# YuyangSunshine/ABR_IOD

Hardware: AMD Instinct MI355X
Metric: training images/sec (R50-C4 Faster R-CNN + ARD) (higher is better)
Workload: dtype f32 (tensors, accumulation and error bound; contractions via a 2-term fp16 split of both operands scaled by their amax, 3 cross products on the fp16 matrix cores: f16x3)

## Files before the change

abr_iod_amd/_lib.py:

```python
import ctypes as C
import os

import torch

_HERE = os.path.dirname(os.path.abspath(__file__))
LIB_PATH = os.environ.get("ABR_IOD_HIP_LIB") or os.path.join(_HERE, "libabr_iod_hip.so")

NCHW, NHWC = 0, 1

_vp, _i, _f, _i64 = C.c_void_p, C.c_int, C.c_float, C.c_int64


class ConvDesc(C.Structure):

    _fields_ = [
        ("B", _i), ("H", _i), ("W", _i), ("Cin", _i),
        ("Cout", _i), ("R", _i), ("S", _i),
        ("stride", _i), ("pad", _i),
        ("Ho", _i), ("Wo", _i),
        ("scale", _vp), ("bias", _vp), ("residual", _vp), ("mask", _vp),
        ("relu", _i),
        ("out_H", _i), ("out_W", _i), ("out_sh", _i), ("out_sw", _i),
        ("math", _i),
        ("wino_v", _vp),
        ("w_planes", _vp),
        ("w_version", _i64),
        ("x_amax", _vp), ("x_amax_epoch", C.c_uint32),
        ("gy_amax", _vp), ("gy_amax_epoch", C.c_uint32),
        ("out_amax", _vp), ("out_amax_epoch", C.c_uint32),
    ]


class ConvOp(C.Structure):

    _fields_ = [("kind", C.c_int32), ("reserved", C.c_int32), ("desc", ConvDesc), ("a", _vp), ("b", _vp), ("out", _vp), ("stream", _vp), ("other", _vp)]


OP_FORWARD, OP_WGRAD, OP_STREAM_WAIT = 0, 1, 2


class PrepItem(C.Structure):

    _fields_ = [("w", _vp), ("scale", _vp), ("wt", _vp),
                ("Cout", C.c_int32), ("R", C.c_int32), ("S", C.c_int32), ("Cin", C.c_int32), ("stride", C.c_int32), ("pad", C.c_int32), ("math", C.c_int32),
                ("w_version", _i64)]


_SIGS = {
    "abr_version": (_i, []),
    "abr_device_info": (_i, [_vp]),
    "abr_prof_begin": (_i, []),
    "abr_prof_mark_overlap": (_i, [_i]),
    "abr_prof_set_mask": (_i, [C.c_uint32, _i]),
    "abr_prof_end": (_i, [_vp, _i]),
    "abr_prof_totals": (_i, [_vp, _i]),
    "abr_prof_bytes": (_i, [_vp, _i]),
    "abr_prof_clocks": (_i, [_vp, _i]),
    "abr_prof_event_overhead_ms": (_i, [_vp, _vp]),
    "abr_prof_step_begin": (_i, []),
    "abr_conv_prepare_weights": (_i, [_vp, _i, _i, _i, _i, _i, _i, _i, _i64, _vp]),
    "abr_conv_prepare_batch": (_i, [_vp, _i, _vp]),
    "abr_conv_run": (_i, [_vp, _i]),
    "abr_conv_cache_clear": (_i, []),
    "abr_conv_cache_drop_range": (_i, [_vp, _i64]),
    "abr_conv_cache_bytes": (_i64, []),
    "abr_scratch_bytes": (_i64, []),
    "abr_roi_head_targets": (_i, [_vp, _vp, _vp, _i, _i, _i, _vp, _vp, _vp, _i, _f, _f, _f, _f, _f, _f, _i, _i, C.c_uint64,
                                  _vp, _vp, _vp, _vp, _vp, _vp, _vp, _vp, _vp, _vp, _vp, _vp, _vp, _vp, _vp, _vp, _vp, _i, _i, _vp]),
    "abr_roi_head_targets_table": (_i, [_vp, _vp, _vp, _i, _i, _vp, _vp, _vp, _i, _f, _f, _f, _f, _f, _f, _i, _i, C.c_uint64,
                                        _vp, _vp, _vp, _vp, _vp, _vp, _vp, _vp, _vp, _vp, _vp, _vp, _vp, _vp, _vp, _vp, _i, _i, _vp]),
    "abr_h3_amax_max": (_i, [_vp, _vp, _i, _vp, C.c_uint32, _vp]),
    "abr_rpn_targets_batched": (_i, [_vp, _i, _i, _vp, _vp, _i, _vp, _f, _f, _f, _f, _f, _f, _vp, _vp, _vp, _i64, _vp]),
    "abr_rpn_loss_indices": (_i, [_vp, _i, _vp, _i, _vp, _i, _i, _i, _vp, _vp, _vp, _vp, _vp, _vp]),
    "abr_loss_sum": (_i, [_vp, _vp, _vp, _i, _vp, _vp, _vp]),
    "abr_loss_sum_backward": (_i, [_vp, _i, _vp, _vp, _vp]),
    "abr_gather_proposals": (_i, [_vp, _vp, _vp, _i, _i, _i, _vp, _i, _vp, _vp, _vp]),
    "abr_h3_amax_alloc": (_i, [_vp, _vp]),
    "abr_h3_amax_alloc_block": (_i, [_i, _vp, _vp]),
    "abr_stream_wait_stream": (_i, [_vp, _vp]),
    "abr_h3_amax": (_i, [_vp, _i64, _vp, C.c_uint32, _vp]),
    "abr_h3_range_stats": (_i, [_vp, _i, _vp]),
    "abr_h3_range_stats_to_device": (_i, [_vp, _i, _vp]),
    "abr_x6_range_flags": (_i, [_vp, _i, _vp]),
    "abr_x6_range_flags_async": (_i, [_vp, _vp]),
    "abr_x6_range_flags_to_device": (_i, [_vp, _vp]),
    "abr_roi_align_forward": (_i, [_vp, _vp, _i, _i, _i, _i, _i, _f, _i, _i, _i, _i, _i, _vp, _vp]),
    "abr_roi_align_backward": (_i, [_vp, _vp, _i, _i, _i, _i, _i, _f, _i, _i, _i, _i, _i, _i, _vp, _vp]),
    "abr_roi_align_backward_ws_bytes": (_i64, [_i, _i, _i, _i, _i, _i, _i]),
    "abr_roi_align_backward_gather": (_i, [_vp, _vp, _i, _i, _i, _i, _i, _f, _i, _i, _i, _i, _i, _vp, _vp, _i64, _vp]),
    "abr_roi_align_taps": (_i, [_vp, _i, _i, _i, _f, _i, _i, _i, _i, _vp, _vp, _vp]),
    "abr_fpn_levels": (_i, [_vp, _i, _f, _f, _f, _f, _f, _vp, _vp]),
    "abr_roi_align_pyramid_forward": (_i, [_vp, _vp, _vp, _vp, _i, _vp, _i, _i, _i, _i, _i, _i, _f, _f, _f, _f, _f, _vp, _vp, _vp]),
    "abr_roi_align_pyramid_backward": (_i, [_vp, _vp, _i, _i, _i, _vp, _vp, _vp, _i, _i, _i, _i, _f, _f, _f, _f, _f, _i, _vp, _vp]),
    "abr_fpn_topdown_forward": (_i, [_vp, _vp, _vp, _vp, _i, _i, _i, _vp]),
    "abr_fpn_topdown_backward": (_i, [_vp, _vp, _vp, _vp, _i, _i, _i, _vp]),
    "abr_fpn_subsample2_forward": (_i, [_vp, _i, _i, _i, _i, _vp, _vp]),
    "abr_fpn_subsample2_backward": (_i, [_vp, _vp, _i, _i, _i, _i, _vp, _vp]),
    "abr_roi_pool_forward": (_i, [_vp, _vp, _i, _i, _i, _i, _i, _f, _i, _i, _i, _vp, _vp, _vp]),
    "abr_roi_pool_backward": (_i, [_vp, _vp, _vp, _i, _i, _i, _i, _i, _i, _i, _i, _i, _vp, _vp]),
    "abr_roi_pool_forward_f64": (_i, [_vp, _vp, _i, _i, _i, _i, _i, C.c_double, _i, _i, _vp, _vp, _vp]),
    "abr_roi_pool_backward_f64": (_i, [_vp, _vp, _vp, _i, _i, _i, _i, _i, _i, _i, _vp, _vp]),
    "abr_deform_psroi_forward": (_i, [_vp, _vp, _vp, _vp, _i, _i, _i, _i, _i, _f, _i, _i, _i, _i, _i, _f, _i, _i, _vp, _vp, _vp]),
    "abr_deform_psroi_backward": (_i, [_vp, _vp, _vp, _vp, _vp, _vp, _i, _i, _i, _i, _i, _f, _i, _i, _i, _i, _i, _f, _i, _i, _vp, _vp, _vp, _vp]),
    "abr_nms_workspace_bytes": (_i64, [_i, _i]),
    "abr_nms_unsorted_workspace_bytes": (_i64, [_i]),
    "abr_nms": (_i, [_vp, _vp, _i, _f, _i, _vp, _vp, _vp, _i64, _vp]),
    "abr_sort_scores_max_n": (_i64, []),
    "abr_sort_scores_desc": (_i, [_vp, _i, _vp, _vp]),
    "abr_nms_sorted_batched": (_i, [_vp, _vp, _i, _i, _f, _i, _i, _vp, _vp, _vp, _i64, _vp]),
    "abr_roi_align_forward_f64": (_i, [_vp, _vp, _i, _i, _i, _i, _i, C.c_double, _i, _i, _i, _vp, _vp]),
    "abr_roi_align_backward_f64": (_i, [_vp, _vp, _i, _i, _i, _i, _i, C.c_double, _i, _i, _i, _vp, _vp]),
    "abr_sigmoid_focal_forward_f64": (_i, [_vp, _vp, _i, _i, _f, _f, _vp, _vp]),
    "abr_sigmoid_focal_backward_f64": (_i, [_vp, _vp, _vp, _i, _i, _f, _f, _vp, _vp]),
    "abr_sigmoid_focal_forward": (_i, [_vp, _vp, _i, _i, _f, _f, _vp, _vp]),
    "abr_sigmoid_focal_backward": (_i, [_vp, _vp, _vp, _i, _i, _f, _f, _vp, _vp]),
    "abr_ard_forward": (_i, [_vp, _vp, _i, _i, _i, _f, _i, _vp, _vp, _vp]),
    "abr_ard_backward": (_i, [_vp, _vp, _vp, _i, _i, _i, _f, _i, _f, _vp, _vp, _vp]),
    "abr_smooth_l1": (_i, [_vp, _vp, _i64, _f, _f, _vp, _f, _vp, _vp]),
    "abr_smooth_l1_rows": (_i, [_vp, _i, _vp, _vp, _vp, _vp, _i, _f, _f, _vp, _vp, _f, _vp, _vp]),
    "abr_softmax_ce": (_i, [_vp, _i, _vp, _i, _i, _i, _i, _vp, _f, _vp, _i, _vp]),
    "abr_feat_distill": (_i, [_vp, _vp, _i64, _vp, _vp, _f, _vp, _vp]),
    "abr_rpn_distill": (_i, [_vp, _vp, _i, _i, _vp, _vp, _i, _i, _i64, _i, _f, _i, _vp, _f, _vp, _vp, _i, _i, _vp]),
    "abr_roi_distill": (_i, [_vp, _vp, _vp, _vp, _i, _i, _i, _vp, _i, _vp, _f, _vp, _vp, _vp]),
    "abr_bce_logits_gather": (_i, [_vp, _vp, _vp, _vp, _i, _vp, _vp, _f, _vp, _vp]),
    "abr_img_resample_u8": (_i, [_vp, _i, _i, _vp, _i, _i, _vp, _vp, _i, _vp, _vp, _i, _vp, _vp]),
    "abr_img_blend_paste_u8": (_i, [_vp, _i, _i, _vp, _i, _i, _i, _i, _i, _i, _i, _i, C.c_double, _vp]),
    "abr_img_copy_rect_u8": (_i, [_vp, _i, _i, _vp, _i, _i, _i, _i, _i, _i, _i, _i, _vp]),
    "abr_img_fill_u8": (_i, [_vp, _i64, _i, _vp]),
    "abr_img_color_jitter_u8": (_i, [_vp, _i, _i, _i, C.c_double, _vp, _vp]),
    "abr_img_normalize_to_batch": (_i, [_vp, _i, _i, _i, _i, C.POINTER(C.c_float), C.POINTER(C.c_float), _vp, _i, _i, _vp]),
    "abr_conv_forward": (_i, [C.POINTER(ConvDesc), _vp, _vp, _vp, _vp]),
    "abr_conv_tail64_forward": (_i, [C.POINTER(ConvDesc), C.POINTER(ConvDesc), _vp, _vp, _vp, _vp, _vp]),
    "abr_conv_wgrad": (_i, [C.POINTER(ConvDesc), _vp, _vp, _vp, _vp]),
    "abr_conv_wino_v_floats": (_i64, [C.POINTER(ConvDesc)]),
    "abr_conv_route_info": (_i, [C.POINTER(ConvDesc), C.POINTER(C.c_int32)]),
    "abr_conv_packed_bytes": (_i64, [_i64, _i64]),
    "abr_conv_pack_weights": (_i, [_vp, _i64, _i, _vp, _vp]),
    "abr_conv_dgrad_weights": (_i, [_vp, _vp, _i, _i, _i, _i, _vp, _vp]),
    "abr_bias_grad": (_i, [_vp, _i64, _i, _vp, _vp]),
    "abr_nchw_to_nhwc_pad": (_i, [_vp, _i, _i, _i, _i, _i, _vp, _vp]),
    "abr_nchw_to_nhwc": (_i, [_vp, _i, _i, _i, _i, _vp, _vp]),
    "abr_nhwc_to_nchw": (_i, [_vp, _i, _i, _i, _i, _vp, _vp]),
    "abr_maxpool3x3s2": (_i, [_vp, _i, _i, _i, _i, _vp, _vp]),
    "abr_maxpool3x3s2_backward": (_i, [_vp, _vp, _i, _i, _i, _i, _vp, _vp]),
    "abr_deform_im2col": (_i, [_vp, _vp, _i, _i, _i, _i, _i, _i, _i, _vp, _vp]),
    "abr_deform_col2im_coord": (_i, [_vp, _vp, _vp, _i, _i, _i, _i, _i, _i, _i, _vp, _vp, _vp, C.c_uint32, _vp]),
    "abr_deform_im2col_general": (_i, [_vp, _vp, _vp] + [_i] * 16 + [_vp, _vp]),
    "abr_deform_col2im_coord_general": (_i, [_vp, _vp, _vp, _vp] + [_i] * 16 + [_vp, _vp, _vp, _vp]),
    "abr_avgpool_forward": (_i, [_vp, _i, _i, _i, _vp, _vp]),
    "abr_avgpool_backward": (_i, [_vp, _i, _i, _i, _vp, _vp]),
    "abr_avgpool_relu_backward": (_i, [_vp, _vp, _i, _i, _i, _vp, _vp]),
    "abr_avgpool_relu_backward_amax": (_i, [_vp, _vp, _i, _i, _i, _vp, _vp, C.c_uint32, _vp]),
    "abr_channel_mean": (_i, [_vp, _i64, _i, _vp, _vp]),
    "abr_relu_backward": (_i, [_vp, _vp, _i64, _vp, _vp]),
    "abr_add_inplace": (_i, [_vp, _vp, _i64, _vp]),
    "abr_scale_inplace": (_i, [_vp, _i64, _f, _vp, _vp]),
    "abr_grid_anchors": (_i, [_vp, _i, _i, _i, _i, _i, _i, _i, _vp, _vp, _vp]),
    "abr_topk_sigmoid": (_i, [_vp, _i64, _i, _i, _i, _i, _i, _vp, _vp, _vp]),
    "abr_det_softmax_decode": (_i, [_vp, _i, _vp, _i, _i, _i, _vp, _i, _i, _vp, _f, _f, _f, _f, _vp, _vp, _vp]),
    "abr_det_select_workspace_bytes": (_i64, [_i, _i, _i]),
    "abr_det_select": (_i, [_vp, _vp, _vp, _i, _i, _i, _f, _f, _i, _i, _vp, _vp, _vp, _vp, _vp, _vp, _vp, _vp, _i64, _vp]),
    "abr_rpn_decode_clip": (_i, [_vp, _i, _i, _i, _vp, _vp, _i, _i, _i, _vp, _f, _f, _f, _f, _vp, _vp]),
    "abr_rpn_pyramid_max_k": (_i, []),
    "abr_rpn_pyramid_topk": (_i, [_vp, _vp, _vp, _vp, _i, _i, _i, _i, _vp, _vp, _vp]),
    "abr_rpn_pyramid_decode": (_i, [_vp, _vp, _vp, _vp, _vp, _i, _i, _i, _i, _vp, _vp, _vp, _f, _f, _f, _f, _f, _vp, _vp, _vp, _vp]),
    "abr_rpn_pyramid_select": (_i, [_vp, _vp, _vp, _vp, _i, _i, _i, _i, _i, _i, _vp, _vp, _vp, _vp, _vp]),
    "abr_rpn_pyramid_loss": (_i, [_vp, _vp, _i, _i, _i, _i, _vp, _vp, _vp, _i, _vp, _i, _vp, _vp, _vp, _vp, _vp]),
    "abr_rpn_pyramid_loss_backward": (_i, [_vp, _i, _i, _i, _i, _vp, _vp, _i, _i, _vp, _vp, _vp, _vp]),
    "abr_box_encode": (_i, [_vp, _vp, _i, _f, _f, _f, _f, _vp, _vp]),
    "abr_match_workspace_bytes": (_i64, [_i, _i]),
    "abr_match_encode": (_i, [_vp, _i, _vp, _vp, _i, _vp, _f, _f, _i, _f, _f, _f, _f, _vp, _vp, _vp, _vp, _vp, _i64, _vp]),
    "abr_sample_pos_neg": (_i, [_vp, _i, _i, _i, _i64, _i, _i, C.c_uint64, _i, _i64, _vp, _vp, _vp, _vp]),
    "abr_sgd_momentum": (_i, [_vp, _vp, _vp, _i64, _vp, _vp, _vp, _i, _f, _f, _i, _vp]),
    "abr_comm_rccl_version": (_i, []),
    "abr_comm_unique_id": (_i, [_vp]),
    "abr_comm_init": (_i, [_i, _i, _vp, C.POINTER(_vp)]),
    "abr_comm_info": (_i, [_vp, _vp]),
    "abr_comm_destroy": (_i, [_vp]),
    "abr_allreduce_flat": (_i, [_vp, _vp, _vp, _i, _vp]),
    "abr_mask_compact_pos": (_i, [_vp, _i, _i, _vp, _vp, _vp, _vp, _vp]),
    "abr_mask_gather_rows": (_i, [_vp, _vp, _i, _i, _i64, _vp, _vp]),
    "abr_mask_targets": (_i, [_vp, _vp, _i, _vp, _vp, _vp, _i, _i, _i, _i, _vp, _vp]),
    "abr_mask_d2s_bias_relu": (_i, [_vp, _vp, _i, _i, _i, _i, _vp, _vp]),
    "abr_mask_d2s_bias_relu_backward": (_i, [_vp, _vp, _i, _i, _i, _i, _vp, _vp]),
    "abr_mask_loss": (_i, [_vp, _i, _i, _vp, _vp, _i, _i, _vp, _vp, _f, _vp, _vp]),
    "abr_mask_select_sigmoid": (_i, [_vp, _i, _i, _vp, _i, _i, _vp, _vp]),
    "abr_mask_paste": (_i, [_vp, _vp, _i, _i, _i, _i, _f, _vp, _vp]),
    "abr_mask_pack_bits": (_i, [_vp, _i, _i, _i, _i, _vp, _vp]),
    "abr_mask_resize_pack_bits": (_i, [_vp, _i, _i, _i, _i, _i, _vp, _vp]),
    "abr_mask_pair_counts": (_i, [_vp, _vp, _vp, _vp, _i, _i, _i, _i, _i64, _vp, _vp, _vp, _vp]),
    "abr_rle_decode_workspace_bytes": (_i64, [_i, _i64]),
    "abr_rle_decode": (_i, [_vp, _vp, _vp, _i, _i64, _i, _i, _vp, _vp, _vp, _vp, _i64, _vp]),
    "abr_rle_encode_workspace_bytes": (_i64, [_i, _i, _i]),
    "abr_rle_encode": (_i, [_vp, _vp, _i, _i, _i, _vp, _i64, _vp, _vp, _vp, _i64, _vp]),
    "abr_poly_rasterize_workspace_bytes": (_i64, [_i64, _i, _i]),
    "abr_poly_rasterize": (_i, [_vp, _vp, _vp, _i, _i64, _i64, _i, _i, _vp, _vp, _vp, _vp, _i64, _vp]),
    "abr_poly_mask_targets": (_i, [_vp, _vp, _vp, _vp, _vp, _vp, _vp, _i, _i, _i, _i, _vp, _vp]),
    "abr_coco_match_max_gt": (_i, []),
    "abr_coco_box_iou": (_i, [_vp, _vp, _vp, _vp, _vp, _vp, _i, _i64, _vp, _vp]),
    "abr_coco_mask_iou": (_i, [_vp, _vp, _vp, _vp, _i, _i, _vp, _vp]),
    "abr_coco_match": (_i, [_vp, _vp, _vp, _vp, _vp, _vp, _vp, _i, _i64, _i64, _vp, _i, _vp, _i, _vp, _vp, _vp, _vp, _vp]),
    "abr_coco_match_ig": (_i, [_vp, _vp, _vp, _vp, _vp, _vp, _vp, _vp, _i, _i64, _i64, _vp, _i, _vp, _i, _vp, _vp, _vp, _vp, _vp]),
    "abr_coco_oks": (_i, [_vp, _vp, _vp, _vp, _vp, _i, _vp, _vp, _vp, _i, _i64, _vp, _vp]),
    "abr_kp_select_targets": (_i, [_vp, _vp, _i, _vp, _vp, _vp, _i, _i, _i, _i, _vp, _vp, _vp, _vp, _vp, _vp, _vp]),
    "abr_kp_deconv_fold": (_i, [_vp, _vp, _i, _i, _i, _i, _vp, _vp]),
    "abr_kp_deconv_unfold": (_i, [_vp, _i, _i, _i, _i, _vp, _vp]),
    "abr_kp_upsample2x": (_i, [_vp, _i, _i, _i, _i, _vp, _vp]),
    "abr_kp_loss_max_plane": (_i, []),
    "abr_kp_loss": (_i, [_vp, _i, _i, _i, _i, _vp, _vp, _vp, _f, _vp, _vp, _vp, _vp]),
    "abr_kp_decode": (_i, [_vp, _i64, _i64, _vp, _i, _i, _i, _i, _vp, _vp, _vp]),
    "abr_proposal_cover_max_prop": (_i, []),
    "abr_proposal_cover": (_i, [_vp, _vp, _vp, _vp, _vp, _i, _i64, _i64, _vp, _i, _vp, _i, _vp, _i, _vp, _vp, _vp, _vp, _vp]),
}

EXPORTS = sorted(list(_SIGS) + ["abr_last_error"])

_lib = None
# ... 60 lines not shown
```

abr_iod_amd/csrc/common.h:

```cpp
#pragma once
#include <hip/hip_runtime.h>
#include <stdint.h>
#include <stdio.h>

#include <functional>
#include <vector>

#include "abr_iod_hip.h"
#include "scratch.h"

namespace abr {

__device__ __forceinline__ float relu_f(const float v) { return v < 0.f ? 0.f : v; }

__device__ __forceinline__ float box_iou(const float4 g, const float4 b) {
#pragma clang fp contract(off)
    const float area1 = (g.z - g.x + 1) * (g.w - g.y + 1);
    const float area2 = (b.z - b.x + 1) * (b.w - b.y + 1);
    const float lx = fmaxf(g.x, b.x), ly = fmaxf(g.y, b.y), rx = fminf(g.z, b.z), ry = fminf(g.w, b.w);
    const float w = fmaxf(rx - lx + 1, 0.f), h = fmaxf(ry - ly + 1, 0.f);
    const float inter = w * h;
    return inter / (area1 + area2 - inter);
}

// ... 19 lines not shown
constexpr int kWave = 64;
constexpr int kNumXCD = 8;

__device__ __forceinline__ unsigned xcd_remap(unsigned bid, unsigned nblk) {
    const unsigned q = nblk / kNumXCD, r = nblk % kNumXCD;
    const unsigned xcd = bid % kNumXCD, pos = bid / kNumXCD;
    const unsigned base = xcd < r ? xcd * (q + 1) : r * (q + 1) + (xcd - r) * q;
    return base + pos;
}

__device__ __forceinline__ float wave_sum(float v) {
#pragma unroll
    for (int o = 32; o > 0; o >>= 1) v += __shfl_xor(v, o, 64);
    return v;
}
__device__ __forceinline__ float wave_max(float v) {
#pragma unroll
    for (int o = 32; o > 0; o >>= 1) v = fmaxf(v, __shfl_xor(v, o, 64));
    return v;
}

template <int NW>
__device__ __forceinline__ float block_sum(float v, float* sm) {
    v = wave_sum(v);
    const int w = threadIdx.x >> 6, l = threadIdx.x & 63;
    __syncthreads();
    if (l == 0) sm[w] = v;
    __syncthreads();
    float t = 0.f;
#pragma unroll
    for (int i = 0; i < NW; i++) t += sm[i];
    return t;
}

struct DetWs {
    float* part;
    unsigned* ticket;
};
DetWs det_ws(hipStream_t st, size_t nfloats);
template <int NV>
__device__ __forceinline__ bool det_sum_last(const float (&vals)[NV], const DetWs ws, float (&total)[NV]) {
    __shared__ int s_last;
    __shared__ float s_w[16];
    const unsigned nblk = gridDim.x * gridDim.y, bid = blockIdx.y * gridDim.x + blockIdx.x;
    if (threadIdx.x == 0) {
#pragma unroll
        for (int j = 0; j < NV; j++) __hip_atomic_store(ws.part + (size_t)bid * NV + j, vals[j], __ATOMIC_RELAXED, __HIP_MEMORY_SCOPE_AGENT);
        __builtin_amdgcn_fence(__ATOMIC_RELEASE, "agent");
        asm volatile("s_waitcnt vmcnt(0)" ::: "memory");
        s_last = atomicAdd(ws.ticket, 1u) == nblk - 1u;
    }
    __syncthreads();
    if (!s_last) return false;
    if (threadIdx.x == 0) {
        __builtin_amdgcn_fence(__ATOMIC_ACQUIRE, "agent");
        *ws.ticket = 0u;
    }
    __syncthreads();
#pragma unroll
    for (int j = 0; j < NV; j++) {
        float a = 0.f;
        for (unsigned i = threadIdx.x; i < nblk; i += blockDim.x) a += __hip_atomic_load(ws.part + (size_t)i * NV + j, __ATOMIC_RELAXED, __HIP_MEMORY_SCOPE_AGENT);
        a = wave_sum(a);
        __syncthreads();
        if ((threadIdx.x & 63) == 0) s_w[threadIdx.x >> 6] = a;
        __syncthreads();
        float t = 0.f;
        for (unsigned w = 0; w < (blockDim.x >> 6); w++) t += s_w[w];
        total[j] = t;
    }
    return true;
}

enum ProfId { PROF_IGEMM_128x128 = 0, PROF_IGEMM_128x64, PROF_IGEMM_64x64, PROF_IGEMM_SMALLC, PROF_WGRAD, PROF_ROIALIGN_FWD,
              PROF_ROIALIGN_BWD, PROF_IGEMM_BF16, PROF_WGRAD_BF16,
              PROF_X6_128x128, PROF_X6_128x64, PROF_X6_64x64, PROF_X6W_128x128, PROF_X6W_128x64, PROF_X6W_64x64, PROF_X6W_TAIL64,
              PROF_H3W_128x128, PROF_H3W_128x64, PROF_H3W_64x64, PROF_WGRAD_H3,
              PROF_F16W_128x128, PROF_F16W_128x64, PROF_F16W_64x64, PROF_WGRAD_F16, PROF_COUNT };
struct AmaxRef;
int wino_input_transform(const float* x, int B, int H, int W, int C, float* V, hipStream_t st, const AmaxRef* amax = nullptr);
int wino_output_transform(const float* M, int B, int H, int W, int N, const float* scale, const float* bias, int relu, const float* mask,
                          float* out, hipStream_t st, const AmaxRef* amax = nullptr);
int wino_outgrad_transform(const float* gy, int B, int H, int W, int N, float* Mg, hipStream_t st, const AmaxRef* amax = nullptr);
int wino_wgrad_inverse(const float* dU, int N, int C, const float* scale, float* dw, hipStream_t st);
ScratchPool& scratch_pool();
inline void* scratch(ScratchSlot slot, hipStream_t st, size_t bytes, size_t zero_prefix = 0) { return scratch_pool().scratch(slot, st, bytes, zero_prefix); }
inline float* wino_ws(hipStream_t st, size_t floats) { return static_cast<float*>(scratch(SCRATCH_WINO, st, floats * sizeof(float))); }
int num_cus();
enum DerivedKind { DERIVED_NONE = -1, DERIVED_WINO_U = 0, DERIVED_X6_PLANES = 1, DERIVED_WINO_U_X6_PLANES = 2, DERIVED_H3_PLANES = 3, DERIVED_WINO_U_H3_PLANES = 4 };
void* derived_cached(const void* w, int kind, size_t bytes, int64_t version, hipStream_t st, const std::function<int(void*)>& fill);
void* derived_acquire(const void* w, int kind, size_t bytes, int64_t version, hipStream_t st, void** token, std::vector<hipStream_t>* waited = nullptr);
void derived_commit(void* const* tokens, int n, hipStream_t st);
void derived_abandon(void* const* tokens, int n);

struct ConvRoute {
    int math;
    int wgrad_math;
    bool fwd_wino;
    bool wgrad_wino;
    int64_t v_floats;
    int kind;
    int64_t rows;
    int K;
    size_t bytes;
};
ConvRoute conv_route(const abr_conv_desc& d);

struct PrepJob {
    const float* src;
    const float* scale;
    void* dst;
    int a, b, c;
    int gx, gy;
    int first_block;
};
struct PrepTable { const PrepJob* jobs; int njobs; };
template <int PrepJob::*F = &PrepJob::first_block>
__device__ __forceinline__ PrepJob prep_job(const PrepTable& t, int block) {
    int lo = 0, hi = t.njobs - 1;
    while (lo < hi) {
        const int mid = (lo + hi + 1) >> 1;
        if (t.jobs[mid].*F <= block) lo = mid; else hi = mid - 1;
    }
    return t.jobs[lo];
}
template <int PrepJob::*F = &PrepJob::first_block>
__device__ __forceinline__ PrepJob prep_job(const PrepJob& j, int) { return j; }
struct PrepJobs { int n = 0; PrepJob one{}; const PrepJob* dev = nullptr; };
template <class F>
void prep_each(const PrepJobs& s, F&& f) {
    if (s.n == 1) f(s.one);
    else if (s.n > 1) f(PrepTable{s.dev, s.n});
}
__device__ __forceinline__ size_t h3_planes_bytes_dev(int rows, int K) { return (size_t)((rows + 31) / 32 * 32) * (size_t)K * 4; }
__host__ __device__ __forceinline__ int prep_transpose_tile(int Cout, int Cin, const void* w, const void* wt) {
    return (((Cout | Cin) & 3) == 0 && ((reinterpret_cast<uintptr_t>(w) | reinterpret_cast<uintptr_t>(wt)) & 15) == 0) ? 64 : 32;
}
void prep_wino_u(const PrepJobs& jobs, int blocks, hipStream_t st);
void prep_wino_h3_direct(const PrepJobs& jobs, int pack_blocks, int scale_blocks, unsigned* flags, hipStream_t st);
void derived_cache_clear();
void derived_cache_drop_range(const void* base, size_t bytes);
size_t derived_cache_bytes();

unsigned* x6_flags_ptr();
constexpr unsigned kX6TinyB = (17u << 24) - 1u;
__device__ __forceinline__ void x6_report(unsigned bmin, float nonfin, unsigned* flags) {
    unsigned f = 0;
    if (bmin < kX6TinyB) f |= ABR_X6_FLAG_TINY;
    if (nonfin != nonfin) f |= ABR_X6_FLAG_NONFINITE;
    if (f) atomicOr(flags, f);
}

struct AmaxRef {
    unsigned long long* word;
    unsigned epoch;
};
constexpr unsigned kH3RangeBinades = 18;
AmaxRef h3_amax_alloc();
int h3_amax_reduce(const float* x, int64_t n, AmaxRef ref, hipStream_t st);
void h3_amax_remember(const void* tensor, AmaxRef ref);
AmaxRef h3_amax_recall(const void* tensor);

__device__ __forceinline__ unsigned h3_amax_load(const unsigned long long* word, unsigned epoch) {
    const unsigned long long v = __hip_atomic_load(word, __ATOMIC_RELAXED, __HIP_MEMORY_SCOPE_AGENT);
    return (unsigned)(v >> 32) == epoch ? (unsigned)v : 0xFFFFFFFFu;
}
__device__ __forceinline__ void h3_scales(unsigned amax_bits, float& s, float& inv_s) {
    int e = (int)(amax_bits >> 23);
    if (amax_bits == 0u || e >= 255) { s = 1.f; inv_s = 1.f; return; }
    e = e < 15 ? 15 : e;
    s = __uint_as_float((unsigned)(e - 14) << 23);
    inv_s = __uint_as_float((unsigned)(268 - e) << 23);
}
__device__ __forceinline__ void h3_amax_emit(unsigned long long* word, unsigned epoch, unsigned local_bits) {
    __shared__ unsigned sm[16];
#pragma unroll
    for (int o = 32; o > 0; o >>= 1) local_bits = max(local_bits, (unsigned)__shfl_xor((int)local_bits, o, 64));
    __syncthreads();
    if ((threadIdx.x & 63) == 0) sm[threadIdx.x >> 6] = local_bits;
    __syncthreads();
    if (threadIdx.x == 0) {
        unsigned m = sm[0];
        for (unsigned i = 1; i < (blockDim.x >> 6); i++) m = max(m, sm[i]);
        const unsigned long long mine = ((unsigned long long)epoch << 32) | m;
        if (__hip_atomic_load(word, __ATOMIC_RELAXED, __HIP_MEMORY_SCOPE_AGENT) < mine) atomicMax(word, mine);
    }
}
__device__ __forceinline__ void h3_split2(const float a, const float b, const float inv_s, unsigned& o0, unsigned& o1) {
    unsigned h0, h1;
    asm("v_fma_mixlo_f16 %0, %1, %2, 0 op_sel_hi:[0,0,0]" : "=v"(h0) : "v"(a), "v"(inv_s));
    asm("v_fma_mixhi_f16 %0, %1, %2, 0 op_sel_hi:[0,0,0]" : "+v"(h0) : "v"(b), "v"(inv_s));
    asm("v_fma_mixlo_f16 %0, %1, %2, -%3 op_sel:[0,0,0] op_sel_hi:[0,0,1]" : "=v"(h1) : "v"(a), "v"(inv_s), "v"(h0));
    asm("v_fma_mixhi_f16 %0, %1, %2, -%3 op_sel:[0,0,1] op_sel_hi:[0,0,1]" : "+v"(h1) : "v"(b), "v"(inv_s), "v"(h0));
    o0 = h0; o1 = h1;
}
__device__ __forceinline__ unsigned h3_round2(const float a, const float b, const float inv_s) {
    unsigned h0;
// ... 57 lines not shown
```

abr_iod_amd/csrc/conv_igemm.hip:

```cpp
#include <algorithm>
#include <map>

#include <map>
#include <mutex>
#include <vector>

#include "common.h"

namespace {

typedef float f32x16 __attribute__((ext_vector_type(16)));

constexpr int BK = 32;
constexpr int LDP = BK + 4;

constexpr int kMaxSplitUnits = 1024, kMaxSplitTiles = 512;
constexpr int EPAD = 4;

struct FastDiv {
    unsigned mul, shr, d;
    __host__ void init(unsigned div) {
        d = div;
        shr = 0;
        while ((1u << shr) < div) shr++;
// ... 1151 lines not shown
    const int64_t t12864 = (int64_t)((p.M + 127) / 128) * ((p.Cout + 63) / 64) * nb;
    const int cus = abr::num_cus();
    static const int split_mode = getenv("ABR_IGEMM_SPLIT") ? atoi(getenv("ABR_IGEMM_SPLIT")) : 1;
    const int nk = (p.K + BK - 1) / BK;
    int best_nfull = -1, best_s = 1;
    double cost128 = (double)((t128 + cus - 1) / cus) * nk;
    if (split_mode && !small_c && p.Cout > 64 && nb == 1) {
        const long nfull = (t128 / cus) * cus, tail = t128 - nfull;
        for (int sp = 2; sp <= 6 && tail > 0 && nfull > 0; sp++) {
            if (nk / sp < 32 || tail * sp > kMaxSplitUnits || tail > kMaxSplitTiles) break;
            const double c = (double)(nfull / cus) * nk + (double)((tail * sp + cus - 1) / cus) * ((double)nk / sp + 24.0);
            if (c < cost128 * 0.93) { cost128 = c; best_nfull = (int)nfull; best_s = sp; }
        }
    }
    const int64_t t64 = (int64_t)((p.M + 63) / 64) * ((p.Cout + 63) / 64) * nb;
    const double cost12864 = (double)((t12864 + cus - 1) / cus) * nk * 0.5 / 0.85;
    const double cost64 = (double)((t64 + cus - 1) / cus) * nk * 0.25 / 0.80;
    const bool rule128 = p.Cout > 64 && t128 >= 2 * cus;
    const bool rule12864 = !rule128 && (t12864 >= 2 * cus || p.Cout <= 64);
    const bool take_split128 = best_s > 1 && (rule128 || cost128 < 0.9 * (rule12864 ? cost12864 : cost64));

    const int64_t wgs128 = take_split128 ? best_nfull + (t128 - best_nfull) * best_s : t128;
    const bool sb = p.K <= 512 || (wgs128 > 2 * cus && wgs128 <= 3 * cus) || take_split128;
    const char* fc_env = getenv("ABR_IGEMM_FC_SPLIT");
    const bool fc_split = !(fc_env && atoi(fc_env) == 0);
    if (fc_split && !small_c && nb == 1 && p.Cout <= 128 && t64 * 2 <= cus && nk >= 16 && t64 <= kMaxSplitTiles) {
        int sp = (int)std::min<int64_t>(nk / 4, std::max<int64_t>(2, 2 * cus / t64));
        sp = (int)std::min<int64_t>(sp, kMaxSplitUnits / t64);
        if (sp >= 2) {
            launch<64, 64, 2, 2, false, true>(p, x, w, out, st, abr::PROF_IGEMM_64x64, 0, sp);
            return;
        }
    }
    if (small_c) {
        launch<128, 64, 4, 1, true, true>(p, x, w, out, st, abr::PROF_IGEMM_SMALLC);
    } else if (rule128 || take_split128) {
        const int nf = take_split128 ? best_nfull : -1, sp = take_split128 ? best_s : 1;
        if (sb) launch<128, 128, 2, 2, false, true>(p, x, w, out, st, abr::PROF_IGEMM_128x128, nf, sp);
        else launch<128, 128, 2, 2, false, false>(p, x, w, out, st, abr::PROF_IGEMM_128x128, nf, sp);
    } else if (rule12864) {
        launch<128, 64, 4, 1, false, true>(p, x, w, out, st, abr::PROF_IGEMM_128x64);
    } else {
        launch<64, 64, 2, 2, false, true>(p, x, w, out, st, abr::PROF_IGEMM_64x64);
    }
}

static void dispatch_igemm_x6(const ConvP& p, const float* x, const float* , float* out, hipStream_t st) {
    const int cus = abr::num_cus();
    const int64_t nb = p.nbatch > 1 ? p.nbatch : 1;
    const int64_t t128 = (int64_t)((p.M + 127) / 128) * ((p.Cout + 127) / 128) * nb;
    const int64_t t12864 = (int64_t)((p.M + 127) / 128) * ((p.Cout + 63) / 64) * nb;
    if (p.K <= 256 && nb == 1 && p.nprod != 3) launch_x6w<64, 64, 2, 2>(p, x, out, st);
    else if (p.Cout > 64 && t128 >= 2 * cus) launch_x6w<128, 128, 1, 4>(p, x, out, st);
    else if (t12864 >= 2 * cus || p.Cout <= 64) launch_x6w<128, 64, 2, 2>(p, x, out, st);
    else launch_x6w<64, 64, 2, 2>(p, x, out, st);
}

namespace abr {
ConvRoute conv_route(const abr_conv_desc& d) {
    static const int min_c = getenv("ABR_WINOGRAD_MIN_C") ? atoi(getenv("ABR_WINOGRAD_MIN_C")) : 128;
    static const bool wino_wgrad = !(getenv("ABR_WINOGRAD_WGRAD") && atoi(getenv("ABR_WINOGRAD_WGRAD")) == 0);
    ConvRoute r{};
    const bool bf16_off = d.math == ABR_MATH_BF16 && d.Cin % 64 != 0;
    r.math = ((d.math == ABR_MATH_BF16X6 || d.math == ABR_MATH_F16X3 || d.math == ABR_MATH_F16) && d.Cin % BKX != 0) || bf16_off ? ABR_MATH_F32 : d.math;
    r.wgrad_math = bf16_off ? ABR_MATH_F32 : d.math;
    const int64_t T = (int64_t)d.B * ((d.H + 3) / 4) * ((d.W + 3) / 4);
    const bool wide3x3 = min_c > 0 && d.R == 3 && d.S == 3 && d.stride == 1 && d.pad == 1 && d.Cin >= min_c && d.Cout >= 128 &&
                         T * std::max(d.Cin, d.Cout) * 4 < (int64_t)0x7FFFFFF0;
    const bool scatter = !((d.out_H <= 0 || d.out_H == d.Ho) && (d.out_W <= 0 || d.out_W == d.Wo) && d.out_sh <= 1 && d.out_sw <= 1);
    const bool rounded = r.math == ABR_MATH_BF16 || r.math == ABR_MATH_F16, wg_rounded = r.wgrad_math == ABR_MATH_BF16 || r.wgrad_math == ABR_MATH_F16;
    r.fwd_wino = wide3x3 && !scatter && !d.residual && !rounded && d.Cin % BK == 0 && d.Cout % 4 == 0 &&
                 (r.math == ABR_MATH_F32 || d.Cout % 32 == 0);
    r.wgrad_wino = wide3x3 && wino_wgrad && !wg_rounded && d.Cin % 4 == 0;
    r.v_floats = r.fwd_wino && r.wgrad_wino && d.math != ABR_MATH_BF16 && d.math != ABR_MATH_F16 ? 36 * T * d.Cin : 0;
    const bool h3 = r.math == ABR_MATH_F16X3 || r.math == ABR_MATH_F16, x6 = r.math == ABR_MATH_BF16X6 || r.math == ABR_MATH_BF16;
    r.rows = r.fwd_wino ? (int64_t)36 * d.Cout : d.Cout;
    r.K = r.fwd_wino ? d.Cin : d.R * d.S * d.Cin;
    if (r.fwd_wino) r.kind = h3 ? DERIVED_WINO_U_H3_PLANES : (x6 ? DERIVED_WINO_U_X6_PLANES : DERIVED_WINO_U);
    else if ((h3 ? h3_planes_bytes(r.rows, r.K) : x6_packed_bytes(r.rows, r.K)) >= (int64_t)0xFFFFFFF0) r.kind = DERIVED_NONE;
    else r.kind = h3 ? DERIVED_H3_PLANES : (x6 ? DERIVED_X6_PLANES : DERIVED_NONE);
    r.bytes = r.kind == DERIVED_NONE ? 0 : (size_t)(r.kind == DERIVED_WINO_U ? r.rows * r.K * 4 : (h3 ? h3_packed_bytes(r.rows, r.K) : x6_packed_bytes(r.rows, r.K)));
    return r;
}
}

static bool wino_split_kind(int kind) { return kind == abr::DERIVED_WINO_U_X6_PLANES || kind == abr::DERIVED_WINO_U_H3_PLANES; }

namespace {
constexpr size_t kPrepRing = 8192;
struct PrepTables {
    abr::PrepJob* host = nullptr;
    abr::PrepJob* dev = nullptr;
    size_t head = 0;
    std::vector<std::pair<size_t, hipEvent_t>> inflight;
    size_t inflight_begin = 0;
};
std::map<hipStream_t, PrepTables> g_prep_tables;
std::mutex g_prep_mu;

bool prep_ring_take(PrepTables& T, hipStream_t st, size_t n, size_t* first) {
    if (n > kPrepRing) return false;
    if (!T.host) {
        void* dev = abr::scratch(abr::SCRATCH_PREP_RING, st, kPrepRing * sizeof(abr::PrepJob));
        if (!dev || hipHostMalloc(&T.host, kPrepRing * sizeof(abr::PrepJob)) != hipSuccess) { T.host = nullptr; return false; }
        T.dev = static_cast<abr::PrepJob*>(dev);
    }
    if (T.head + n > kPrepRing) {
        for (auto& pr : T.inflight) { (void)hipEventSynchronize(pr.second); (void)hipEventDestroy(pr.second); }
        T.inflight.clear();
        T.head = 0;
    }
    *first = T.head;
    T.head += n;
    return true;
}

enum PrepKind { PREP_TRANSPOSE, PREP_WINO_U, PREP_X6, PREP_H3, PREP_WINO_H3, PREP_KINDS };
struct PrepPlan {
    std::vector<abr::PrepJob> jobs[PREP_KINDS];
    int blocks[PREP_KINDS] = {};
    int scale_blocks[PREP_KINDS] = {};
    struct ViaU { size_t u_job, pack_job; int pack_kind; size_t off; };
    std::vector<ViaU> via_u;
    size_t u_floats = 0;

    abr::PrepJob& add(int k, const float* src, void* dst, int a, int b, int gx, int gy, int nblocks) {
        abr::PrepJob j{};
        j.src = src; j.dst = dst; j.a = a; j.b = b; j.gx = gx; j.gy = gy; j.first_block = blocks[k];
        blocks[k] += nblocks;
        jobs[k].push_back(j);
        return jobs[k].back();
    }
    void transpose(const float* w, const float* scale, float* wt, int Cout, int RS, int Cin) {
        const int tile = abr::prep_transpose_tile(Cout, Cin, w, wt);
        const int gx = (Cin + tile - 1) / tile, gy = (Cout + tile - 1) / tile;
        abr::PrepJob& j = add(PREP_TRANSPOSE, w, wt, Cout, RS, gx, gy, gx * gy * RS);
        j.scale = scale; j.c = Cin;
    }
    void pack(bool h3, const float* m, int64_t rows, int K, void* dst) {
        const int gx = (K + 63) / 64, gy = (int)((rows + 31) / 32);
        abr::PrepJob& j = add(h3 ? PREP_H3 : PREP_X6, m, dst, (int)rows, K, gx, gy, gx * gy);
        if (h3) { j.c = scale_blocks[PREP_H3]; scale_blocks[PREP_H3] += gy * 8; }
    }
    void derived(const abr::ConvRoute& r, const float* w, void* dst) {
        if (r.kind == abr::DERIVED_NONE) return;
        const bool h3 = r.kind == abr::DERIVED_H3_PLANES || r.kind == abr::DERIVED_WINO_U_H3_PLANES;
        if (r.kind == abr::DERIVED_H3_PLANES || r.kind == abr::DERIVED_X6_PLANES) return pack(h3, w, r.rows, r.K, dst);
        const int N = (int)(r.rows / 36), C = r.K;
        if (h3 && C % 64 == 0) {
            abr::PrepJob& j = add(PREP_WINO_H3, w, dst, N, C, C / 64, N / 32, (C / 64) * (N / 32));
            j.c = scale_blocks[PREP_WINO_H3];
            scale_blocks[PREP_WINO_H3] += N / 4;
            return;
        }
        const int gx = (int)(((int64_t)N * (C / 4) + 255) / 256);
        const bool via = r.kind != abr::DERIVED_WINO_U;
        add(PREP_WINO_U, w, via ? nullptr : dst, N, C, gx, 1, gx);
        if (!via) return;
        const int pk = h3 ? PREP_H3 : PREP_X6;
        via_u.push_back({jobs[PREP_WINO_U].size() - 1, jobs[pk].size(), pk, u_floats});
        pack(h3, nullptr, r.rows, r.K, dst);
        u_floats += (size_t)r.rows * r.K;
    }
};

const char* prep_launch(PrepPlan& p, float* u, hipStream_t st, PrepTables* T = nullptr) {
    if (p.u_floats && !u) return "no memory for the Winograd-domain scratch";
    for (const PrepPlan::ViaU& v : p.via_u) {
        p.jobs[PREP_WINO_U][v.u_job].dst = u + v.off;
        p.jobs[v.pack_kind][v.pack_job].src = u + v.off;
    }
    abr::PrepJobs src[PREP_KINDS];
    size_t njobs = 0;
    for (int k = 0; k < PREP_KINDS; k++) {
        src[k].n = (int)p.jobs[k].size();
        if (src[k].n == 1) src[k].one = p.jobs[k][0];
        else njobs += p.jobs[k].size();
    }
    if (njobs) {
        size_t first = 0;
        if (!T || !prep_ring_take(*T, st, njobs, &first)) return "no memory for the job tables";
        for (int k = 0, at = 0; k < PREP_KINDS; k++)
            if (src[k].n > 1) {
                std::copy(p.jobs[k].begin(), p.jobs[k].end(), T->host + first + at);
                src[k].dev = T->dev + first + at;
                at += src[k].n;
            }
        if (hipMemcpyAsync(T->dev + first, T->host + first, njobs * sizeof(abr::PrepJob), hipMemcpyHostToDevice, st) != hipSuccess) return "table upload failed";
        hipEvent_t up = nullptr;
        if (hipEventCreateWithFlags(&up, hipEventDisableTiming) == hipSuccess) {
            (void)hipEventRecord(up, st);
            T->inflight.emplace_back(first + njobs, up);
        }
    }
    abr::prep_each(src[PREP_TRANSPOSE], [&](auto s) { dgrad_weights_multi_kernel<<<(unsigned)p.blocks[PREP_TRANSPOSE], 256, 0, st>>>(s); });
    abr::prep_wino_u(src[PREP_WINO_U], p.blocks[PREP_WINO_U], st);
    abr::prep_each(src[PREP_X6], [&](auto s) { x6_pack_multi_kernel<<<(unsigned)p.blocks[PREP_X6], 256, 0, st>>>(s, abr::x6_flags_ptr()); });
    abr::prep_each(src[PREP_H3], [&](auto s) {
        h3_rowscale_multi_kernel<<<(unsigned)p.scale_blocks[PREP_H3], 256, 0, st>>>(s, abr::x6_flags_ptr());
        h3_pack_multi_kernel<<<(unsigned)p.blocks[PREP_H3], 256, 0, st>>>(s);
    });
    abr::prep_wino_h3_direct(src[PREP_WINO_H3], p.blocks[PREP_WINO_H3], p.scale_blocks[PREP_WINO_H3], abr::x6_flags_ptr(), st);
    return nullptr;
}
}

static const void* cached_weights(const abr::ConvRoute& r, const float* w, int64_t version, hipStream_t st) {
    if (!version) return nullptr;
    return abr::derived_cached(w, r.kind, r.bytes, version, st, [&](void* buf) {
        PrepPlan p;
        p.derived(r, w, buf);
        return prep_launch(p, p.u_floats ? abr::wino_ws(st, p.u_floats) : nullptr, st) || hipGetLastError() != hipSuccess;
    });
}

static const void* conv_weights(const abr::ConvRoute& r, const float* w, int64_t version, hipStream_t st, size_t own = 0, float** ws = nullptr) {
    const void* cached = cached_weights(r, w, version, st);
    const size_t mine = cached ? 0 : r.bytes / 4 + (wino_split_kind(r.kind) ? (size_t)r.rows * r.K : 0);
    float* s = own + mine ? abr::wino_ws(st, own + mine) : nullptr;
    if (ws) *ws = s;
    if (cached || !s) return cached;
    float* buf = s + own;
    PrepPlan p;
    p.derived(r, w, buf);
    return prep_launch(p, buf + r.bytes / 4, st) || hipGetLastError() != hipSuccess ? nullptr : buf;
}

static bool wino_conv(const ConvP& p, const abr::ConvRoute& r, const float* x, const float* w, float* out, hipStream_t st) {
    const int th_n = (p.H + 3) / 4, tw_n = (p.W + 3) / 4;
    const int64_t T = (int64_t)p.B * th_n * tw_n;
    const size_t nV = p.v_out ? 0 : (size_t)36 * T * p.Cin, nM = (size_t)36 * T * p.Cout;
    float* ws = nullptr;
    const void* U = conv_weights(r, w, p.w_version, st, nV + nM, &ws);
    if (!U || !ws) return false;
    float* V = p.v_out ? p.v_out : ws;
    float* Mm = ws + nV;
    const bool h3 = p.math == ABR_MATH_F16X3, x6 = p.math == ABR_MATH_BF16X6;
    abr::AmaxRef v_ref{nullptr, 0};
    if (h3) {
        v_ref = abr::h3_amax_alloc();
        if (!v_ref.word) return false;
        if (p.v_out) abr::h3_amax_remember(p.v_out, v_ref);
    }
    if (abr::wino_input_transform(x, p.B, p.H, p.W, p.Cin, V, st, h3 ? &v_ref : nullptr)) return false;
    ConvP g = p;
    g.B = (int)T; g.H = g.W = 1; g.R = g.S = 1; g.stride = 1; g.pad = 0; g.Ho = g.Wo = 1;
    g.M = (int)T; g.K = p.Cin;
    g.out_H = g.out_W = 1; g.out_sh = g.out_sw = 1; g.scatter = 0; g.relu = 0;
    g.scale = g.bias = g.residual = g.mask = nullptr;
    g.d_howo.init(1u); g.d_wo.init(1u); g.d_cin.init((unsigned)p.Cin); g.d_s.init(1u);
    g.x_bytes = (unsigned)(T * p.Cin * 4); g.w_bytes = (unsigned)((int64_t)p.Cout * p.Cin * 4);
    g.nbatch = 36; g.a_bs = (long)T * p.Cin; g.w_bs = (long)p.Cout * p.Cin; g.o_bs = (long)T * p.Cout;
    g.v_out = nullptr;
    g.out_amax = nullptr;
    if (h3) {
        g.w_planes = U; g.wp_bytes = (unsigned)h3_planes_bytes(p.Cout, p.Cin); g.wp_bs = (long)h3_planes_bytes(p.Cout, p.Cin); g.wp_nblocks = p.Cout / 32;
        g.w_scales = reinterpret_cast<const float*>(reinterpret_cast<const char*>(U) + h3_planes_bytes((int64_t)36 * p.Cout, p.Cin));
        g.a_amax = v_ref.word; g.a_epoch = v_ref.epoch;
    } else if (x6) {
        g.w_planes = U; g.wp_bytes = (unsigned)x6_packed_bytes(p.Cout, p.Cin); g.wp_bs = (long)x6_packed_bytes(p.Cout, p.Cin); g.wp_nblocks = p.Cout / 32;
    }
    if (h3 || x6) dispatch_igemm_x6(g, V, nullptr, Mm, st);
    else dispatch_igemm(g, V, static_cast<const float*>(U), Mm, st);
    const abr::AmaxRef o_ref{p.out_amax, p.out_epoch};
    return abr::wino_output_transform(Mm, p.B, p.H, p.W, p.Cout, p.scale, p.bias, p.relu, p.mask, out, st, p.out_amax ? &o_ref : nullptr) == 0;
}

extern "C" int64_t abr_conv_wino_v_floats(const abr_conv_desc* d) { return d ? abr::conv_route(*d).v_floats : 0; }

extern "C" int abr_conv_route_info(const abr_conv_desc* d, int32_t out[4]) {
    ABR_REQUIRE(d && out, "conv_route_info: null pointer");
    const abr::ConvRoute r = abr::conv_route(*d);
    out[0] = r.math; out[1] = r.fwd_wino ? 1 : 0; out[2] = r.wgrad_wino ? 1 : 0; out[3] = r.wgrad_math;
    return ABR_OK;
}

extern "C" int abr_conv_forward(const abr_conv_desc* d, const float* x, const float* w, float* out, void* stream) {
    ABR_REQUIRE(d && x && w && out, "conv_forward: null pointer");
    ABR_REQUIRE(d->B > 0 && d->H > 0 && d->W > 0 && d->Cin > 0 && d->Cout > 0 && d->R > 0 && d->S > 0 && d->stride > 0,
                "conv_forward: bad shape");
    ABR_REQUIRE(d->Cin % 4 == 0, "conv_forward: Cin must be a multiple of 4 (pad the 3-channel image to 4)");
    ABR_REQUIRE(d->Ho == (d->H + 2 * d->pad - d->R) / d->stride + 1 && d->Wo == (d->W + 2 * d->pad - d->S) / d->stride + 1,
                "conv_forward: Ho/Wo inconsistent with H,W,R,S,stride,pad");
    ConvP p;
    p.B = d->B; p.H = d->H; p.W = d->W; p.Cin = d->Cin; p.Cout = d->Cout; p.R = d->R; p.S = d->S;
    p.stride = d->stride; p.pad = d->pad; p.Ho = d->Ho; p.Wo = d->Wo;
    p.M = d->B * d->Ho * d->Wo;
    p.K = d->R * d->S * d->Cin;
    p.out_H = d->out_H > 0 ? d->out_H : d->Ho;
    p.out_W = d->out_W > 0 ? d->out_W : d->Wo;
    p.out_sh = d->out_sh > 0 ? d->out_sh : 1;
    p.out_sw = d->out_sw > 0 ? d->out_sw : 1;
    p.scatter = !(p.out_H == p.Ho && p.out_W == p.Wo && p.out_sh == 1 && p.out_sw == 1);
    ABR_REQUIRE((p.Ho - 1) * p.out_sh < p.out_H && (p.Wo - 1) * p.out_sw < p.out_W, "conv_forward: scatter out of range");
    p.relu = d->relu;
    p.scale = d->scale; p.bias = d->bias; p.residual = d->residual; p.mask = d->mask;
    p.tiles_m = p.tiles_n = 0; p.ngroup = 0;
    p.nbatch = 1; p.tiles_pb = 0; p.a_bs = p.w_bs = p.o_bs = 0;
    p.v_out = d->wino_v;
    p.w_version = d->w_version;
    p.w_planes = nullptr;
    ABR_REQUIRE(x6_packed_bytes(d->Cout, p.K) < (int64_t)0xFFFFFFF0, "conv_forward: weight tensor too large for 32-bit buffer offsets");
    p.wp_bytes = (unsigned)x6_packed_bytes(d->Cout, p.K); p.wp_bs = 0; p.wp_nblocks = (d->Cout + 31) / 32;
    const int64_t xb = (int64_t)d->B * d->H * d->W * d->Cin * 4, wb = (int64_t)d->Cout * p.K * 4;
    ABR_REQUIRE(xb < (int64_t)0x7FFFFFF0 && wb < (int64_t)0x7FFFFFF0, "conv_forward: input / weight tensors must be < 2 GB (32-bit buffer offsets)");
    p.x_bytes = (unsigned)xb; p.w_bytes = (unsigned)wb;
    p.d_howo.init((unsigned)(p.Ho * p.Wo)); p.d_wo.init((unsigned)p.Wo); p.d_cin.init((unsigned)p.Cin); p.d_s.init((unsigned)p.S);
    hipStream_t st = abr::as_stream(stream);
    ABR_REQUIRE(d->math == ABR_MATH_F32 || d->math == ABR_MATH_BF16 || d->math == ABR_MATH_BF16X6 || d->math == ABR_MATH_F16X3 || d->math == ABR_MATH_F16,
                "conv_forward: unknown math mode");
    const abr::ConvRoute r = abr::conv_route(*d);
    p.math = r.math;
    p.nprod = p.math == ABR_MATH_BF16 ? 1 : 6;
    p.a_amax = nullptr; p.a_epoch = 0; p.w_scales = nullptr;
    p.out_amax = reinterpret_cast<unsigned long long*>(d->out_amax); p.out_epoch = d->out_amax_epoch;
    const bool h3 = p.math == ABR_MATH_F16X3 || p.math == ABR_MATH_F16;
    if (h3) {
        abr::AmaxRef ar{reinterpret_cast<unsigned long long*>(const_cast<uint64_t*>(d->x_amax)), d->x_amax_epoch};
        if (!ar.word) {
            ar = abr::h3_amax_alloc();
            ABR_REQUIRE(ar.word && abr::h3_amax_reduce(x, (int64_t)d->B * d->H * d->W * d->Cin, ar, st) == 0, "conv_forward (f16x3): amax reduction failed");
        }
        p.a_amax = ar.word; p.a_epoch = ar.epoch;
        p.nprod = p.math == ABR_MATH_F16 ? 1 : 3;
        ABR_REQUIRE(h3_planes_bytes(d->Cout, p.K) < (int64_t)0xFFFFFFF0, "conv_forward: weight tensor too large for 32-bit buffer offsets");
        p.wp_bytes = (unsigned)h3_planes_bytes(d->Cout, p.K);
    }
    if (r.fwd_wino) {
        ABR_REQUIRE(wino_conv(p, r, x, w, out, st), "conv_forward (winograd): no memory for the scratch or an amax word, or a launch failed");
        ABR_CHECK_LAUNCH("conv_forward (winograd)");
        return ABR_OK;
    }
    ABR_REQUIRE(!d->wino_v, "conv_forward: wino_v given for a conv that does not take the Winograd path (abr_conv_wino_v_floats)");
    if (p.math != ABR_MATH_F32) {
        p.w_planes = !h3 ? d->w_planes : nullptr;
        if (!p.w_planes) p.w_planes = conv_weights(r, w, p.w_version, st);
        ABR_REQUIRE(p.w_planes, "conv_forward: no memory for the weight planes");
        if (h3) p.w_scales = reinterpret_cast<const float*>(reinterpret_cast<const char*>(p.w_planes) + h3_planes_bytes(d->Cout, p.K));
        dispatch_igemm_x6(p, x, w, out, st);
    } else {
        dispatch_igemm(p, x, w, out, st);
    }
    ABR_CHECK_LAUNCH("conv_forward");
    return ABR_OK;
}

static void convp_from_desc(const abr_conv_desc* d, ConvP& p) {
    p.B = d->B; p.H = d->H; p.W = d->W; p.Cin = d->Cin; p.Cout = d->Cout; p.R = d->R; p.S = d->S;
    p.stride = d->stride; p.pad = d->pad; p.Ho = d->Ho; p.Wo = d->Wo;
    p.M = d->B * d->Ho * d->Wo;
    p.K = d->R * d->S * d->Cin;
    p.out_H = d->Ho; p.out_W = d->Wo; p.out_sh = p.out_sw = 1; p.scatter = 0;
    p.relu = d->relu;
    p.scale = d->scale; p.bias = d->bias; p.residual = d->residual; p.mask = d->mask;
    p.tiles_m = (p.M + 127) / 128; p.tiles_n = 1; p.ngroup = 0;
    p.nbatch = 1; p.tiles_pb = p.tiles_m; p.a_bs = p.w_bs = p.o_bs = 0;
    p.n_full = p.tiles_m; p.split = 1; p.ws = nullptr; p.cnt = nullptr;
    p.v_out = nullptr;
    p.w_version = d->w_version;
    p.w_planes = d->w_planes;
    p.wp_bytes = (unsigned)x6_packed_bytes(d->Cout, p.K); p.wp_bs = 0; p.wp_nblocks = (d->Cout + 31) / 32;
    p.x_bytes = (unsigned)((int64_t)d->B * d->H * d->W * d->Cin * 4); p.w_bytes = (unsigned)((int64_t)d->Cout * p.K * 4);
    p.d_howo.init((unsigned)(p.Ho * p.Wo)); p.d_wo.init((unsigned)p.Wo); p.d_cin.init((unsigned)p.Cin); p.d_s.init((unsigned)p.S);
    p.math = d->math;
    p.nprod = 6;
    p.x6_flags = abr::x6_flags_ptr();
    p.prof_ts = nullptr;
}

extern "C" int abr_conv_tail64_forward(const abr_conv_desc* d2, const abr_conv_desc* d3, const float* x, const float* w2, const float* w3, float* out,
                                       void* stream) {
    ABR_REQUIRE(d2 && d3 && x && w2 && w3 && out, "conv_tail64_forward: null pointer");
    ABR_REQUIRE(d2->math == ABR_MATH_BF16X6 && d3->math == ABR_MATH_BF16X6, "conv_tail64_forward: bf16x6 arithmetic only");
    ABR_REQUIRE(d2->R == 3 && d2->S == 3 && d2->stride == 1 && d2->pad == 1 && d2->Cin == 64 && d2->Cout == 64 && d2->Ho == d2->H && d2->Wo == d2->W &&
                    !d2->residual && !d2->mask,
                "conv_tail64_forward: the first conv must be 3x3, stride 1, pad 1, 64 -> 64 channels, without residual / mask");
    ABR_REQUIRE(d3->R == 1 && d3->S == 1 && d3->stride == 1 && d3->pad == 0 && d3->Cin == 64 && d3->Cout == 256 && d3->B == d2->B && d3->H == d2->H &&
                    d3->W == d2->W && d3->Ho == d2->H && d3->Wo == d2->W && !d3->mask,
                "conv_tail64_forward: the second conv must be 1x1, stride 1, 64 -> 256 channels, on the first conv's output");
    ABR_REQUIRE((d2->out_H <= 0 || d2->out_H == d2->Ho) && (d3->out_H <= 0 || d3->out_H == d3->Ho) && d2->out_sh <= 1 && d3->out_sh <= 1 &&
                    (d2->out_W <= 0 || d2->out_W == d2->Wo) && (d3->out_W <= 0 || d3->out_W == d3->Wo) && d2->out_sw <= 1 && d3->out_sw <= 1,
                "conv_tail64_forward: no scattered outputs");
    ABR_REQUIRE((int64_t)d2->B * d2->H * d2->W * 256 * 4 < (int64_t)0x7FFFFFF0, "conv_tail64_forward: tensors must be < 2 GB (32-bit buffer offsets)");
    hipStream_t st = abr::as_stream(stream);
    ConvP p, q;
    convp_from_desc(d2, p);
    convp_from_desc(d3, q);
    auto planes_of = [&](const abr_conv_desc* d, const float* w, ConvP& c) -> bool {
        if (!c.w_planes) c.w_planes = cached_weights(abr::conv_route(*d), w, d->w_version, st);
        return c.w_planes != nullptr;
    };
    ABR_REQUIRE(planes_of(d2, w2, p) && planes_of(d3, w3, q), "conv_tail64_forward: needs w_version != 0 (or caller-packed planes) for both weights");
    static bool attr_set = false;
    if (!attr_set) {
        (void)hipFuncSetAttribute(reinterpret_cast<const void*>(conv_tail64_x6w_kernel), hipFuncAttributeMaxDynamicSharedMemorySize, (int)kTail64Lds);
        attr_set = true;
    }
    p.prof_ts = abr::prof_stamp_slot(abr::PROF_X6W_TAIL64, 2.0 * (double)p.M * ((double)p.Cout * p.K + (double)q.Cout * q.K));
    abr::prof_add_bytes(abr::PROF_X6W_TAIL64, 4.0 * (double)p.M * (64.0 + 256.0 * (q.residual ? 2.0 : 1.0)) + 6.0 * (64.0 * 576.0 + 256.0 * 64.0));
    conv_tail64_x6w_kernel<<<(unsigned)p.tiles_m, 256, kTail64Lds, st>>>(p, q, x, out);
    ABR_CHECK_LAUNCH("conv_tail64_forward");
    return ABR_OK;
}

static abr::ConvRoute prep_route(int Cout, int R, int S, int Cin, int stride, int pad, int math) {
    abr_conv_desc d{};
    d.Cout = Cout; d.R = R; d.S = S; d.Cin = Cin; d.stride = stride; d.pad = pad; d.math = math;
    return abr::conv_route(d);
}

extern "C" int abr_conv_prepare_weights(const float* w, int Cout, int R, int S, int Cin, int stride, int pad, int math, int64_t w_version,
                                        void* stream) {
    ABR_REQUIRE(w && w_version != 0, "conv_prepare_weights: needs a weight pointer and a non-zero w_version");
    ABR_REQUIRE(Cout > 0 && R > 0 && S > 0 && Cin > 0, "conv_prepare_weights: bad shape");
    const abr::ConvRoute r = prep_route(Cout, R, S, Cin, stride, pad, math);
    if (r.kind == abr::DERIVED_NONE) return ABR_OK;
    ABR_REQUIRE(cached_weights(r, w, w_version, abr::as_stream(stream)) != nullptr, "conv_prepare_weights: no memory for the derived weights");
    ABR_CHECK_LAUNCH("conv_prepare_weights");
    return ABR_OK;
}

extern "C" int abr_conv_prepare_batch(const abr_prep_item* items, int n, void* stream) {
    ABR_REQUIRE(n >= 0 && (n == 0 || items), "conv_prepare_batch: bad args");
    if (n == 0) return ABR_OK;
    hipStream_t st = abr::as_stream(stream);
    std::lock_guard<std::mutex> lock(g_prep_mu);
    PrepTables& T = g_prep_tables[st];
    PrepPlan plan;
    std::vector<void*> tokens;
    std::vector<hipStream_t> waited;
    struct TokenGuard {
        std::vector<void*>& t; bool committed = false;
        ~TokenGuard() { if (!committed && !t.empty()) abr::derived_abandon(t.data(), (int)t.size()); }
    } token_guard{tokens};
    auto derive = [&](const float* w, int Cout, int R, int S, int Cin, int stride, int pad, int math, int64_t ver) {
        const abr::ConvRoute r = prep_route(Cout, R, S, Cin, stride, pad, math);
        if (r.kind == abr::DERIVED_NONE) return true;
        void* tok = nullptr;
        void* dst = abr::derived_acquire(w, r.kind, r.bytes, ver, st, &tok, &waited);
        if (!dst) return false;
        if (tok) {
            tokens.push_back(tok);
            plan.derived(r, w, dst);
        }
        return true;
    };
    for (int i = 0; i < n; i++) {
        const abr_prep_item& it = items[i];
        ABR_REQUIRE(it.w && it.w_version != 0 && it.Cout > 0 && it.R > 0 && it.S > 0 && it.Cin > 0, "conv_prepare_batch: bad item");
        ABR_REQUIRE(derive(it.w, it.Cout, it.R, it.S, it.Cin, it.stride, it.pad, it.math, it.w_version), "conv_prepare_batch: no memory for the derived weights");
        if (it.wt) {
            plan.transpose(it.w, it.scale, it.wt, it.Cout, it.R * it.S, it.Cin);
            ABR_REQUIRE(derive(it.wt, it.Cin, it.R, it.S, it.Cout, 1, it.R - 1 - it.pad, it.math, it.w_version),
                        "conv_prepare_batch: no memory for the derived weights");
        }
    }
    float* u = plan.u_floats ? static_cast<float*>(abr::scratch(abr::SCRATCH_PREP_U, st, plan.u_floats * sizeof(float))) : nullptr;
    ABR_REQUIRE(!plan.u_floats || u, "conv_prepare_batch: no memory for the Winograd-domain scratch");
    const char* err = prep_launch(plan, u, st, &T);
    ABR_REQUIRE(!err, "conv_prepare_batch: %s", err);
    ABR_REQUIRE(hipGetLastError() == hipSuccess, "conv_prepare_batch: launch failed");
    abr::derived_commit(tokens.data(), (int)tokens.size(), st);
    token_guard.committed = true;
    ABR_CHECK_LAUNCH("conv_prepare_batch");
    return ABR_OK;
}

extern "C" int abr_conv_run(const abr_conv_op* ops, int n) {
    ABR_REQUIRE(n >= 0 && (n == 0 || ops), "conv_run: bad args");
    for (int i = 0; i < n; i++) {
        const abr_conv_op& o = ops[i];
        int rc;
        switch (o.kind) {
            case ABR_OP_FORWARD: rc = abr_conv_forward(&o.desc, o.a, o.b, o.out, o.stream); break;
            case ABR_OP_WGRAD: rc = abr_conv_wgrad(&o.desc, o.a, o.b, o.out, o.stream); break;
            case ABR_OP_STREAM_WAIT: rc = abr_stream_wait_stream(o.stream, o.other); break;
            default: ABR_REQUIRE(false, "conv_run: unknown op kind");
        }
        if (rc != ABR_OK) return rc;
    }
    return ABR_OK;
}

extern "C" int abr_conv_cache_clear(void) {
    abr::derived_cache_clear();
    return ABR_OK;
}
extern "C" int abr_conv_cache_drop_range(const void* base, int64_t bytes) {
    if (base && bytes > 0) abr::derived_cache_drop_range(base, (size_t)bytes);
    return ABR_OK;
}
extern "C" int64_t abr_conv_cache_bytes(void) { return (int64_t)abr::derived_cache_bytes(); }

extern "C" int64_t abr_conv_packed_bytes(int64_t rows, int64_t K) { return rows > 0 && K > 0 && K % 16 == 0 ? x6_packed_bytes(rows, K) : 0; }

extern "C" int abr_conv_pack_weights(const float* w, int64_t rows, int K, void* planes, void* stream) {
    ABR_REQUIRE(w && planes && rows > 0 && K > 0 && K % 16 == 0, "conv_pack_weights: needs pointers, rows > 0 and K a positive multiple of 16");
    ABR_REQUIRE(x6_packed_bytes(rows, K) < (int64_t)0xFFFFFFF0, "conv_pack_weights: packed matrix must stay below 4 GB (32-bit buffer offsets)");
    PrepPlan p;
    p.pack(false, w, rows, K, planes);
    ABR_REQUIRE(!prep_launch(p, nullptr, abr::as_stream(stream)) && hipGetLastError() == hipSuccess, "conv_pack_weights: launch failed");
    return ABR_OK;
}

extern "C" int abr_conv_dgrad_weights(const float* w, const float* scale, int Cout, int R, int S, int Cin, float* wt,
                                      void* stream) {
    ABR_REQUIRE(w && wt && Cout > 0 && R > 0 && S > 0 && Cin > 0, "conv_dgrad_weights: bad args");
    PrepPlan p;
    p.transpose(w, scale, wt, Cout, R * S, Cin);
    const char* err = prep_launch(p, nullptr, abr::as_stream(stream));
    ABR_REQUIRE(!err, "conv_dgrad_weights: %s", err);
    ABR_CHECK_LAUNCH("conv_dgrad_weights");
    return ABR_OK;
}

extern "C" int abr_bias_grad(const float* gy, int64_t M, int C, float* db, void* stream) {
    ABR_REQUIRE(M >= 0 && C > 0 && db, "bias_grad: bad args");
    if (M == 0) return ABR_OK;
    ABR_REQUIRE(gy, "bias_grad: null pointer");
    const int rows_per_block = 256;
    dim3 grid((C + 63) / 64, (unsigned)((M + rows_per_block - 1) / rows_per_block));
    abr::DetWs ws = grid.x <= 64 ? abr::det_ws(abr::as_stream(stream), (size_t)grid.x * grid.y * 64) : abr::DetWs{nullptr, nullptr};
    unsigned* tk = ws.part ? static_cast<unsigned*>(abr::scratch(abr::SCRATCH_BIAS_TICKETS, abr::as_stream(stream), 64 * sizeof(unsigned), 64 * sizeof(unsigned))) : nullptr;
    bias_grad_kernel<<<grid, 256, 0, abr::as_stream(stream)>>>(gy, M, C, rows_per_block, db, tk ? ws.part : nullptr, tk);
    ABR_CHECK_LAUNCH("bias_grad");
    return ABR_OK;
}
```

abr_iod_amd/csrc/conv_wgrad.hip:

```cpp
#include <algorithm>

#include "common.h"

namespace {

typedef float f32x16 __attribute__((ext_vector_type(16)));
typedef _Float16 f16x8 __attribute__((ext_vector_type(8)));

constexpr int TN_ = 128;
constexpr int TK_ = 128;
constexpr int MR = 32;

struct FastDiv {
    unsigned mul, shr, d;
    __host__ void init(unsigned div) {
        d = div;
        shr = 0;
        while ((1u << shr) < div) shr++;
        mul = (unsigned)((((unsigned long long)1 << 32) * (((unsigned long long)1 << shr) - div)) / div + 1);
    }
    __device__ __forceinline__ void divmod(unsigned n, unsigned& q, unsigned& r) const {
        q = (__umulhi(n, mul) + n) >> shr;
        r = n - q * d;
    }
// ... 481 lines not shown
    if (p.overwrite) splits = 1;
    p.splits = splits;
    p.mt_per_split = (m_tiles + splits - 1) / splits;
    wgrad_plan_reduction(p, tiles, abr::as_stream(stream));
    if (p.final_store && splits > 1 && !p.ws) {
        (void)hipMemsetAsync(dw, 0, sizeof(float) * (size_t)nb * p.Cout * p.K, abr::as_stream(stream));
        p.final_store = 0;
    }
    if (p.math == ABR_MATH_BF16X6 || p.math == ABR_MATH_BF16 || p.math == ABR_MATH_F16X3 || p.math == ABR_MATH_F16) {
        static bool attr6 = false;
        const bool one = p.math == ABR_MATH_BF16;
        const bool h3 = p.math == ABR_MATH_F16X3;
        const bool f16 = p.math == ABR_MATH_F16;
        const size_t lds6 = sizeof(unsigned) * (one || f16 ? 1 : (h3 ? 2 : 3)) * (MRX / 2) * (TN_ + TK_);
        if (!attr6) {
            (void)hipFuncSetAttribute(reinterpret_cast<const void*>(conv_wgrad_x6_kernel<6>), hipFuncAttributeMaxDynamicSharedMemorySize,
                                      (int)(sizeof(unsigned) * 3 * (MRX / 2) * (TN_ + TK_)));
            attr6 = true;
        }
        p.map4 = 1;
        p.x6_flags = !one ? abr::x6_flags_ptr() : nullptr;
        p.h3_stats = (h3 && p.x6_flags) ? abr::h3_stats_ptr() : nullptr;
        if (p.h3_stats) abr::h3_stats_inspected((double)nb * p.M * ((double)p.Cout + (double)p.K));
        const int pid6 = h3 ? abr::PROF_WGRAD_H3 : (f16 ? abr::PROF_WGRAD_F16 : abr::PROF_WGRAD_BF16);
        const int rec6 = abr::prof_start(abr::as_stream(stream), pid6, 2.0 * (double)p.M * (double)p.Cout * (double)p.K * nb);
        p.prof_ts = abr::prof_clock_slot(rec6);
        abr::prof_add_bytes(pid6, 4.0 * nb * ((double)p.M * p.Cout + (p.plain ? (double)p.M * p.K : (double)p.B * p.H * p.W * p.Cin) + (double)p.Cout * p.K));
        if (h3) conv_wgrad_x6_kernel<3><<<(unsigned)(tiles * splits), 256, lds6, abr::as_stream(stream)>>>(p, x, gy, dw);
        else if (f16) conv_wgrad_x6_kernel<1, true><<<(unsigned)(tiles * splits), 256, lds6, abr::as_stream(stream)>>>(p, x, gy, dw);
        else if (one) conv_wgrad_x6_kernel<1><<<(unsigned)(tiles * splits), 256, lds6, abr::as_stream(stream)>>>(p, x, gy, dw);
        else conv_wgrad_x6_kernel<6><<<(unsigned)(tiles * splits), 256, lds6, abr::as_stream(stream)>>>(p, x, gy, dw);
        abr::prof_stop(abr::as_stream(stream), rec6);
        wgrad_reduce(p, tiles, dw, abr::as_stream(stream));
        return;
    }
    const int rec = abr::prof_start(abr::as_stream(stream), abr::PROF_WGRAD, 2.0 * (double)p.M * (double)p.Cout * (double)p.K * nb);
    p.prof_ts = abr::prof_clock_slot(rec);
    conv_wgrad_kernel<true><<<(unsigned)(tiles * splits), 256, sizeof(float) * MR * (TN_ + TK_), abr::as_stream(stream)>>>(p, x, gy, dw);
    abr::prof_stop(abr::as_stream(stream), rec);
    wgrad_reduce(p, tiles, dw, abr::as_stream(stream));
}

extern "C" int abr_conv_wgrad(const abr_conv_desc* d, const float* x, const float* gy, float* dw, void* stream) {
    ABR_REQUIRE(d && x && gy && dw, "conv_wgrad: null pointer");
    ABR_REQUIRE(d->Cin % 4 == 0 && d->Cout % 4 == 0, "conv_wgrad: Cin and Cout must be multiples of 4");
    ABR_REQUIRE(d->Ho == (d->H + 2 * d->pad - d->R) / d->stride + 1 && d->Wo == (d->W + 2 * d->pad - d->S) / d->stride + 1,
                "conv_wgrad: Ho/Wo inconsistent");
    WgP p;
    p.B = d->B; p.H = d->H; p.W = d->W; p.Cin = d->Cin; p.Cout = d->Cout; p.R = d->R; p.S = d->S;
    p.stride = d->stride; p.pad = d->pad; p.Ho = d->Ho; p.Wo = d->Wo;
    p.M = d->B * d->Ho * d->Wo;
    p.K = d->R * d->S * d->Cin;
    p.plain = (d->R == 1 && d->S == 1 && d->stride == 1 && d->pad == 0);
    p.scale = d->scale;
    const int64_t xb = (int64_t)d->B * d->H * d->W * d->Cin * 4, gb = (int64_t)p.M * d->Cout * 4;
    ABR_REQUIRE(xb < (int64_t)0x7FFFFFF0 && gb < (int64_t)0x7FFFFFF0, "conv_wgrad: activation / gradient tensors must be < 2 GB (32-bit buffer offsets)");
    p.x_bytes = (unsigned)xb; p.gy_bytes = (unsigned)gb;
    p.d_howo.init((unsigned)(d->Ho * d->Wo)); p.d_wo.init((unsigned)d->Wo);
    p.tiles_n = (p.Cout + TN_ - 1) / TN_;
    p.tiles_k = (p.K + TK_ - 1) / TK_;
    if (p.M == 0) return ABR_OK;
    p.nbatch = 1; p.tiles_pb = 0; p.x_bs = p.gy_bs = p.dw_bs = 0; p.overwrite = 0;
    p.ws = nullptr; p.final_store = 0; p.map4 = 0;
    p.x6_flags = nullptr;
    p.gy_amax = p.x_amax = nullptr; p.gy_epoch = p.x_epoch = 0; p.h3_stats = nullptr;
    hipStream_t st = abr::as_stream(stream);
    ABR_REQUIRE(d->math == ABR_MATH_F32 || d->math == ABR_MATH_BF16 || d->math == ABR_MATH_BF16X6 || d->math == ABR_MATH_F16X3 || d->math == ABR_MATH_F16,
                "conv_wgrad: unknown math mode");
    const abr::ConvRoute route = abr::conv_route(*d);
    p.math = route.wgrad_math;
    const bool h3 = p.math == ABR_MATH_F16X3 || p.math == ABR_MATH_F16;
    abr::AmaxRef gy_ref{reinterpret_cast<unsigned long long*>(const_cast<uint64_t*>(d->gy_amax)), d->gy_amax_epoch};
    abr::AmaxRef x_ref{reinterpret_cast<unsigned long long*>(const_cast<uint64_t*>(d->x_amax)), d->x_amax_epoch};
    auto need_ref = [&](abr::AmaxRef& r, const float* t, int64_t n) -> bool {
        if (r.word) return true;
        r = abr::h3_amax_alloc();
        return r.word && abr::h3_amax_reduce(t, n, r, st) == 0;
    };
    if (route.wgrad_wino) {
        const int th_n = (d->H + 3) / 4, tw_n = (d->W + 3) / 4;
        const int64_t T = (int64_t)d->B * th_n * tw_n;
        const size_t nV = (size_t)36 * T * d->Cin, nM = (size_t)36 * T * d->Cout, nU = (size_t)36 * d->Cout * d->Cin;
        float* vin = route.v_floats ? d->wino_v : nullptr;
        float* ws = abr::wino_ws(st, (vin ? 0 : nV) + nM + nU);
        if (ws) {
            float* V = vin ? vin : ws;
            float *Mg = ws + (vin ? 0 : nV), *dU = Mg + nM;
            abr::AmaxRef v_ref{nullptr, 0}, m_ref{nullptr, 0};
            if (h3) {
                if (vin) v_ref = abr::h3_amax_recall(vin);
                else v_ref = abr::h3_amax_alloc();
                m_ref = abr::h3_amax_alloc();
                ABR_REQUIRE(m_ref.word && (vin || v_ref.word), "conv_wgrad (f16x3): no amax words");
                if (vin && !v_ref.word) ABR_REQUIRE(need_ref(v_ref, vin, (int64_t)nV), "conv_wgrad (f16x3): amax reduction failed");
            }
            int bad = vin ? 0 : abr::wino_input_transform(x, d->B, d->H, d->W, d->Cin, V, st, h3 ? &v_ref : nullptr);
            bad |= abr::wino_outgrad_transform(gy, d->B, d->H, d->W, d->Cout, Mg, st, h3 ? &m_ref : nullptr);
            const int cus_ = abr::num_cus();
            const long out_tiles = 36L * ((d->Cout + TN_ - 1) / TN_) * ((d->Cin + TK_ - 1) / TK_);
            const int own = out_tiles >= 2L * cus_;
            if (!bad) {
                WgP g = p;
                g.overwrite = own;
                g.final_store = !own;
                g.B = (int)T; g.H = g.W = 1; g.R = g.S = 1; g.stride = 1; g.pad = 0; g.Ho = g.Wo = 1;
                g.M = (int)T; g.K = d->Cin; g.plain = 1; g.scale = nullptr;
                g.d_howo.init(1u); g.d_wo.init(1u);
                g.tiles_n = (g.Cout + TN_ - 1) / TN_; g.tiles_k = (g.K + TK_ - 1) / TK_;
                g.x_bytes = (unsigned)(T * d->Cin * 4); g.gy_bytes = (unsigned)(T * d->Cout * 4);
                g.nbatch = 36; g.x_bs = (long)T * d->Cin; g.gy_bs = (long)T * d->Cout; g.dw_bs = (long)d->Cout * d->Cin;
                if (h3) { g.x_amax = v_ref.word; g.x_epoch = v_ref.epoch; g.gy_amax = m_ref.word; g.gy_epoch = m_ref.epoch; }
                launch_wgrad(g, V, Mg, dU, stream);
                bad = abr::wino_wgrad_inverse(dU, d->Cout, d->Cin, d->scale, dw, st);
            }
            ABR_REQUIRE(!bad, "conv_wgrad: winograd launch failed");
            ABR_CHECK_LAUNCH("conv_wgrad (winograd)");
            return ABR_OK;
        }
    }
    if (h3) {
        ABR_REQUIRE(need_ref(gy_ref, gy, (int64_t)p.M * d->Cout) && need_ref(x_ref, x, (int64_t)d->B * d->H * d->W * d->Cin), "conv_wgrad (f16x3): amax reduction failed");
        p.gy_amax = gy_ref.word; p.gy_epoch = gy_ref.epoch; p.x_amax = x_ref.word; p.x_epoch = x_ref.epoch;
    }
    launch_wgrad(p, x, gy, dw, stream);
    ABR_CHECK_LAUNCH("conv_wgrad");
    return ABR_OK;
}
```

abr_iod_amd/csrc/conv_winograd.hip:

```cpp
#include <map>

#include <algorithm>
#include <map>
#include <functional>
#include <mutex>
#include <utility>
#include <type_traits>
#include <vector>

#include "common.h"

namespace {

template <int V>
struct vf {
    float v[V];
};
template <int V>
__device__ __forceinline__ vf<V> operator+(vf<V> a, vf<V> b) {
    vf<V> r;
#pragma unroll
    for (int i = 0; i < V; i++) r.v[i] = a.v[i] + b.v[i];
    return r;
}
// ... 60 lines not shown
}

template <int V>
__device__ __forceinline__ unsigned vabs_max(unsigned m, vf<V> a) {
#pragma unroll
    for (int i = 0; i < V; i++) m = max(m, __float_as_uint(a.v[i]) & 0x7FFFFFFFu);
    return m;
}

template <int V>
__global__ __launch_bounds__(256) void wino_input_kernel(const float* __restrict__ x, int B, int H, int W, int C, int th_n, int tw_n,
                                                         float* __restrict__ Vo, unsigned long long* amax, unsigned epoch) {
    unsigned am = 0;
    typedef vf<V> f2;
    const int64_t T = (int64_t)B * th_n * tw_n;
    const int C2 = C / V;
    const int64_t total = T * C2;
    const int64_t ps = T * C;
    const __amdgpu_buffer_rsrc_t rx = __builtin_amdgcn_make_buffer_rsrc(const_cast<float*>(x), 0, (unsigned)((int64_t)B * H * W * C * 4), 0x00020000);
    for (int64_t idx = (int64_t)blockIdx.x * blockDim.x + threadIdx.x; idx < total; idx += (int64_t)gridDim.x * blockDim.x) {
        const int c = V * (int)(idx % C2);
        const int64_t t = idx / C2;
        const int tw = (int)(t % tw_n), th = (int)((t / tw_n) % th_n), b = (int)(t / ((int64_t)tw_n * th_n));
        const int y0 = 4 * th - 1, x0 = 4 * tw - 1;
        f2 tcol[6][6];
        const int base = (b * H * W) * C + c;
#pragma unroll
        for (int j = 0; j < 6; j++) {
            const int xx = x0 + j;
            const bool xin = (unsigned)xx < (unsigned)W;
            f2 d[6];
#pragma unroll
            for (int i = 0; i < 6; i++) {
                const int y = y0 + i;
                const bool in = xin & ((unsigned)y < (unsigned)H);
                d[i] = vld_buf<V>(rx, in ? (unsigned)(base + (y * W + xx) * C) * 4u : 0x80000000u);
            }
            bt6(d[0], d[1], d[2], d[3], d[4], d[5], tcol[0][j], tcol[1][j], tcol[2][j], tcol[3][j], tcol[4][j], tcol[5][j]);
        }
#pragma unroll
        for (int i = 0; i < 6; i++) {
            f2 v0, v1, v2, v3, v4, v5;
            bt6(tcol[i][0], tcol[i][1], tcol[i][2], tcol[i][3], tcol[i][4], tcol[i][5], v0, v1, v2, v3, v4, v5);
            float* o = Vo + ((int64_t)(6 * i) * T + t) * C + c;
            vst(o, v0); vst(o + ps, v1); vst(o + 2 * ps, v2); vst(o + 3 * ps, v3); vst(o + 4 * ps, v4); vst(o + 5 * ps, v5);
            if (amax) am = vabs_max(vabs_max(vabs_max(vabs_max(vabs_max(vabs_max(am, v0), v1), v2), v3), v4), v5);
        }
    }
    if (amax) abr::h3_amax_emit(amax, epoch, am);
}

template <int I, int V>
__device__ __forceinline__ void wino_u_row(const vf<V> (&g)[3][3], vf<V> (&u)[6]) {
#pragma clang fp contract(off)
    constexpr float k6 = -1.f / 6.f, c24 = 1.f / 24.f, c12 = 1.f / 12.f, c6 = 1.f / 6.f;
    constexpr float k = I == 0 ? 0.25f : k6;
#pragma unroll
    for (int e = 0; e < V; e++) {
        float t[3], s[3];
#pragma unroll
        for (int q = 0; q < 3; q++) {
            const float a = g[0][q].v[e], b = g[1][q].v[e], c = g[2][q].v[e];
            if constexpr (I == 0) { s[q] = a; t[q] = 0.25f * a; }
            else if constexpr (I == 1) { s[q] = (a + b) + c; t[q] = k6 * s[q]; }
            else if constexpr (I == 2) { s[q] = (a - b) + c; t[q] = k6 * s[q]; }
            else if constexpr (I == 3) { s[q] = 0.f; t[q] = __builtin_fmaf(c, c6, __builtin_fmaf(a, c24, b * c12)); }
            else if constexpr (I == 4) { s[q] = 0.f; t[q] = __builtin_fmaf(c, c6, __builtin_fmaf(a, c24, -(b * c12))); }
            else { s[q] = 0.f; t[q] = c; }
        }
        u[0].v[e] = 0.25f * t[0];
        if constexpr (I < 3) {
            u[1].v[e] = k6 * __builtin_fmaf(s[2], k, __builtin_fmaf(s[1], k, t[0]));
            u[2].v[e] = k6 * __builtin_fmaf(s[2], k, __builtin_fmaf(-s[1], k, t[0]));
        } else {
            u[1].v[e] = k6 * ((t[0] + t[1]) + t[2]);
            u[2].v[e] = k6 * ((t[0] - t[1]) + t[2]);
        }
        const float m = t[1] * c12;
        u[3].v[e] = __builtin_fmaf(t[2], c6, __builtin_fmaf(t[0], c24, m));
        u[4].v[e] = __builtin_fmaf(t[2], c6, __builtin_fmaf(t[0], c24, -m));
        u[5].v[e] = t[2];
    }
}
template <typename F>
__device__ __forceinline__ void for_rows6(F&& f) {
    f(std::integral_constant<int, 0>{}); f(std::integral_constant<int, 1>{}); f(std::integral_constant<int, 2>{});
    f(std::integral_constant<int, 3>{}); f(std::integral_constant<int, 4>{}); f(std::integral_constant<int, 5>{});
}

template <class Src>
__global__ __launch_bounds__(256) void wino_weight_multi_kernel(Src jobs) {
    typedef vf<4> fv;
    const abr::PrepJob jb = abr::prep_job(jobs, blockIdx.x);
    const float* w = jb.src;
    float* U = reinterpret_cast<float*>(jb.dst);
    const int N = jb.a, C = jb.b, Cv = C / 4;
    const int64_t total = (int64_t)N * Cv, ps = (int64_t)N * C;
    const int64_t idx = (int64_t)(blockIdx.x - jb.first_block) * 256 + threadIdx.x;
    if (idx >= total) return;
    const int c = 4 * (int)(idx % Cv);
    const int64_t n = idx / Cv;
    fv g[3][3];
#pragma unroll
    for (int r = 0; r < 3; r++)
#pragma unroll
        for (int q = 0; q < 3; q++) g[r][q] = vld<4>(w + ((n * 3 + r) * 3 + q) * C + c);
    for_rows6([&](auto I) {
        constexpr int i = decltype(I)::value;
        fv u[6];
        wino_u_row<i>(g, u);
        float* o = U + ((int64_t)(6 * i) * N + n) * C + c;
        vst(o, u[0]); vst(o + ps, u[1]); vst(o + 2 * ps, u[2]); vst(o + 3 * ps, u[3]); vst(o + 4 * ps, u[4]); vst(o + 5 * ps, u[5]);
    });
}


template <class Src>
__global__ __launch_bounds__(256, 3) void wino_h3_scales_multi_kernel(Src jobs, unsigned* flags) {
    typedef vf<4> fv;
    const abr::PrepJob jb = abr::prep_job<&abr::PrepJob::c>(jobs, blockIdx.x);
    const float* w = jb.src;
    const int N = jb.a, C = jb.b;
    const int lane = threadIdx.x & 63;
    const int64_t n = (int64_t)(blockIdx.x - jb.c) * 4 + (threadIdx.x >> 6);
    float* scales = reinterpret_cast<float*>(reinterpret_cast<char*>(jb.dst) + abr::h3_planes_bytes_dev(36 * N, C));
    unsigned mx[36];
#pragma unroll
    for (int k = 0; k < 36; k++) mx[k] = 0u;
#pragma clang loop unroll(disable) vectorize(disable) interleave(disable)
    for (int c = 4 * lane; c < C; c += 256) {
        fv g[3][3];
#pragma unroll
        for (int r = 0; r < 3; r++)
#pragma unroll
            for (int q = 0; q < 3; q++) g[r][q] = vld<4>(w + ((n * 3 + r) * 3 + q) * C + c);
        for_rows6([&](auto I) {
            constexpr int i = decltype(I)::value;
            fv u[6];
            wino_u_row<i>(g, u);
#pragma unroll
            for (int jj = 0; jj < 6; jj++) mx[6 * i + jj] = vabs_max(mx[6 * i + jj], u[jj]);
        });
    }
    __shared__ __attribute__((aligned(16))) unsigned red_[4][36][64];
    unsigned (*red)[64] = red_[threadIdx.x >> 6];
#pragma unroll
    for (int k = 0; k < 36; k++) red[k][lane] = mx[k];
    __builtin_amdgcn_wave_barrier();
    unsigned mine = 0u;
    if (lane < 36) {
        const uint4* rowp = reinterpret_cast<const uint4*>(red[lane]);
#pragma unroll
        for (int q = 0; q < 16; q++) {
            const uint4 v = rowp[q];
            mine = max(max(mine, max(v.x, v.y)), max(v.z, v.w));
        }
    }
    if (lane < 36) {
        float sc, inv;
        abr::h3_scales(mine, sc, inv);
        scales[(size_t)lane * N + n] = sc;
        if (flags && (mine >> 23) >= 255u) atomicOr(flags, ABR_X6_FLAG_NONFINITE);
    }
}

constexpr int kWhPitch = 9 * 64 + 4;
constexpr size_t kWhLds = sizeof(float) * 32 * kWhPitch;

template <class Src>
__global__ __launch_bounds__(256) void wino_h3_pack_multi_kernel(Src jobs) {
    typedef vf<4> fv;
    extern __shared__ __attribute__((aligned(16))) float wt_[];
    const abr::PrepJob jb = abr::prep_job(jobs, blockIdx.x);
    const float* w = jb.src;
    const int N = jb.a, C = jb.b;
    const int lb = blockIdx.x - jb.first_block;
    const int nblk = lb / jb.gx, kc = lb % jb.gx;
    const int n0 = nblk * 32, k0 = kc * 64;
    const int tid = threadIdx.x;
#pragma unroll
    for (int it = 0; it < 18; it++) {
        const int f = tid + 256 * it, rt = f >> 4, c4 = (f & 15) * 4;
        const int row = rt / 9, tap = rt - row * 9;
        *reinterpret_cast<float4*>(wt_ + row * kWhPitch + tap * 64 + c4) =
            *reinterpret_cast<const float4*>(w + (((int64_t)(n0 + row)) * 9 + tap) * C + k0 + c4);
    }
    __syncthreads();
    const int wave = tid >> 6, lane = tid & 63, row = lane & 31, k8 = wave * 16 + (lane >> 5) * 8;
    const float* src = wt_ + row * kWhPitch + k8;
    fv gA[3][3], gB[3][3];
#pragma unroll
    for (int r = 0; r < 3; r++)
#pragma unroll
        for (int q = 0; q < 3; q++) {
            const float4 a = *reinterpret_cast<const float4*>(src + (r * 3 + q) * 64), b = *reinterpret_cast<const float4*>(src + (r * 3 + q) * 64 + 4);
            gA[r][q] = {{a.x, a.y, a.z, a.w}};
            gB[r][q] = {{b.x, b.y, b.z, b.w}};
        }
    uint4* planes = reinterpret_cast<uint4*>(jb.dst);
    const float* scales = reinterpret_cast<const float*>(reinterpret_cast<const char*>(jb.dst) + abr::h3_planes_bytes_dev(36 * N, C));
    const int ks = kc * 4 + wave, KS = C / 16;
    auto emit = [&](int xi, const fv& uA, const fv& uB, float sc) {
        const float inv = 1.f / sc;
        unsigned h0[4], h1[4];
        abr::h3_split2(uA.v[0], uA.v[1], inv, h0[0], h1[0]);
        abr::h3_split2(uA.v[2], uA.v[3], inv, h0[1], h1[1]);
        abr::h3_split2(uB.v[0], uB.v[1], inv, h0[2], h1[2]);
        abr::h3_split2(uB.v[2], uB.v[3], inv, h0[3], h1[3]);
        const size_t nb = ((size_t)xi * N + n0) / 32;
        const size_t ch = (nb * KS + ks) * 2;
        planes[ch * 64 + lane] = make_uint4(h0[0], h0[1], h0[2], h0[3]);
        planes[(ch + 1) * 64 + lane] = make_uint4(h1[0], h1[1], h1[2], h1[3]);
    };
    auto row_i = [&](auto I) {
        constexpr int i = decltype(I)::value;
        float sc[6];
#pragma unroll
        for (int jj = 0; jj < 6; jj++) sc[jj] = scales[(size_t)(6 * i + jj) * N + n0 + row];
        fv uA[6], uB[6];
        wino_u_row<i>(gA, uA);
        wino_u_row<i>(gB, uB);
#pragma unroll
        for (int jj = 0; jj < 6; jj++) emit(6 * i + jj, uA[jj], uB[jj], sc[jj]);
    };
    for_rows6(row_i);
}

template <typename T>
__device__ __forceinline__ void at4(const T m0, const T m1, const T m2, const T m3, const T m4, const T m5, T& o0, T& o1, T& o2, T& o3) {
    const T s12 = m1 + m2, d12 = m1 - m2, s34 = m3 + m4, d34 = m3 - m4;
    o0 = m0 + s12 + s34;
    o1 = d12 + 2.f * d34;
    o2 = s12 + 4.f * s34;
    o3 = d12 + 8.f * d34 + m5;
}

template <int V>
__global__ __launch_bounds__(256) void wino_output_kernel(const float* __restrict__ Mm, int B, int H, int W, int N, int th_n, int tw_n,
                                                          const float* __restrict__ scale, const float* __restrict__ bias, int relu,
                                                          const float* __restrict__ mask, float* __restrict__ out, unsigned long long* amax, unsigned epoch) {
    typedef vf<V> f2;
    unsigned am = 0;
    const int64_t T = (int64_t)B * th_n * tw_n;
    const int N2 = N / V;
    const int64_t total = T * N2;
    const int64_t ps = T * N;
    for (int64_t idx = (int64_t)blockIdx.x * blockDim.x + threadIdx.x; idx < total; idx += (int64_t)gridDim.x * blockDim.x) {
        const int n = V * (int)(idx % N2);
        const int64_t t = idx / N2;
        const int tw = (int)(t % tw_n), th = (int)((t / tw_n) % th_n), b = (int)(t / ((int64_t)tw_n * th_n));
        const float* m = Mm + t * N + n;
        f2 tcol[4][6];
#pragma unroll
        for (int j = 0; j < 6; j++)
            at4(vld<V>(m + (0 + j) * ps), vld<V>(m + (6 + j) * ps), vld<V>(m + (12 + j) * ps), vld<V>(m + (18 + j) * ps), vld<V>(m + (24 + j) * ps),
                vld<V>(m + (30 + j) * ps), tcol[0][j], tcol[1][j], tcol[2][j], tcol[3][j]);
        f2 sc, bi;
#pragma unroll
        for (int e = 0; e < V; e++) { sc.v[e] = scale ? scale[n + e] : 1.f; bi.v[e] = bias ? bias[n + e] : 0.f; }
        f2 mk[4][4];
        if (mask) {
#pragma unroll
            for (int i = 0; i < 4; i++)
#pragma unroll
                for (int j = 0; j < 4; j++) {
                    const int oy = 4 * th + i, ox = 4 * tw + j;
                    const bool in = oy < H && ox < W;
                    mk[i][j] = vld<V>(mask + (((int64_t)b * H + (in ? oy : 4 * th)) * W + (in ? ox : 4 * tw)) * N + n);
                }
        }
#pragma unroll
        for (int i = 0; i < 4; i++) {
            f2 y[4];
            at4(tcol[i][0], tcol[i][1], tcol[i][2], tcol[i][3], tcol[i][4], tcol[i][5], y[0], y[1], y[2], y[3]);
            const int oy = 4 * th + i;
            if (oy >= H) continue;
#pragma unroll
            for (int j = 0; j < 4; j++) {
                const int ox = 4 * tw + j;
                if (ox >= W) continue;
                const int64_t o = (((int64_t)b * H + oy) * W + ox) * N + n;
                f2 v;
#pragma unroll
                for (int e = 0; e < V; e++) {
                    v.v[e] = y[j].v[e] * sc.v[e] + bi.v[e];
                    if (relu) v.v[e] = abr::relu_f(v.v[e]);
                }
                if (mask) {
#pragma unroll
                    for (int e = 0; e < V; e++) v.v[e] = mk[i][j].v[e] > 0.f ? v.v[e] : 0.f;
                }
                vst(out + o, v);
                if (amax) am = vabs_max(am, v);
            }
        }
    }
    if (amax) abr::h3_amax_emit(amax, epoch, am);
}

template <typename T>
__device__ __forceinline__ void a6(const T y0, const T y1, const T y2, const T y3, T& o0, T& o1, T& o2, T& o3, T& o4, T& o5) {
    o0 = y0;
    o1 = y0 + y1 + y2 + y3;
    o2 = y0 - y1 + y2 - y3;
    o3 = y0 + 2.f * y1 + 4.f * y2 + 8.f * y3;
    o4 = y0 - 2.f * y1 + 4.f * y2 - 8.f * y3;
    o5 = y3;
}

template <int V>
__global__ __launch_bounds__(256) void wino_outgrad_kernel(const float* __restrict__ gy, int B, int H, int W, int N, int th_n, int tw_n,
                                                           float* __restrict__ Mg, unsigned long long* amax, unsigned epoch) {
    typedef vf<V> f2;
    unsigned am = 0;
    const int64_t T = (int64_t)B * th_n * tw_n;
    const int N2 = N / V;
    const int64_t total = T * N2;
    const int64_t ps = T * N;
    for (int64_t idx = (int64_t)blockIdx.x * blockDim.x + threadIdx.x; idx < total; idx += (int64_t)gridDim.x * blockDim.x) {
        const int n = V * (int)(idx % N2);
        const int64_t t = idx / N2;
        const int tw = (int)(t % tw_n), th = (int)((t / tw_n) % th_n), b = (int)(t / ((int64_t)tw_n * th_n));
        f2 tcol[6][4];
#pragma unroll
        for (int j = 0; j < 4; j++) {
            const int ox = 4 * tw + j;
            f2 y[4];
#pragma unroll
            for (int i = 0; i < 4; i++) {
                const int oy = 4 * th + i;
                y[i] = (oy < H && ox < W) ? vld<V>(gy + (((int64_t)b * H + oy) * W + ox) * N + n) : vzero<V>();
            }
            a6(y[0], y[1], y[2], y[3], tcol[0][j], tcol[1][j], tcol[2][j], tcol[3][j], tcol[4][j], tcol[5][j]);
        }
#pragma unroll
        for (int i = 0; i < 6; i++) {
            f2 v0, v1, v2, v3, v4, v5;
            a6(tcol[i][0], tcol[i][1], tcol[i][2], tcol[i][3], v0, v1, v2, v3, v4, v5);
            float* o = Mg + ((int64_t)(6 * i) * T + t) * N + n;
            vst(o, v0); vst(o + ps, v1); vst(o + 2 * ps, v2); vst(o + 3 * ps, v3); vst(o + 4 * ps, v4); vst(o + 5 * ps, v5);
            if (amax) am = vabs_max(vabs_max(vabs_max(vabs_max(vabs_max(vabs_max(am, v0), v1), v2), v3), v4), v5);
        }
    }
    if (amax) abr::h3_amax_emit(amax, epoch, am);
}

template <typename T>
__device__ __forceinline__ void gt3(const T u0, const T u1, const T u2, const T u3, const T u4, const T u5, T& o0, T& o1, T& o2) {
    o0 = 0.25f * u0 - (1.f / 6.f) * (u1 + u2) + (1.f / 24.f) * (u3 + u4);
    o1 = (1.f / 6.f) * (u2 - u1) + (1.f / 12.f) * (u3 - u4);
    o2 = (1.f / 6.f) * (u3 + u4 - u1 - u2) + u5;
}

template <int V>
__global__ __launch_bounds__(256) void wino_wgrad_inverse_kernel(const float* __restrict__ dU, int N, int C, const float* __restrict__ scale,
                                                                 float* __restrict__ dw) {
    typedef vf<V> fv;
    const int Cv = C / V;
    const int64_t total = (int64_t)N * Cv;
    const int64_t ps = (int64_t)N * C;
    for (int64_t idx = (int64_t)blockIdx.x * blockDim.x + threadIdx.x; idx < total; idx += (int64_t)gridDim.x * blockDim.x) {
        const int c = V * (int)(idx % Cv);
        const int64_t n = idx / Cv;
        const float* u = dU + n * C + c;
        fv tcol[3][6];
#pragma unroll
        for (int j = 0; j < 6; j++)
            gt3(vld<V>(u + (0 + j) * ps), vld<V>(u + (6 + j) * ps), vld<V>(u + (12 + j) * ps), vld<V>(u + (18 + j) * ps), vld<V>(u + (24 + j) * ps),
                vld<V>(u + (30 + j) * ps), tcol[0][j], tcol[1][j], tcol[2][j]);
        const float sc = scale ? scale[n] : 1.f;
        fv old[3][3];
#pragma unroll
        for (int r = 0; r < 3; r++)
#pragma unroll
            for (int q = 0; q < 3; q++) old[r][q] = vld<V>(dw + ((n * 3 + r) * 3 + q) * C + c);
#pragma unroll
        for (int r = 0; r < 3; r++) {
            fv g0, g1, g2;
            gt3(tcol[r][0], tcol[r][1], tcol[r][2], tcol[r][3], tcol[r][4], tcol[r][5], g0, g1, g2);
            float* o = dw + ((n * 3 + r) * 3) * C + c;
            vst(o, old[r][0] + sc * g0); vst(o + C, old[r][1] + sc * g1); vst(o + 2 * C, old[r][2] + sc * g2);
        }
    }
}

inline unsigned grid_for(int64_t n) { return (unsigned)std::min<int64_t>((n + 255) / 256, 32768); }
inline unsigned grid_for(int64_t n, bool) { return grid_for(n); }

}

namespace abr {

static inline bool wide(int64_t tiles, int C) {
    return C % 4 == 0 && tiles * (C / 4) >= (int64_t)256 * 4 * 256;
}

int wino_input_transform(const float* x, int B, int H, int W, int C, float* V, hipStream_t st, const AmaxRef* amax) {
    const int th_n = (H + 3) / 4, tw_n = (W + 3) / 4;
    unsigned long long* aw = amax ? amax->word : nullptr;
    const unsigned ae = amax ? amax->epoch : 0u;
    wino_input_kernel<2><<<grid_for((int64_t)B * th_n * tw_n * (C / 2), aw != nullptr), 256, 0, st>>>(x, B, H, W, C, th_n, tw_n, V, aw, ae);
    return hipGetLastError() == hipSuccess ? 0 : 1;
}

void prep_wino_h3_direct(const PrepJobs& jobs, int pack_blocks, int scale_blocks, unsigned* flags, hipStream_t st) {
    if (!jobs.n) return;
    static std::once_flag attr_once;
    std::call_once(attr_once, [] {
        (void)hipFuncSetAttribute(reinterpret_cast<const void*>(wino_h3_pack_multi_kernel<PrepTable>), hipFuncAttributeMaxDynamicSharedMemorySize, (int)kWhLds);
        (void)hipFuncSetAttribute(reinterpret_cast<const void*>(wino_h3_pack_multi_kernel<PrepJob>), hipFuncAttributeMaxDynamicSharedMemorySize, (int)kWhLds);
    });
    prep_each(jobs, [&](auto src) {
        wino_h3_scales_multi_kernel<<<(unsigned)scale_blocks, 256, 0, st>>>(src, flags);
        wino_h3_pack_multi_kernel<<<(unsigned)pack_blocks, 256, kWhLds, st>>>(src);
    });
}

void prep_wino_u(const PrepJobs& jobs, int blocks, hipStream_t st) {
    prep_each(jobs, [&](auto src) { wino_weight_multi_kernel<<<(unsigned)blocks, 256, 0, st>>>(src); });
}

int wino_output_transform(const float* Mm, int B, int H, int W, int N, const float* scale, const float* bias, int relu, const float* mask,
                          float* out, hipStream_t st, const AmaxRef* amax) {
    const int th_n = (H + 3) / 4, tw_n = (W + 3) / 4;
    unsigned long long* aw = amax ? amax->word : nullptr;
    const unsigned ae = amax ? amax->epoch : 0u;
    if (wide((int64_t)B * th_n * tw_n, N))
        wino_output_kernel<4><<<grid_for((int64_t)B * th_n * tw_n * (N / 4), aw != nullptr), 256, 0, st>>>(Mm, B, H, W, N, th_n, tw_n, scale, bias, relu, mask, out, aw, ae);
    else
        wino_output_kernel<2><<<grid_for((int64_t)B * th_n * tw_n * (N / 2), aw != nullptr), 256, 0, st>>>(Mm, B, H, W, N, th_n, tw_n, scale, bias, relu, mask, out, aw, ae);
    return hipGetLastError() == hipSuccess ? 0 : 1;
}

int wino_outgrad_transform(const float* gy, int B, int H, int W, int N, float* Mg, hipStream_t st, const AmaxRef* amax) {
    const int th_n = (H + 3) / 4, tw_n = (W + 3) / 4;
    unsigned long long* aw = amax ? amax->word : nullptr;
    const unsigned ae = amax ? amax->epoch : 0u;
    if (wide((int64_t)B * th_n * tw_n, N)) wino_outgrad_kernel<4><<<grid_for((int64_t)B * th_n * tw_n * (N / 4), aw != nullptr), 256, 0, st>>>(gy, B, H, W, N, th_n, tw_n, Mg, aw, ae);
    else wino_outgrad_kernel<2><<<grid_for((int64_t)B * th_n * tw_n * (N / 2), aw != nullptr), 256, 0, st>>>(gy, B, H, W, N, th_n, tw_n, Mg, aw, ae);
    return hipGetLastError() == hipSuccess ? 0 : 1;
}

int wino_wgrad_inverse(const float* dU, int N, int C, const float* scale, float* dw, hipStream_t st) {
    if (C % 4 == 0) wino_wgrad_inverse_kernel<4><<<grid_for((int64_t)N * (C / 4)), 256, 0, st>>>(dU, N, C, scale, dw);
    else wino_wgrad_inverse_kernel<2><<<grid_for((int64_t)N * (C / 2)), 256, 0, st>>>(dU, N, C, scale, dw);
    return hipGetLastError() == hipSuccess ? 0 : 1;
}

namespace {
struct DEntry {
    void* buf = nullptr; size_t bytes = 0; int64_t version = 0; hipStream_t stream = nullptr; hipEvent_t filled = nullptr;
    std::vector<hipStream_t> readers;
    uint64_t last_use = 0;
    int64_t pending = 0;
};
std::map<std::pair<const void*, int>, DEntry> g_dcache;
std::mutex g_dcache_mu;
uint64_t g_dcache_clock = 0;
size_t g_dcache_bytes = 0;

void dcache_drop(DEntry& e) {
    if (e.stream) (void)hipStreamSynchronize(e.stream);
    for (hipStream_t r : e.readers) (void)hipStreamSynchronize(r);
    if (e.buf) { (void)hipFree(e.buf); g_dcache_bytes -= e.bytes; }
    if (e.filled) (void)hipEventDestroy(e.filled);
    e = DEntry();
}
size_t dcache_limit() {
    static const size_t mb = getenv("ABR_WINO_CACHE_MB") ? (size_t)atoll(getenv("ABR_WINO_CACHE_MB")) : 4096;
    return mb << 20;
}
}

static DEntry* dcache_acquire_locked(const void* w, int kind, size_t bytes, int64_t version, hipStream_t st, bool* needs_fill, std::vector<hipStream_t>* waited = nullptr) {
    DEntry& e = g_dcache[std::make_pair(w, kind)];
    e.last_use = ++g_dcache_clock;
    if (e.buf && e.bytes != bytes) dcache_drop(e);
    if (!e.buf) {
        while (g_dcache_bytes + bytes > dcache_limit()) {
            auto victim = g_dcache.end();
            for (auto it = g_dcache.begin(); it != g_dcache.end(); ++it)
                if (it->second.buf && &it->second != &e && !it->second.pending && (victim == g_dcache.end() || it->second.last_use < victim->second.last_use)) victim = it;
            if (victim == g_dcache.end()) break;
            dcache_drop(victim->second);
            g_dcache.erase(victim);
        }
        if (hipMalloc(&e.buf, bytes) != hipSuccess) { e.buf = nullptr; return nullptr; }
        e.bytes = bytes;
        g_dcache_bytes += bytes;
        e.last_use = g_dcache_clock;
        if (!e.filled) (void)hipEventCreateWithFlags(&e.filled, hipEventDisableTiming);
    }
    if (e.version == version && !e.pending) {
        if (st != e.stream && std::find(e.readers.begin(), e.readers.end(), st) == e.readers.end()) {
            (void)hipStreamWaitEvent(st, e.filled, 0);
            e.readers.push_back(st);
        }
        *needs_fill = false;
        return &e;
    }
    std::vector<hipStream_t> users = e.readers;
    if (e.stream && e.stream != st) users.push_back(e.stream);
    for (hipStream_t r : users) {
        if (r == st) continue;
        if (waited) {
            if (std::find(waited->begin(), waited->end(), r) != waited->end()) continue;
            waited->push_back(r);
        }
        hipEvent_t ev = nullptr;
        if (hipEventCreateWithFlags(&ev, hipEventDisableTiming) != hipSuccess) { (void)hipStreamSynchronize(r); continue; }
        (void)hipEventRecord(ev, r);
        (void)hipStreamWaitEvent(st, ev, 0);
        (void)hipEventDestroy(ev);
// ... 82 lines not shown
```

abr_iod_amd/modeling/backbone/resnet.py:

```python
import os
import threading
from collections import namedtuple

import torch
from torch import nn
from torch.autograd import Function

from ... import ops
from ...layers import FrozenBatchNorm2d
from ...layers._layout import as_nhwc, from_nhwc

StageSpec = namedtuple("StageSpec", ["index", "block_count", "return_features"])
ResNet50StagesTo4 = tuple(StageSpec(index=i, block_count=c, return_features=r) for (i, c, r) in ((1, 3, False), (2, 4, False), (3, 6, True)))
ResNet50StagesTo5 = tuple(StageSpec(index=i, block_count=c, return_features=r) for (i, c, r) in ((1, 3, False), (2, 4, False), (3, 6, False), (4, 3, True)))
ResNet101StagesTo4 = tuple(StageSpec(index=i, block_count=c, return_features=r) for (i, c, r) in ((1, 3, False), (2, 4, False), (3, 23, True)))
ResNet50FPNStagesTo5 = tuple(StageSpec(index=i, block_count=c, return_features=r) for (i, c, r) in ((1, 3, True), (2, 4, True), (3, 6, True), (4, 3, True)))
ResNet101FPNStagesTo5 = tuple(StageSpec(index=i, block_count=c, return_features=r) for (i, c, r) in ((1, 3, True), (2, 4, True), (3, 23, True), (4, 3, True)))
ResNet152FPNStagesTo5 = tuple(StageSpec(index=i, block_count=c, return_features=r) for (i, c, r) in ((1, 3, True), (2, 8, True), (3, 36, True), (4, 3, True)))

STAGE_SPECS = {"R-50-C4": ResNet50StagesTo4, "R-101-C4": ResNet101StagesTo4,
               "R-50-FPN": ResNet50FPNStagesTo5, "R-101-FPN": ResNet101FPNStagesTo5, "R-152-FPN": ResNet152FPNStagesTo5}
FPN_BODIES = ("R-50-FPN", "R-101-FPN", "R-152-FPN")


# ... 273 lines not shown
        self.stride = stride
        self.math = ops.MATH_F32

    def _conv(self, x, conv, stride, pad, **kw):
        return ops.conv_forward(x, conv.weight, stride, pad, math=self.math, w_version=conv.version(), **kw)

    def _dgrad(self, g, conv, scale, pad, **kw):
        return ops.conv_forward(g, conv.dgrad_weight(scale), 1, pad, math=self.math, w_version=conv.version(), **kw)

    def prep_entries(self):
        return [(conv, scale, conv.stride, conv.padding, self.math) for conv, scale in self._conv_scales()
                if conv.weight.requires_grad and conv.weight.is_cuda]

    def _conv_scales(self):
        if self.dcn:
            pairs = [(self.conv1, self.bn1), (self.conv2.offset, None), (self.conv2.conv, self.bn2), (self.conv3, self.bn3)]
        else:
            pairs = [(self.conv1, self.bn1), (self.conv2, self.bn2), (self.conv3, self.bn3)]
        if self.downsample is not None:
            pairs.append((self.downsample[0], self.downsample[1]))
        return [(conv, bn.scale_bias()[0] if bn is not None else None) for conv, bn in pairs]

    def fwd(self, x, save, stride=None):
        s = self.stride if stride is None else stride
        if self.dcn:
            return self._fwd_dcn(x, save, s)
        if (BLOCK_PLANS and ops.H3_TAGS and x.is_cuda and x.is_contiguous() and x.dtype == torch.float32
                and (save or not (self.math == ops.MATH_BF16X6 and self.conv2.weight.shape[0] == 64))):
            plans = self.__dict__.setdefault("_fwd_plans", {})
            keep_v = bool(save and ops.KEEP_WINO_V and self.conv2.weight.requires_grad)
            key = (x.shape, s, self.math, save, keep_v)
            plan = plans.get(key)
            if plan is None or not plan.valid():
                if len(plans) > 32:
                    plans.clear()
                plan = plans[key] = _FwdPlan(self, x.shape, s, save)
            return plan.run(x)
        s1, b1 = self.bn1.scale_bias()
        s2, b2 = self.bn2.scale_bias()
        s3, b3 = self.bn3.scale_bias()
        o1 = self._conv(x, self.conv1, s, 0, scale=s1, bias=b1, relu=True)
        v2 = ops.wino_v_alloc(o1, self.conv2.weight, 1, 1, self.math) if (save and self.conv2.weight.requires_grad) else None
        if self.downsample is not None:
            sd, bd = self.downsample[1].scale_bias()
            idt = self._conv(x, self.downsample[0], s, 0, scale=sd, bias=bd)
        else:
            idt = x
        if not save and ops.bottleneck_tail64_applies(o1, self.conv2.weight, self.conv3.weight, self.math):
            out = ops.bottleneck_tail64(o1, self.conv2.weight, self.conv3.weight, s2, b2, s3, b3, idt, self.conv2.version(), self.conv3.version())
            return out, None
        o2 = self._conv(o1, self.conv2, 1, 1, scale=s2, bias=b2, relu=True, wino_v=v2)
        out = self._conv(o2, self.conv3, 1, 0, scale=s3, bias=b3, residual=idt, relu=True)
        return out, ((x, o1, o2, out, s, v2) if save else None)

    def _fwd_dcn(self, x, save, s):
        s1, b1 = self.bn1.scale_bias()
        s2, b2 = self.bn2.scale_bias()
        s3, b3 = self.bn3.scale_bias()
        off, dc = self.conv2.offset, self.conv2.conv
        o1 = self._conv(x, self.conv1, s, 0, scale=s1, bias=b1, relu=True)
        if self.downsample is not None:
            sd, bd = self.downsample[1].scale_bias()
            idt = self._conv(x, self.downsample[0], s, 0, scale=sd, bias=bd)
        else:
            idt = x
        om = self._conv(o1, off, 1, 1, bias=off.bias)
        cols = ops.deform_im2col(o1, om, self.conv2.deformable_groups, self.conv2.modulated)
        o2 = self._conv(cols, dc, 1, 0, scale=s2, bias=b2, relu=True)
        out = self._conv(o2, self.conv3, 1, 0, scale=s3, bias=b3, residual=idt, relu=True)
        return out, ((x, o1, o2, out, s, om, cols) if save else None)

    def bwd(self, saved, gout, need_dx, g_owned, g_masked=False, mask_dx=None):
        if self.dcn:
            return self._bwd_dcn(saved, gout, need_dx, g_owned, g_masked, mask_dx)
        x, o1, o2, out, s, v2 = saved
        s1, _ = self.bn1.scale_bias()
        s2, _ = self.bn2.scale_bias()
        s3, _ = self.bn3.scale_bias()
        g = gout if g_masked else ops.relu_backward(gout, out, inplace=g_owned)
        if BLOCK_PLANS:
            return self._bwd_pairs(x, o1, o2, s, v2, g, need_dx, mask_dx, s1, s2, s3)
        ops.conv_wgrad_async(o2, g, _grad_buf(self.conv3.weight), 1, 0, scale=s3, math=self.math)
        g2 = self._dgrad(g, self.conv3, s3, 0, mask=o2)
        ops.conv_wgrad_async(o1, g2, _grad_buf(self.conv2.weight), 1, 1, scale=s2, math=self.math, wino_v=v2)
        g1 = self._dgrad(g2, self.conv2, s2, 1, mask=o1)
        ops.conv_wgrad_async(x, g1, _grad_buf(self.conv1.weight), s, 0, scale=s1, math=self.math)
        ds = self.downsample
        if ds is not None:
            sd, _ = ds[1].scale_bias()
            ops.conv_wgrad_async(x, g, _grad_buf(ds[0].weight), s, 0, scale=sd, math=self.math)
        if not need_dx:
            return None
        if s == 1:
            if ds is not None:
                gx = self._dgrad(g, ds[0], sd, 0)
                return self._dgrad(g1, self.conv1, s1, 0, residual=gx, out=gx, mask=mask_dx)
            return self._dgrad(g1, self.conv1, s1, 0, residual=g, mask=mask_dx)
        B, H, W, _ = x.shape
        assert mask_dx is None, "stride-2 blocks open a stage: their input is not a block output of the same stage"
        gx = self._dgrad(g1, self.conv1, s1, 0, out_hw=(H, W), out_stride=(s, s))
        if ds is not None:
            self._dgrad(g, ds[0], sd, 0, residual=gx, out=gx, out_hw=(H, W), out_stride=(s, s))
        return gx


def _bwd_pairs(self, x, o1, o2, s, v2, g, need_dx, mask_dx, s1, s2, s3):
    m = self.math
    c1, c2, c3 = self.conv1, self.conv2, self.conv3
    g2 = ops.conv_backward(o2, g, _grad_buf(c3.weight), c3.dgrad_weight(s3), 1, 0, scale=s3, math=m, w_version=c3.version(), mask=o2)
    g1 = ops.conv_backward(o1, g2, _grad_buf(c2.weight), c2.dgrad_weight(s2), 1, 1, scale=s2, math=m, w_version=c2.version(), wino_v=v2, mask=o1)
    return _bwd_head(self, x, g, g1, s, need_dx, mask_dx, s1)


def _bwd_dcn(self, saved, gout, need_dx, g_owned, g_masked=False, mask_dx=None):
    x, o1, o2, out, s, om, cols = saved
    s1, _ = self.bn1.scale_bias()
    s2, _ = self.bn2.scale_bias()
    s3, _ = self.bn3.scale_bias()
    m = self.math
    c3, off, dc = self.conv3, self.conv2.offset, self.conv2.conv
    g = gout if g_masked else ops.relu_backward(gout, out, inplace=g_owned)
    g2 = ops.conv_backward(o2, g, _grad_buf(c3.weight), c3.dgrad_weight(s3), 1, 0, scale=s3, math=m, w_version=c3.version(), mask=o2)
    dcol = ops.conv_backward(cols, g2, _grad_buf(dc.weight), dc.dgrad_weight(s2), 1, 0, scale=s2, math=m, w_version=dc.version())
    dx_part, d_om = ops.deform_col2im_coord(dcol, o1, om, self.conv2.deformable_groups, self.conv2.modulated)
    del dcol
    g1 = ops.conv_backward(o1, d_om, _grad_buf(off.weight), off.dgrad_weight(None), 1, 1, math=m, w_version=off.version(), residual=dx_part, mask=o1)
    ops.bias_grad(d_om, _grad_buf(off.bias))
    return _bwd_head(self, x, g, g1, s, need_dx, mask_dx, s1)


def _bwd_head(self, x, g, g1, s, need_dx, mask_dx, s1):
    m = self.math
    c1 = self.conv1
    ds = self.downsample
    sd = ds[1].scale_bias()[0] if ds is not None else None
    if not need_dx:
        ops.conv_backward(x, g1, _grad_buf(c1.weight), None, s, 0, scale=s1, math=m, dgrad=False)
        if ds is not None:
            ops.conv_backward(x, g, _grad_buf(ds[0].weight), None, s, 0, scale=sd, math=m, dgrad=False)
        return None
    if s == 1:
        if ds is not None:
            gx = ops.conv_backward(x, g, _grad_buf(ds[0].weight), ds[0].dgrad_weight(sd), s, 0, scale=sd, math=m, w_version=ds[0].version())
            return ops.conv_backward(x, g1, _grad_buf(c1.weight), c1.dgrad_weight(s1), s, 0, scale=s1, math=m, w_version=c1.version(),
                                     residual=gx, out=gx, mask=mask_dx)
        return ops.conv_backward(x, g1, _grad_buf(c1.weight), c1.dgrad_weight(s1), s, 0, scale=s1, math=m, w_version=c1.version(),
                                 residual=g, mask=mask_dx)
    B, H, W, _ = x.shape
    assert mask_dx is None, "stride-2 blocks open a stage: their input is not a block output of the same stage"
    gx = ops.conv_backward(x, g1, _grad_buf(c1.weight), c1.dgrad_weight(s1), s, 0, scale=s1, math=m, w_version=c1.version(),
                           out_hw=(H, W), out_stride=(s, s))
    if ds is not None:
        ops.conv_backward(x, g, _grad_buf(ds[0].weight), ds[0].dgrad_weight(sd), s, 0, scale=sd, math=m, w_version=ds[0].version(),
                          residual=gx, out=gx, out_hw=(H, W), out_stride=(s, s))
    return gx


Bottleneck._bwd_pairs = _bwd_pairs
Bottleneck._bwd_dcn = _bwd_dcn


class _StageFn(Function):

    @staticmethod
    def forward(ctx, x, blocks, first_stride, need_dx, *params):
        ctx.blocks, ctx.need_dx = blocks, need_dx
        ctx.saved = []
        save = True
# ... 209 lines not shown
```

abr_iod_amd/modeling/rpn/rpn.py:

```python
import math

import numpy as np
import os

import torch
from torch import nn
from torch.autograd import Function

from ... import ops
from ...layers._layout import as_nhwc, from_nhwc
from ...structures.bounding_box import BoxList
from ...structures.image_list import ImageList
from ..backbone.resnet import Conv2d, _grad_buf
from ..balanced_positive_negative_sampler import BalancedPositiveNegativeSampler
from ..box_coder import BoxCoder
from ..matcher import Matcher


def generate_anchors(stride=16, sizes=(32, 64, 128, 256, 512), aspect_ratios=(0.5, 1, 2)):
    base = float(stride)
    xc = yc = 0.5 * (base - 1)
    area = base * base
    out = []
    for r in aspect_ratios:
# ... 64 lines not shown
    def level_cell_anchors(self, level):
        return self.cell_anchors if level == 0 else getattr(self, "cell_anchors_%d" % level)

    def num_anchors_per_location(self):
        return [self.level_cell_anchors(l).shape[0] for l in range(len(self.strides))]

    def grid(self, H, W, image_hw, level=0):
        cell = self.level_cell_anchors(level)
        lv = (level,) if level else ()
        key = (H, W, int(image_hw[0]), int(image_hw[1]), cell.device) + lv
        hit = self._cache.get(key)
        if hit is None:
            a, vis = ops.grid_anchors(cell, H, W, self.strides[level], int(image_hw[0]), int(image_hw[1]), self.straddle_thresh)
            a = self._cache.setdefault((H, W, cell.device) + lv, a)
            hit = self._cache[key] = (a, vis, vis.bool())
        return hit

    def pyramid(self, grids, image_hw):
        grids = tuple((int(h), int(w)) for h, w in grids)
        assert len(grids) == len(self.strides), "one grid per anchor stride"
        dev = self.cell_anchors.device
        key = ("pyramid", grids, int(image_hw[0]), int(image_hw[1]), dev)
        hit = self._cache.get(key)
        if hit is None:
            per = [self.grid(H, W, image_hw, l) for l, (H, W) in enumerate(grids)]
            boxes = self._cache.get(("pyramid", grids, dev))
            if boxes is None:
                boxes = self._cache[("pyramid", grids, dev)] = torch.cat([p[0] for p in per])
            offs = [0]
            for p in per:
                offs.append(offs[-1] + p[0].shape[0])
            hit = self._cache[key] = (boxes, torch.cat([p[1] for p in per]), tuple(offs))
        return hit

    def forward(self, image_list, feature_maps):
        assert len(feature_maps) == len(self.strides), "one feature map per anchor stride"
        grids = [f.shape[-2:] for f in feature_maps]
        anchors = []
        for (ih, iw) in image_list.image_sizes:
            per_level = []
            for l, (H, W) in enumerate(grids):
                a, vis, vis_bool = self.grid(H, W, (ih, iw), l)
                bl = BoxList(a, (iw, ih), mode="xyxy")
                bl.add_field("visibility", vis_bool)
                bl._visibility_u8 = vis
                per_level.append(bl)
            if len(grids) > 1:
                per_level[0]._pyramid = self.pyramid(grids, (ih, iw))
            anchors.append(per_level)
        return anchors


def make_anchor_generator(cfg):
    sizes, strides = cfg.MODEL.RPN.ANCHOR_SIZES, cfg.MODEL.RPN.ANCHOR_STRIDE
    if cfg.MODEL.RPN.USE_FPN:
        assert len(strides) == len(sizes), "FPN should have len(ANCHOR_STRIDE) == len(ANCHOR_SIZES)"
    else:
        assert len(strides) == 1, "Non-FPN should have a single ANCHOR_STRIDE"
    return AnchorGenerator(sizes, cfg.MODEL.RPN.ASPECT_RATIOS, strides, cfg.MODEL.RPN.STRADDLE_THRESH)


class _RPNHeadFn(Function):

    @staticmethod
    def forward(ctx, x, head, *params):
        xh = as_nhwc(x)
        v = ops.wino_v_alloc(xh, head.conv.weight, 1, 1, head.math) if head.conv.weight.requires_grad else None
        t = ops.conv_forward(xh, head.conv.weight, 1, 1, bias=head.conv.bias, relu=True, math=head.math, wino_v=v, w_version=head.conv.version())
        y = ops.conv_forward(t, head.fused_weight, 1, 0, bias=head.fused_bias, math=head.math, w_version=head.fused_version())
        ctx.head, ctx.saved = head, (xh, t, v)
        ctx.need_dx = x.requires_grad
        return from_nhwc(y)

    @staticmethod
    def backward(ctx, gy):
        head = ctx.head
        xh, t, v = ctx.saved
        g = as_nhwc(gy)
        if not g.is_contiguous():
            g = g.contiguous()
        ops.conv_wgrad_async(t, g, head.fused_weight_grad, 1, 0, math=head.math)
        ops.bias_grad(g, head.fused_bias_grad)
        gt = ops.conv_forward(g, head.fused_dgrad_weight(), 1, 0, mask=t, math=head.math)
        ops.conv_wgrad_async(xh, gt, _grad_buf(head.conv.weight), 1, 1, math=head.math, wino_v=v)
        ops.bias_grad(gt, _grad_buf(head.conv.bias))
        gx = from_nhwc(ops.conv_forward(gt, head.conv.dgrad_weight(), 1, 1, math=head.math, w_version=head.conv.version())) if ctx.need_dx else None
        ctx.saved = None
        return (gx, None) + (None,) * (len(ctx.needs_input_grad) - 2)


class RPNHead(nn.Module):

    def __init__(self, cfg, in_channels, num_anchors):
        super().__init__()
        self.num_anchors = num_anchors
        self.math = ops.MATH_F32
        self.conv = Conv2d(in_channels, in_channels, 3, stride=1, padding=1)
        self.cls_logits = Conv2d(in_channels, num_anchors, 1)
        self.bbox_pred = Conv2d(in_channels, num_anchors * 4, 1)
        for l in (self.conv, self.cls_logits, self.bbox_pred):
            nn.init.normal_(l.weight, std=0.01)
            nn.init.constant_(l.bias, 0)
        if cfg.MODEL.RPN.CONV_FREEZE:
            for p in self.conv.parameters():
                p.requires_grad = False
        if cfg.MODEL.RPN.CLS_FREEZE:
            for p in self.cls_logits.parameters():
                p.requires_grad = False
        if cfg.MODEL.RPN.BBS_FREEZE:
            for p in self.bbox_pred.parameters():
                p.requires_grad = False
        self.n_out = num_anchors * 5
        self.n_out_pad = (self.n_out + 3) // 4 * 4
        self._fuse()

    def _fuse(self):
        A, C_, dev = self.num_anchors, self.conv.in_channels, self.cls_logits.weight.device
        fw = torch.zeros(self.n_out_pad, 1, 1, C_, device=dev)
        fb = torch.zeros(self.n_out_pad, device=dev)
        with torch.no_grad():
            fw[:A].copy_(self.cls_logits.weight)
            fw[A:5 * A].copy_(self.bbox_pred.weight)
            fb[:A].copy_(self.cls_logits.bias)
            fb[A:5 * A].copy_(self.bbox_pred.bias)
        self._set_fused(fw, fb, torch.zeros_like(fw), torch.zeros_like(fb))

    def _set_fused(self, fw, fb, gw, gb):
        A = self.num_anchors
        self.fused_weight, self.fused_bias = fw, fb
        self.fused_weight_grad, self.fused_bias_grad = gw, gb
        for mod, lo, hi in ((self.cls_logits, 0, A), (self.bbox_pred, A, 5 * A)):
            mod.weight.data, mod.bias.data = fw[lo:hi], fb[lo:hi]
            mod.weight.grad, mod.bias.grad = gw[lo:hi], gb[lo:hi]
        self._wt, self._wt_version = None, -1

    def rehome(self, which, view, grad_view):
        if which == "weight":
            shp = self.fused_weight.shape
            self._set_fused(view.view(shp), self.fused_bias, grad_view.view(shp), self.fused_bias_grad)
        else:
            self._set_fused(self.fused_weight, view, self.fused_weight_grad, grad_view)

    def _apply(self, fn, *a, **k):
        out = super()._apply(fn, *a, **k)
        self._fuse()
        return out

    def flat_groups(self):
        return [("weight", [self.cls_logits.weight, self.bbox_pred.weight], self.n_out_pad - self.n_out),
                ("bias", [self.cls_logits.bias, self.bbox_pred.bias], self.n_out_pad - self.n_out)]

    def prep_entries(self):
        return [(self.conv, None, 1, 1, self.math)] if (self.conv.weight.requires_grad and self.conv.weight.is_cuda) else []

    def prepare_rest(self):
        if self.fused_weight.is_cuda and self.fused_weight_grad is not None and (self.cls_logits.weight.requires_grad or self.bbox_pred.weight.requires_grad):
            self.fused_dgrad_weight()
            ops.conv_prepare_weights(self.fused_weight, 1, 0, self.math, self.fused_version())

    def fused_version(self):
        from ..backbone.resnet import _PARAM_VERSION, _STATIC_VERSION
        opt = self.cls_logits._optimised or self.bbox_pred._optimised
        return 2 * _PARAM_VERSION[0] + 1 if opt else 2 * _STATIC_VERSION[0] + 2

    def fused_dgrad_weight(self):
        from ..backbone.resnet import _PARAM_VERSION
        ops.prep_wait()
        if self._wt is None or self._wt_version != _PARAM_VERSION[0]:
            self._wt = ops.conv_dgrad_weights(self.fused_weight, None, out=self._wt)
# ... 436 lines not shown
```

abr_iod_amd/ops.py:

```python
import ctypes as C
import os
import threading

import torch

from . import _lib as L

_f32 = torch.float32


def _empty(shape, like, dtype=_f32):
    return torch.empty(shape, dtype=dtype, device=like.device)


def _cached_workspace(cache, nbytes, device, floor):
    key = (device, L.stream())
    ws = cache.get(key)
    if ws is None or ws.numel() < nbytes:
        ws = cache[key] = torch.empty((max(nbytes, floor),), dtype=torch.uint8, device=device)
    return ws


def roi_align_forward(feat, rois, spatial_scale, ph, pw, sampling_ratio, bin_step=1, out=None):
    L.require_cuda(feat, rois)
# ... 446 lines not shown
            try:
                c = next(_amax_block["it"])
            except StopIteration:
                base, first = C.c_void_p(0), C.c_uint64(0)
                L.check(L.lib().abr_h3_amax_alloc_block(_AMAX_BLOCK, C.byref(base), C.byref(first)), "h3_amax_alloc_block")
                _amax_block["base"] = int(base.value)
                it = iter(range(int(first.value), int(first.value) + _AMAX_BLOCK))
                c = next(it)
                _amax_block["it"] = it
    _amax_count[0] += 1
    return _amax_block["base"] + (c % _AMAX_RING) * 8, (c + 1) & 0xFFFFFFFF


def amax_tag(t, word, epoch, stream=None):
    t._abr_amax = (word, epoch, t.data_ptr(), t._version, _amax_count[0], stream)
    return t


def amax_of(t):
    tag = getattr(t, "_abr_amax", None)
    if (tag is not None and tag[2] == t.data_ptr() and tag[3] == t._version and _amax_count[0] - tag[4] < _AMAX_RING // 4
            and (tag[5] is None or tag[5] == L.stream())):
        return tag[0], tag[1]
    return None, 0


def amax_carry(dst, src):
    tag = getattr(src, "_abr_amax", None)
    if tag is not None and tag[2] == dst.data_ptr() and dst.numel() == src.numel():
        dst._abr_amax = (tag[0], tag[1], tag[2], dst._version, tag[4], tag[5])
    return dst


def amax_carry_bound(dst, src):
    w, e = amax_of(src)
    if w is not None:
        dst._abr_amax = (w, e, dst.data_ptr(), dst._version, src._abr_amax[4], src._abr_amax[5])
    return dst


def amax_drop(t):
    if getattr(t, "_abr_amax", None) is not None:
        t._abr_amax = None
    if getattr(t, "_abr_scatter", None) is not None:
        t._abr_scatter = None
    return t


def amax_compute(t):
    t = L.f32c(t)
    w, e = amax_new()
    st = L.stream()
    L.check(L.lib().abr_h3_amax(L.ptr(t), t.numel(), w, e, st), "h3_amax")
    amax_reductions[0] += 1
    amax_reductions[1] += t.numel() * 4
    return amax_tag(t, w, e, st)


def amax_bound_levels(dst, srcs):
    if not H3_TAGS or not 1 <= len(srcs) <= MAX_PYRAMID_LEVELS:
        return dst
    refs = [amax_of(s) for s in srcs]
    if any(w is None for w, _ in refs):
        return dst
    streams = {s._abr_amax[5] for s in srcs} - {None}
    st = L.stream()
    if streams - {st}:
        return dst
    n = len(refs)
    words = (C.c_void_p * n)(*[w for w, _ in refs])
    epochs = (C.c_uint32 * n)(*[e for _, e in refs])
    w, e = amax_new()
    L.check(L.lib().abr_h3_amax_max(C.cast(words, C.c_void_p), C.cast(epochs, C.c_void_p), n, w, e, st), "h3_amax_max")
    return amax_tag(dst, w, e, st if streams else None)


def amax_operand(t, reduce=True):
    w, e = amax_of(t)
    if w is None and reduce and H3_TAGS:
        w, e = amax_of(amax_compute(t))
    return w, e


def amax_wgrad_operands(x, gy, wino_v=None):
    return amax_operand(x, reduce=wino_v is None), amax_operand(gy)


def conv_out_emits(out, residual, sh, sw, emit_amax, math):
    if emit_amax is None:
        emit_amax = uses_amax(math)
    if not (emit_amax and H3_TAGS):
        return False
    if out is None:
        return True
    if out is not residual:
        return False
    return (sh == 1 and sw == 1) or getattr(out, "_abr_scatter", None) == (out.data_ptr(), sh, sw)


def conv_out_done(out, fresh, word, epoch, sh=1, sw=1):
    if word is not None:
        amax_tag(out, word, epoch)
    elif not fresh:
        amax_drop(out)
    if fresh and (sh != 1 or sw != 1):
        out._abr_scatter = (out.data_ptr(), sh, sw)
    return out


def _conv_result(d, scattered, device):
    return (torch.zeros if scattered else torch.empty)((d.B, d.out_H, d.out_W, d.Cout), dtype=_f32, device=device)


def h3_range_stats(reset=True):
    import ctypes
    v = (ctypes.c_uint64 * 2)(0, 0)
    L.check(L.lib().abr_h3_range_stats(ctypes.cast(v, ctypes.c_void_p), int(bool(reset)), L.stream()), "h3_range_stats")
    return int(v[0]), int(v[1])


def x6_range_flags(reset=True):
    import ctypes
    v = ctypes.c_uint32(0)
    L.check(L.lib().abr_x6_range_flags(ctypes.cast(ctypes.pointer(v), ctypes.c_void_p), int(bool(reset)), L.stream()), "x6_range_flags")
    return int(v.value)


class X6RangeWatch(object):

    def __init__(self):
        self._host = torch.zeros(1, dtype=torch.int32).pin_memory()
        self._dev = None
        self._event = None

    def poll(self, reduce_over_ranks=False):
        seen = 0
        if self._event is not None and reduce_over_ranks:
            self._event.synchronize()
        if self._event is not None and self._event.query():
            seen = int(self._host[0].item()) & 0xFFFFFFFF
            self._event = None
        if self._event is None:
            if reduce_over_ranks:
                import torch.distributed as dist
                if self._dev is None:
                    self._dev = torch.zeros(1, dtype=torch.int32, device="cuda")
                L.check(L.lib().abr_x6_range_flags_to_device(self._dev.data_ptr(), L.stream()), "x6_range_flags_to_device")
                dist.all_reduce(self._dev, op=dist.ReduceOp.MAX)
                self._host.copy_(self._dev, non_blocking=True)
            else:
                L.check(L.lib().abr_x6_range_flags_async(self._host.data_ptr(), L.stream()), "x6_range_flags_async")
            self._event = torch.cuda.Event()
            self._event.record()
        return seen

    def reset(self):
        x6_range_flags(reset=True)
        self._event = None
        self._host.zero_()

    def poll_h3_stats(self, reduce_over_ranks=False):
        seen = None
        ev = getattr(self, "_h3_event", None)
        if ev is not None and reduce_over_ranks:
            ev.synchronize()
        if ev is not None and ev.query():
            seen = (int(self._h3_host[0].item()), int(self._h3_host[1].item()))
            self._h3_event = ev = None
        if ev is None:
            if getattr(self, "_h3_dev", None) is None:
                self._h3_dev = torch.zeros(2, dtype=torch.int64, device="cuda")
                self._h3_host = torch.zeros(2, dtype=torch.int64).pin_memory()
            L.check(L.lib().abr_h3_range_stats_to_device(self._h3_dev.data_ptr(), 1, L.stream()), "h3_range_stats_to_device")
            if reduce_over_ranks:
                import torch.distributed as dist
                dist.all_reduce(self._h3_dev, op=dist.ReduceOp.SUM)
            self._h3_host.copy_(self._h3_dev, non_blocking=True)
            self._h3_event = torch.cuda.Event()
            self._h3_event.record()
        return seen


_desc_templates = {}


def conv_desc(x_shape, w_shape, stride, pad, scale=None, bias=None, residual=None, mask=None, relu=False,
              out_hw=None, out_stride=(1, 1), math=MATH_F32):
    key = (x_shape, w_shape, stride, pad, relu, out_hw, out_stride, math)
    tmpl = _desc_templates.get(key)
    if tmpl is None:
        B, H, W, Cin = x_shape
        Cout, R, S, Cin2 = w_shape
        if Cin != Cin2:
            raise RuntimeError(f"conv: input has {Cin} channels, weight expects {Cin2}")
        Ho = (H + 2 * pad - R) // stride + 1
        Wo = (W + 2 * pad - S) // stride + 1
        d = L.ConvDesc()
        d.B, d.H, d.W, d.Cin, d.Cout, d.R, d.S = B, H, W, Cin, Cout, R, S
        d.stride, d.pad, d.Ho, d.Wo = stride, pad, Ho, Wo
        d.relu = int(relu)
        if out_hw is None:
            d.out_H, d.out_W, d.out_sh, d.out_sw = Ho, Wo, 1, 1
        else:
            d.out_H, d.out_W = out_hw
            d.out_sh, d.out_sw = out_stride
        d.math = int(math)
        if len(_desc_templates) > 8192:
            _desc_templates.clear()
        tmpl = _desc_templates[key] = bytes(d)
    d = L.ConvDesc.from_buffer_copy(tmpl)
    if scale is not None:
        d.scale = scale.data_ptr()
    if bias is not None:
        d.bias = bias.data_ptr()
    if residual is not None:
        d.residual = residual.data_ptr()
    if mask is not None:
        d.mask = mask.data_ptr()
    return d


def conv_route_info(x_shape, w_shape, stride, pad, scale=None, bias=None, residual=None, mask=None, relu=False,
                    out_hw=None, out_stride=(1, 1), math=MATH_F32):
    d = conv_desc(tuple(x_shape), tuple(w_shape), stride, pad, scale, bias, residual, mask, relu, out_hw, out_stride, math)
    out = (C.c_int32 * 4)()
    L.check(L.lib().abr_conv_route_info(C.byref(d), out), "conv_route_info")
    return int(out[0]), bool(out[1]), bool(out[2]), int(out[3])


KEEP_WINO_V = os.environ.get("ABR_WINOGRAD_KEEP_V", "1") != "0"


def wino_v_alloc(x, w, stride, pad, math=MATH_F32):
    if not KEEP_WINO_V:
        return None
    d = conv_desc(x.shape, w.shape, stride, pad, math=math)
    n = int(L.lib().abr_conv_wino_v_floats(C.byref(d)))
    return torch.empty(n, dtype=_f32, device=x.device) if n > 0 else None


def conv_forward(x, w, stride=1, pad=0, scale=None, bias=None, residual=None, mask=None, relu=False,
                 out=None, out_hw=None, out_stride=(1, 1), math=MATH_F32, wino_v=None, w_planes=None, w_version=0, emit_amax=None):
    L.require_cuda(x, w)
    xc, w = L.f32c(x), L.f32c(w)
    d = conv_desc(xc.shape, w.shape, stride, pad, scale, bias, residual, mask, relu, out_hw, out_stride, math)
    d.wino_v = L.ptr(wino_v)
    d.w_planes = L.ptr(w_planes)
    d.w_version = int(w_version)
    if uses_amax(math):
        d.x_amax, d.x_amax_epoch = amax_operand(xc)
    fresh = out is None
    ow, oe = amax_new() if conv_out_emits(out, residual, d.out_sh, d.out_sw, emit_amax, math) else (None, 0)
    d.out_amax, d.out_amax_epoch = ow, oe
    if fresh:
        out = _conv_result(d, out_hw is not None, x.device)
    L.check(L.lib().abr_conv_forward(C.byref(d), L.ptr(xc), L.ptr(w), L.ptr(out), L.stream()), "conv_forward")
    return conv_out_done(out, fresh, ow, oe, d.out_sh, d.out_sw)


STEP_MARKS = os.environ.get("ABR_STEP_MARKS", "0") != "0"
_marks = []


def mark(name):
    if STEP_MARKS and torch.cuda.is_available():
        ev = torch.cuda.Event(enable_timing=True)
        ev.record()
        _marks.append((name, ev))


def take_marks():
    torch.cuda.synchronize()
    out = [(n, _marks[0][1].elapsed_time(e)) for n, e in _marks] if _marks else []
    del _marks[:]
    return out


def bottleneck_tail64_applies(o1, w2, w3, math):
    return (math == MATH_BF16X6 and tuple(w2.shape) == (64, 3, 3, 64) and tuple(w3.shape) == (256, 1, 1, 64)
            and o1.shape[-1] == 64 and o1.numel() * 4 * 4 < 0x7FFFFFF0)


def bottleneck_tail64(o1, w2, w3, scale2, bias2, scale3, bias3, residual, w2_version, w3_version, out=None):
    L.require_cuda(o1, w2, w3)
    o1, w2, w3 = L.f32c(o1), L.f32c(w2), L.f32c(w3)
    d2 = conv_desc(o1.shape, w2.shape, 1, 1, scale2, bias2, None, None, True, math=MATH_BF16X6)
    B, H, W, _ = o1.shape
    d3 = conv_desc((B, H, W, 64), w3.shape, 1, 0, scale3, bias3, residual, None, True, math=MATH_BF16X6)
    d2.w_version, d3.w_version = int(w2_version), int(w3_version)
    if out is None:
        out = _empty((B, H, W, 256), o1)
    L.check(L.lib().abr_conv_tail64_forward(C.byref(d2), C.byref(d3), L.ptr(o1), L.ptr(w2), L.ptr(w3), L.ptr(out), L.stream()), "conv_tail64_forward")
    return out


def conv_prepare_weights(w, stride, pad, math, w_version):
    Cout, R, S, Cin = w.shape
    L.check(L.lib().abr_conv_prepare_weights(L.ptr(w), Cout, R, S, Cin, stride, pad, int(math), int(w_version), L.stream()), "conv_prepare_weights")


def conv_prepare_batch(entries):
    if not entries:
        return
    arr = (L.PrepItem * len(entries))()
    keep = []
    for a, (w, scale, wt, stride, pad, math, ver) in zip(arr, entries):
        Cout, R, S, Cin = w.shape
        if scale is not None:
            scale = L.f32c(scale)
            keep.append(scale)
        a.w, a.scale, a.wt = L.ptr(w), L.ptr(scale), L.ptr(wt)
        a.Cout, a.R, a.S, a.Cin, a.stride, a.pad, a.math, a.w_version = Cout, R, S, Cin, int(stride), int(pad), int(math), int(ver)
    L.check(L.lib().abr_conv_prepare_batch(C.cast(arr, C.c_void_p), len(entries), L.stream()), "conv_prepare_batch")


class PreparedBatch(object):

    def __init__(self, entries):
        self.n = len(entries)
        self.arr = (L.PrepItem * max(self.n, 1))()
        self.keep, self.vers, self.sig_src = [], [], []
        for a, (w, scale, wt, stride, pad, math, ver) in zip(self.arr, entries):
            Cout, R, S, Cin = w.shape
            if scale is not None:
                scale = L.f32c(scale)
            self.keep.append((w, scale, wt))
            a.w, a.scale, a.wt = L.ptr(w), L.ptr(scale), L.ptr(wt)
            a.Cout, a.R, a.S, a.Cin, a.stride, a.pad, a.math = Cout, R, S, Cin, int(stride), int(pad), int(math)
            self.vers.append(ver)
        self.ptr = C.cast(self.arr, C.c_void_p)

    def run(self):
        if not self.n:
            return
        for a, ver in zip(self.arr, self.vers):
            a.w_version = int(ver())
        L.check(L.lib().abr_conv_prepare_batch(self.ptr, self.n, L.stream()), "conv_prepare_batch")


def conv_cache_clear():
    L.check(L.lib().abr_conv_cache_clear(), "conv_cache_clear")


def conv_cache_drop_range(base, nbytes):
    L.check(L.lib().abr_conv_cache_drop_range(int(base), int(nbytes)), "conv_cache_drop_range")


def conv_cache_bytes():
    return int(L.lib().abr_conv_cache_bytes())


def scratch_bytes():
    return int(L.lib().abr_scratch_bytes())


def conv_wgrad(x, gy, dw, stride=1, pad=0, scale=None, math=MATH_F32, wino_v=None, amax_refs=None, stream=None):
    L.require_cuda(x, gy, dw)
    xc, gyc = L.f32c(x), L.f32c(gy)
    d = conv_desc(xc.shape, dw.shape, stride, pad, scale=scale, math=math)
    d.wino_v = L.ptr(wino_v)
    if uses_amax(math):
        (d.x_amax, d.x_amax_epoch), (d.gy_amax, d.gy_amax_epoch) = amax_refs or amax_wgrad_operands(xc, gyc, wino_v)
    L.check(L.lib().abr_conv_wgrad(C.byref(d), L.ptr(xc), L.ptr(gyc), L.ptr(dw), L.stream() if stream is None else stream), "conv_wgrad")
    return dw


WGRAD_SIDE_STREAM = os.environ.get("ABR_WGRAD_STREAM", "1") != "0"
_side_streams = {}
_join_pending = [False]


def h2d(values, dtype, device):
    t = torch.tensor(values, dtype=dtype)
    if torch.device(device).type != "cuda":
        return t.to(device)
    return t.pin_memory().to(device, non_blocking=True)


_prep = {"event": None, "waited": set()}


def prep_done(stream):
    ev = torch.cuda.Event()
    ev.record(stream)
    _prep["event"], _prep["waited"] = ev, set()


def prep_wait():
    ev = _prep["event"]
    if ev is not None:
        raw = L.stream()
        if raw not in _prep["waited"]:
            torch.cuda.current_stream().wait_event(ev)
            _prep["waited"].add(raw)


def side_stream(key):
    s = _side_streams.get(key)
    if s is None:
        s = _side_streams[key] = torch.cuda.Stream(device=key[0] if isinstance(key, tuple) else key)
    return s


def mark_overlap(on):
    L.lib().abr_prof_mark_overlap(1 if on else 0)


WGRAD_STREAMS = max(1, int(os.environ.get("ABR_WGRAD_STREAMS", "2")))
_wg_owner = {}
_wg_keep = {}
_wg_lock = threading.Lock()


def _wg_hold(main, item):
    lst = _wg_keep.get(main)
    if lst is None:
        with _wg_lock:
            lst = _wg_keep.setdefault(main, [])
    lst.append(item)


_wgrad_keys = {}


def _wgrad_stream(dev, i):
    key = _wgrad_keys.get((dev, i))
    if key is None:
        key = _wgrad_keys[(dev, i)] = dev if i == 0 else (dev, "wgrad%d" % i)
    return side_stream(key)


def _wgrad_owner(dw):
    owner = _wg_owner.get(dw.data_ptr())
    if owner is None:
        owner = _wg_owner[dw.data_ptr()] = len(_wg_owner) % WGRAD_STREAMS
    return owner


def _arm_join():
    if not _join_pending[0]:
        _join_pending[0] = True
        L.lib().abr_prof_mark_overlap(1)
        torch.autograd.Variable._execution_engine.queue_callback(join_side_stream)


def join_side_stream():
    if _join_pending[0]:
        L.lib().abr_prof_mark_overlap(0)
    _join_pending[0] = False
    if torch.cuda.is_available():
        dev = torch.cuda.current_device()
        for i in range(WGRAD_STREAMS):
            s = _side_streams.get(dev if i == 0 else (dev, "wgrad%d" % i))
            if s is not None:
                torch.cuda.current_stream().wait_stream(s)
    lst = _wg_keep.get(L.stream()) if torch.cuda.is_available() else None
    if lst:
        del lst[:]


def conv_wgrad_async(x, gy, dw, stride=1, pad=0, scale=None, math=MATH_F32, wino_v=None):
    if not WGRAD_SIDE_STREAM:
        return conv_wgrad(x, gy, dw, stride, pad, scale, math, wino_v)
    side = _wgrad_stream(x.device.index, _wgrad_owner(dw))
    _arm_join()
    x, gy = L.f32c(x), L.f32c(gy)
    refs = amax_wgrad_operands(x, gy, wino_v) if uses_amax(math) else None
    raw = side.cuda_stream
    main = L.stream()
    L.check(L.lib().abr_stream_wait_stream(raw, main), "stream_wait_stream")
    conv_wgrad(x, gy, dw, stride, pad, scale, math, wino_v, amax_refs=refs, stream=raw)
    _wg_hold(main, (x, gy, wino_v))
    return dw


_bwd_plans = {}


def conv_backward(x, gy, dw, wt, stride, pad, scale=None, math=MATH_F32, w_version=0, wino_v=None, dgrad=True, mask=None, residual=None,
                  out=None, out_hw=None, out_stride=(1, 1)):
    if not (WGRAD_SIDE_STREAM and H3_TAGS and x.is_contiguous() and gy.is_contiguous() and x.dtype == _f32 and gy.dtype == _f32):
        conv_wgrad_async(x, gy, dw, stride, pad, scale=scale, math=math, wino_v=wino_v)
        if not dgrad:
            return None
        return conv_forward(gy, wt, 1, dw.shape[1] - 1 - pad, mask=mask, residual=residual, out=out, out_hw=out_hw, out_stride=out_stride,
                            math=math, w_version=w_version)
    key = (dw.data_ptr(), x.shape, gy.shape, stride, pad, math, dgrad, out_hw, out_stride, wino_v is not None)
    plan = _bwd_plans.get(key)
    wtp = wt.data_ptr() if dgrad else 0
    scp = scale.data_ptr() if scale is not None else 0
    if plan is None or plan[2] != wtp or plan[3] != scp:
        if len(_bwd_plans) > 4096:
            _bwd_plans.clear()
        arr = (L.ConvOp * 3)()
        arr[0].kind = L.OP_STREAM_WAIT
        arr[1].kind = L.OP_WGRAD
        arr[1].desc = conv_desc(x.shape, dw.shape, stride, pad, scale=scale, math=math)
        arr[1].out = dw.data_ptr()
        if dgrad:
            arr[2].kind = L.OP_FORWARD
            arr[2].desc = conv_desc(gy.shape, wt.shape, 1, dw.shape[1] - 1 - pad, out_hw=out_hw, out_stride=out_stride, math=math)
            arr[2].b = wtp
        plan = _bwd_plans[key] = (arr, C.cast(arr, C.c_void_p), wtp, scp, _wgrad_owner(dw), (scale, dw), threading.Lock())
    arr, ptr, _, _, owner, _, lock = plan
    with lock:
        return _conv_backward_run(arr, ptr, owner, x, gy, dw, math, wino_v, dgrad, mask, residual, out, out_hw, w_version)


def _conv_backward_run(arr, ptr, owner, x, gy, dw, math, wino_v, dgrad, mask, residual, out, out_hw, w_version):
    side = _wgrad_stream(x.device.index, owner).cuda_stream
    _arm_join()
    main = L.stream()
    h3 = uses_amax(math)
    xp, gp = x.data_ptr(), gy.data_ptr()
    a0, a1 = arr[0], arr[1]
    a0.stream, a0.other = side, main
    a1.a, a1.b, a1.stream = xp, gp, side
    d1 = a1.desc
    d1.wino_v = wino_v.data_ptr() if wino_v is not None else None
    if h3:
        (d1.x_amax, d1.x_amax_epoch), (gw, ge) = amax_wgrad_operands(x, gy, wino_v)
        d1.gy_amax, d1.gy_amax_epoch = gw, ge
    if dgrad:
        a2 = arr[2]
        d2 = a2.desc
        fresh = out is None
        ow, oe = amax_new() if conv_out_emits(out, residual, d2.out_sh, d2.out_sw, None, math) else (None, 0)
        if h3:
            d2.x_amax, d2.x_amax_epoch, d2.out_amax, d2.out_amax_epoch = gw, ge, ow, oe
        if fresh:
            out = _conv_result(d2, out_hw is not None, x.device)
        a2.a, a2.out, a2.stream = gp, out.data_ptr(), main
        d2.residual = residual.data_ptr() if residual is not None else None
        d2.mask = mask.data_ptr() if mask is not None else None
        d2.w_version = int(w_version)
    L.check(L.lib().abr_conv_run(ptr, 3 if dgrad else 2), "conv_run (conv backward)")
    if dgrad:
        conv_out_done(out, fresh, ow, oe, d2.out_sh, d2.out_sw)
    _wg_hold(main, (x, gy, wino_v))
    return out if dgrad else None


def pack_weights(w, out=None):
    L.require_cuda(w)
    w = L.f32c(w)
    rows, K = w.shape[0], w.numel() // w.shape[0]
    n = int(L.lib().abr_conv_packed_bytes(rows, K))
    if n <= 0:
        raise RuntimeError("pack_weights: K = {} is not a positive multiple of 16".format(K))
    if out is None:
        out = torch.empty(n, dtype=torch.uint8, device=w.device)
    L.check(L.lib().abr_conv_pack_weights(L.ptr(w), rows, K, L.ptr(out), L.stream()), "conv_pack_weights")
    return out


def conv_dgrad_weights(w, scale=None, out=None):
    w = L.f32c(w)
    Cout, R, S, Cin = w.shape
    if out is None:
        out = _empty((Cin, R, S, Cout), w)
    L.check(L.lib().abr_conv_dgrad_weights(L.ptr(w), L.ptr(scale), Cout, R, S, Cin, L.ptr(out), L.stream()), "dgrad_weights")
    return out


def bias_grad(gy, db):
    gy = L.f32c(gy)
    Ch = gy.shape[-1]
    L.check(L.lib().abr_bias_grad(L.ptr(gy), gy.numel() // Ch, Ch, L.ptr(db), L.stream()), "bias_grad")
    return db


def deform_im2col(x, om, dg=1, modulated=False):
    L.require_cuda(x, om)
    x, om = L.f32c(x), L.f32c(om)
    B, H, W, Ch = x.shape
    if tuple(om.shape[:3]) != (B, H, W):
        raise RuntimeError(f"deform_im2col: offsets {tuple(om.shape)} do not match x {tuple(x.shape)}")
    cols = _empty((B, H, W, 9 * Ch), x)
    L.check(L.lib().abr_deform_im2col(L.ptr(x), L.ptr(om), B, H, W, Ch, om.shape[3], int(dg), int(bool(modulated)), L.ptr(cols), L.stream()),
            "deform_im2col")
    return amax_carry_bound(cols, x)


def deform_col2im_coord(dcol, x, om, dg=1, modulated=False):
    L.require_cuda(dcol, x, om)
    dcol, x, om = L.f32c(dcol), L.f32c(x), L.f32c(om)
    B, H, W, Ch = x.shape
    if tuple(dcol.shape) != (B, H, W, 9 * Ch) or tuple(om.shape[:3]) != (B, H, W):
        raise RuntimeError(f"deform_col2im_coord: dcol {tuple(dcol.shape)} / offsets {tuple(om.shape)} do not match x {tuple(x.shape)}")
    dx = torch.zeros_like(x)
    d_om = _empty(tuple(om.shape), om)
    w, e = amax_new() if H3_TAGS else (None, 0)
    L.check(L.lib().abr_deform_col2im_coord(L.ptr(dcol), L.ptr(x), L.ptr(om), B, H, W, Ch, om.shape[3], int(dg), int(bool(modulated)),
                                            L.ptr(dx), L.ptr(d_om), w, e, L.stream()), "deform_col2im_coord")
    if w is not None:
        amax_tag(d_om, w, e)
    return dx, d_om


def deform_out_size(H, W, kernel, stride, padding, dilation):
    return tuple((n + 2 * p - (d * (k - 1) + 1)) // s + 1 for n, k, s, p, d in zip((H, W), kernel, stride, padding, dilation))


def _deform_general_args(name, x, offset, mask, kernel, stride, padding, dilation, groups, dg):
    B, H, W, Ch = x.shape
    K = kernel[0] * kernel[1]
    Ho, Wo = offset.shape[1], offset.shape[2]
    if tuple(offset.shape) != (B, Ho, Wo, dg * 2 * K):
        raise RuntimeError(f"{name}: offset {tuple(offset.shape)} is not [{B}, Ho, Wo, {dg * 2 * K}]")
    if mask is not None and tuple(mask.shape) != (B, Ho, Wo, dg * K):
        raise RuntimeError(f"{name}: mask {tuple(mask.shape)} is not [{B}, {Ho}, {Wo}, {dg * K}]")
    return (B, H, W, Ch, Ho, Wo, kernel[0], kernel[1], stride[0], stride[1], padding[0], padding[1], dilation[0], dilation[1], int(groups), int(dg))


def deform_im2col_general(x, offset, mask=None, kernel=(3, 3), stride=(1, 1), padding=(1, 1), dilation=(1, 1), groups=1, dg=1):
    L.require_cuda(x, offset, mask)
    x, offset = L.f32c(x), L.f32c(offset)
    mask = None if mask is None else L.f32c(mask)
    a = _deform_general_args("deform_im2col_general", x, offset, mask, kernel, stride, padding, dilation, groups, dg)
    B, Ch, Ho, Wo, K = a[0], a[3], a[4], a[5], a[6] * a[7]
    cols = _empty((int(groups), B * Ho * Wo, K * (Ch // int(groups))), x)
    L.check(L.lib().abr_deform_im2col_general(L.ptr(x), L.ptr(offset), L.ptr(mask), *a, L.ptr(cols), L.stream()), "deform_im2col_general")
# ... 1282 lines not shown
```

include/abr_iod_hip.h:

```cpp
#ifndef ABR_IOD_HIP_H
#define ABR_IOD_HIP_H

#include <stdint.h>

#ifdef __cplusplus
extern "C" {
#endif

#define ABR_OK 0
#define ABR_E_INVALID (-1)
#define ABR_E_LAUNCH (-2)
#define ABR_E_WORKSPACE (-3)

#define ABR_NCHW 0
#define ABR_NHWC 1

const char* abr_last_error(void);
int abr_version(void);
int abr_device_info(int32_t* out_host);

int abr_prof_begin(void);
int abr_prof_mark_overlap(int on);
int abr_stream_wait_stream(void* waiter, void* signaller);
int abr_prof_set_mask(uint32_t id_mask, int every_nth);
// ... 70 lines not shown
                             int W, float spatial_scale, int output_dim, int group_size, int pooled_size, int part_size, int sample_per_part,
                             float trans_std, int num_classes, int layout, float* out, float* top_count, void* stream);

int abr_deform_psroi_backward(const float* out_grad, const float* feat, const float* rois, const float* trans, const float* mask_logits,
                              const float* top_count, int K, int B, int C, int H, int W, float spatial_scale, int output_dim, int group_size,
                              int pooled_size, int part_size, int sample_per_part, float trans_std, int num_classes, int layout,
                              float* grad_feat, float* grad_trans, float* grad_mask_logits, void* stream);

int64_t abr_nms_workspace_bytes(int N, int n_max);
int abr_nms_sorted_batched(const float* boxes, const int32_t* counts, int N, int n_max, float thr,
                           int strict_gt, int max_keep, int32_t* keep, int32_t* n_keep,
                           void* workspace, int64_t workspace_bytes, void* stream);

int64_t abr_nms_unsorted_workspace_bytes(int n);
int abr_nms(const float* dets, const float* scores, int n, float thr, int strict_gt, int64_t* keep_out, int32_t* n_keep_out, void* workspace,
            int64_t workspace_bytes, void* stream);
int64_t abr_sort_scores_max_n(void);
int abr_sort_scores_desc(const float* scores, int n, int64_t* order, void* stream);

int abr_sigmoid_focal_forward(const float* logits, const int32_t* targets, int N, int C, float gamma,
                              float alpha, float* losses, void* stream);
int abr_sigmoid_focal_backward(const float* logits, const int32_t* targets, const float* d_losses, int N,
                               int C, float gamma, float alpha, float* d_logits, void* stream);
int abr_sigmoid_focal_forward_f64(const double* logits, const int32_t* targets, int N, int C, float gamma, float alpha, double* losses, void* stream);
int abr_sigmoid_focal_backward_f64(const double* logits, const int32_t* targets, const double* d_losses, int N, int C, float gamma, float alpha,
                                   double* d_logits, void* stream);


int abr_ard_forward(const float* f_src, const float* f_tgt, int N, int C, int HW, float gamma, int layout,
                    float* coef, float* loss_out, void* stream);
int abr_ard_backward(const float* f_src, const float* f_tgt, const float* coef, int N, int C, int HW,
                     float gamma, int layout, float gscale, const float* gscale_dev, float* grad_tgt,
                     void* stream);

int abr_smooth_l1(const float* x, const float* t, int64_t n, float beta, float scale, float* loss_out,
                  float gscale, float* grad, void* stream);
int abr_smooth_l1_rows(const float* x, int x_cols, const float* t, const int64_t* rows, const int64_t* col0,
                       const int64_t* trows , int n_rows, float beta, float scale,
                       const float* denom_dev ,
                       float* loss_out, float gscale, float* grad, void* stream);

int abr_softmax_ce(const float* logits, int ld_logits , const int64_t* labels, int n, int K,
                   int inclusive, int n_old, float* loss_out, float gscale, float* d_logits, int ld_dlogits,
                   void* stream);

int abr_feat_distill(const float* src, const float* tgt, int64_t n, float* loss_out, float* stats3, float gscale, float* d_tgt,
                     void* stream);
int abr_rpn_distill(const float* obj_s, const float* reg_s, int ld_obj_s, int ld_reg_s, const float* obj_t, const float* reg_t,
                    int ld_obj_t, int ld_reg_t, int64_t rows, int A, float bbox_threshold, int use_bbox, float* loss_out,
                    float gscale, float* d_obj_t, float* d_reg_t, int ld_d_obj, int ld_d_reg, void* stream);

int abr_roi_distill(const float* z_s, const float* b_s, const float* z_t, const float* b_t, int n, int K_old,
                    int K_all, const int32_t* ld_host, int dist_id, float* loss_out, float gscale, float* d_zt,
                    float* d_bt, void* stream);

int abr_bce_logits_gather(const float* x, const float* y, const int64_t* idx, const int64_t* yidx ,
                          int n_idx, const float* denom_dev ,
                          float* loss_out, float gscale, float* grad, void* stream);

#define ABR_MATH_F32 0
#define ABR_MATH_BF16 1
#define ABR_MATH_BF16X6 2
#define ABR_MATH_F16X3 3
#define ABR_MATH_F16 4

typedef struct {
    int B, H, W, Cin;
    int Cout, R, S;
    int stride, pad;
    int Ho, Wo;
    const float* scale;
    const float* bias;
    const float* residual;
    const float* mask;
    int relu;
    int out_H, out_W, out_sh, out_sw;
    int math;
    float* wino_v;
    const void* w_planes;
    int64_t w_version;
    const uint64_t* x_amax;   uint32_t x_amax_epoch;
    const uint64_t* gy_amax;  uint32_t gy_amax_epoch;
    uint64_t* out_amax;       uint32_t out_amax_epoch;
} abr_conv_desc;

#define ABR_H3_AMAX_RING 65536
int abr_h3_amax_alloc(uint64_t** word_out, uint32_t* epoch_out);
int abr_h3_amax_alloc_block(int n, uint64_t** ring_base_out, uint64_t* first_count_out);
int abr_h3_range_stats(uint64_t* out_host, int reset, void* stream);
int abr_h3_range_stats_to_device(uint64_t* out_device, int reset, void* stream);
int abr_h3_amax(const float* x, int64_t n, uint64_t* word, uint32_t epoch, void* stream);
int abr_h3_amax_max(const uint64_t* const* words_host, const uint32_t* epochs_host, int L, uint64_t* out_word, uint32_t out_epoch, void* stream);

int abr_conv_forward(const abr_conv_desc* d_host, const float* x, const float* w, float* out, void* stream);
int abr_conv_tail64_forward(const abr_conv_desc* d2_host, const abr_conv_desc* d3_host, const float* x, const float* w2, const float* w3, float* out,
                            void* stream);
int abr_conv_prepare_weights(const float* w, int Cout, int R, int S, int Cin, int stride, int pad, int math, int64_t w_version, void* stream);
typedef struct abr_prep_item {
    const float* w;
    const float* scale;
    float* wt;
    int32_t Cout, R, S, Cin, stride, pad, math;
    int64_t w_version;
} abr_prep_item;
int abr_conv_prepare_batch(const abr_prep_item* items_host, int n, void* stream);

#define ABR_OP_FORWARD 0
#define ABR_OP_WGRAD 1
#define ABR_OP_STREAM_WAIT 2
typedef struct abr_conv_op {
    int32_t kind;
    int32_t reserved;
    abr_conv_desc desc;
    const float* a;
    const float* b;
    float* out;
    void* stream;
    void* other;
} abr_conv_op;
int abr_conv_run(const abr_conv_op* ops, int n);
int abr_conv_cache_clear(void);
int abr_conv_cache_drop_range(const void* base, int64_t bytes);
int64_t abr_conv_cache_bytes(void);
int64_t abr_scratch_bytes(void);
int64_t abr_conv_wino_v_floats(const abr_conv_desc* d_host);
int abr_conv_route_info(const abr_conv_desc* d_host, int32_t out[4]);
int64_t abr_conv_packed_bytes(int64_t rows, int64_t K);
int abr_conv_pack_weights(const float* w, int64_t rows, int K, void* planes, void* stream);

int abr_conv_wgrad(const abr_conv_desc* d_host, const float* x, const float* gy, float* dw, void* stream);

int abr_conv_dgrad_weights(const float* w, const float* scale, int Cout, int R, int S, int Cin, float* wt,
                           void* stream);
int abr_bias_grad(const float* gy, int64_t M, int C, float* db, void* stream);

int abr_nchw_to_nhwc_pad(const float* x, int B, int C, int H, int W, int Cpad, float* out, void* stream);
int abr_nhwc_to_nchw(const float* x, int B, int C, int H, int W, float* out, void* stream);
int abr_nchw_to_nhwc(const float* x, int B, int C, int H, int W, float* out, void* stream);
int abr_maxpool3x3s2(const float* x, int B, int H, int W, int C, float* out, void* stream);
int abr_maxpool3x3s2_backward(const float* y, const float* g_pool, int B, int H, int W, int C, float* g_y, void* stream);
int abr_deform_im2col(const float* x, const float* om, int B, int H, int W, int C, int Com, int dg, int modulated, float* cols, void* stream);
int abr_deform_col2im_coord(const float* dcol, const float* x, const float* om, int B, int H, int W, int C, int Com, int dg, int modulated,
                            float* dx, float* d_om, uint64_t* d_om_amax, uint32_t d_om_amax_epoch, void* stream);
int abr_deform_im2col_general(const float* x, const float* offset, const float* mask, int B, int H, int W, int C, int Ho, int Wo, int kh, int kw,
                              int stride_h, int stride_w, int pad_h, int pad_w, int dil_h, int dil_w, int groups, int dg, float* cols,
                              void* stream);
int abr_deform_col2im_coord_general(const float* dcol, const float* x, const float* offset, const float* mask, int B, int H, int W, int C, int Ho,
                                    int Wo, int kh, int kw, int stride_h, int stride_w, int pad_h, int pad_w, int dil_h, int dil_w, int groups,
                                    int dg, float* dx, float* d_offset, float* d_mask, void* stream);
int abr_avgpool_forward(const float* x, int N, int HW, int C, float* out, void* stream);
int abr_avgpool_backward(const float* g, int N, int HW, int C, float* gx, void* stream);
int abr_avgpool_relu_backward(const float* g, const float* y, int N, int HW, int C, float* gx, void* stream);
int abr_avgpool_relu_backward_amax(const float* g, const float* y, int N, int HW, int C, float* gx, uint64_t* amax, uint32_t amax_epoch, void* stream);
int abr_channel_mean(const float* x, int64_t rows, int C, float* out, void* stream);
int abr_relu_backward(const float* g, const float* y, int64_t n, float* out, void* stream);
int abr_add_inplace(float* a, const float* b, int64_t n, void* stream);
int abr_loss_sum(const float* const* terms_host, const float* weights_host, const int32_t* groups_host, int n, float* total, float* out,
                 void* stream);
int abr_loss_sum_backward(const float* weights_host, int n, const float* g, float* grads, void* stream);
int abr_scale_inplace(float* x, int64_t n, float s, const float* s_dev, void* stream);

int abr_grid_anchors(const float* cell, int A, int H, int W, int stride, int img_h, int img_w, int straddle,
                     float* out, uint8_t* vis, void* stream);
int abr_topk_sigmoid(const float* logits, int64_t img_stride, int N, int n, int A, int ld, int k, float* scores,
                     int64_t* idx, void* stream);
int abr_det_softmax_decode(const float* logits, int ld_logits, const float* deltas, int ld_deltas, int delta_col0,
                           int agnostic_col, const float* rois, int K, int C, const int32_t* img_hw, float wx, float wy,
                           float ww, float wh, float* prob, float* boxes, void* stream);
int64_t abr_det_select_workspace_bytes(int N, int C, int r_max);
int abr_det_select(const float* prob, const float* boxes, const int32_t* row_offsets, int N, int C, int r_max,
                   float score_thresh, float nms_thresh, int detections_per_img, int cap, float* out_boxes,
                   float* out_scores, int64_t* out_labels, int32_t* out_count, float* bg_boxes, float* bg_scores,
                   int32_t* bg_count, void* workspace, int64_t workspace_bytes, void* stream);
int abr_rpn_decode_clip(const float* reg, int reg_stride, int reg_col0, int A, const float* anchors,
                        const int64_t* idx, int N, int n_anchor, int k, const int32_t* img_hw, float wx,
                        float wy, float ww, float wh, float* out, void* stream);
int abr_rpn_pyramid_max_k(void);
int abr_rpn_pyramid_topk(const float* const* y_host, const int* nloc_host, const int* A_host, const int* ld_host, int L, int N, int pre_nms_top_n,
                         int k_max, float* scores, int64_t* idx, void* stream);
int abr_rpn_pyramid_decode(const float* const* y_host, const int* nloc_host, const int* A_host, const int* ld_host, const float* const* anchors_host,
                           int L, int N, int pre_nms_top_n, int k_max, const int64_t* idx, const float* scores_in, const int32_t* img_hw, float wx,
                           float wy, float ww, float wh, float min_size, float* props, float* scores_out, int32_t* counts, void* stream);
int abr_rpn_pyramid_select(const float* props, const float* scores, const int32_t* keep, const int32_t* n_keep, int N, int L, int k_max, int post,
                           int fpn_post_n, int mode, float* rois, float* out_scores, int32_t* src, int32_t* n_out, void* stream);
int abr_rpn_pyramid_loss(const float* const* y_host, const int* nloc_host, int L, int N, int A, int Cf, const float* labels,
                         const float* reg_targets, const int64_t* pos, int max_pos, const int64_t* neg, int batch, const int32_t* counts,
                         float* losses, int64_t* rec_dst, float* rec_val, void* stream);
int abr_rpn_pyramid_loss_backward(const int* nloc_host, int L, int N, int A, int Cf, const int64_t* rec_dst, const float* rec_val, int max_pos,
                                  int batch, const float* g_obj, const float* g_box, float* grad, void* stream);
int abr_box_encode(const float* gt, const float* ex, int n, float wx, float wy, float ww, float wh, float* out,
                   void* stream);
int abr_match_encode(const float* boxes, int n, const float* gt, const int64_t* gt_labels, int G,
                     const uint8_t* vis, float hi, float lo, int allow_low_quality, float wx, float wy,
                     float ww, float wh, int64_t* matched, float* labels_f32, int64_t* labels_i64,
                     float* reg_targets, void* workspace, int64_t workspace_bytes, void* stream);
int64_t abr_match_workspace_bytes(int n, int G);

int abr_sample_pos_neg(const void* labels, int labels_are_int64, int N, int n, int64_t stride, int batch_size,
                       int max_pos, uint64_t seed, int first_image, int64_t index_offset_per_image,
                       int64_t* pos_idx, int64_t* neg_idx, int32_t* counts, void* stream);

int abr_roi_head_targets(const float* props, const int32_t* keep, const int32_t* n_keep, int N, int k_pre, int post,
                         const float* const* gt_ptrs, const int64_t* const* gt_label_ptrs, const int32_t* n_gt, int g_max, float hi,
                         float lo, float wx, float wy, float ww, float wh, int batch_size, int max_pos, uint64_t seed, float* cand,
                         int64_t* labels_all, float* regt_all, int32_t* n_cand, int64_t* pos_idx, int64_t* neg_idx, int32_t* counts,
                         float* rois, int64_t* labels, float* reg_targets, int64_t* sampled_idx, float* n_valid, const float* scores,
                         float* obj_all, float* obj, int64_t* pos_rows, int64_t* col0, int num_classes, int cls_agnostic, void* stream);
int abr_roi_head_targets_table(const float* rois_in, const float* scores, const int32_t* n_out, int N, int cap,
// ... 106 lines not shown
```

Baseline: 229.0.

## Share Winograd output-gradient transform between wgrad and dgrad for 3x3 convs

For stride-1 3x3 convs whose wgrad and dgrad both take the Winograd path, the output-gradient transform Mg is computed once on the main stream. It is then reused by the weight-gradient GEMM (on the side stream) and by the data-gradient convolution, which now runs as an adjoint Winograd product with tap-reversed cached weights followed by a new input-gradient inverse transform. This removes one input transform and one transform workspace per backward conv. In exchange it allocates an extra Mg buffer per call and adds a new transform kernel and weight-cache variant, and it moves the transform onto the main stream before the stream split.

```diff
diff --git a/abr_iod_amd/_lib.py b/abr_iod_amd/_lib.py
--- a/abr_iod_amd/_lib.py
+++ b/abr_iod_amd/_lib.py
@@ -28,6 +28,7 @@
         ("x_amax", _vp), ("x_amax_epoch", C.c_uint32),
         ("gy_amax", _vp), ("gy_amax_epoch", C.c_uint32),
         ("out_amax", _vp), ("out_amax_epoch", C.c_uint32),
+        ("wino_mg", _vp),
     ]
 
 
@@ -36,7 +37,7 @@
     _fields_ = [("kind", C.c_int32), ("reserved", C.c_int32), ("desc", ConvDesc), ("a", _vp), ("b", _vp), ("out", _vp), ("stream", _vp), ("other", _vp)]
 
 
-OP_FORWARD, OP_WGRAD, OP_STREAM_WAIT = 0, 1, 2
+OP_FORWARD, OP_WGRAD, OP_STREAM_WAIT, OP_WINO_OUTGRAD = 0, 1, 2, 3
 
 
 class PrepItem(C.Structure):
@@ -133,6 +134,8 @@
     "abr_conv_tail64_forward": (_i, [C.POINTER(ConvDesc), C.POINTER(ConvDesc), _vp, _vp, _vp, _vp, _vp]),
     "abr_conv_wgrad": (_i, [C.POINTER(ConvDesc), _vp, _vp, _vp, _vp]),
     "abr_conv_wino_v_floats": (_i64, [C.POINTER(ConvDesc)]),
+    "abr_conv_wino_mg_floats": (_i64, [C.POINTER(ConvDesc)]),
+    "abr_conv_wino_outgrad": (_i, [C.POINTER(ConvDesc), _vp, _vp]),
     "abr_conv_route_info": (_i, [C.POINTER(ConvDesc), C.POINTER(C.c_int32)]),
     "abr_conv_packed_bytes": (_i64, [_i64, _i64]),
     "abr_conv_pack_weights": (_i, [_vp, _i64, _i, _vp, _vp]),
diff --git a/abr_iod_amd/csrc/common.h b/abr_iod_amd/csrc/common.h
--- a/abr_iod_amd/csrc/common.h
+++ b/abr_iod_amd/csrc/common.h
@@ -125,12 +125,14 @@
 int wino_output_transform(const float* M, int B, int H, int W, int N, const float* scale, const float* bias, int relu, const float* mask,
                           float* out, hipStream_t st, const AmaxRef* amax = nullptr);
 int wino_outgrad_transform(const float* gy, int B, int H, int W, int N, float* Mg, hipStream_t st, const AmaxRef* amax = nullptr);
+int wino_ingrad_transform(const float* dV, int B, int H, int W, int C, const float* mask, float* out, hipStream_t st, const AmaxRef* amax = nullptr);
 int wino_wgrad_inverse(const float* dU, int N, int C, const float* scale, float* dw, hipStream_t st);
 ScratchPool& scratch_pool();
 inline void* scratch(ScratchSlot slot, hipStream_t st, size_t bytes, size_t zero_prefix = 0) { return scratch_pool().scratch(slot, st, bytes, zero_prefix); }
 inline float* wino_ws(hipStream_t st, size_t floats) { return static_cast<float*>(scratch(SCRATCH_WINO, st, floats * sizeof(float))); }
 int num_cus();
-enum DerivedKind { DERIVED_NONE = -1, DERIVED_WINO_U = 0, DERIVED_X6_PLANES = 1, DERIVED_WINO_U_X6_PLANES = 2, DERIVED_H3_PLANES = 3, DERIVED_WINO_U_H3_PLANES = 4 };
+enum DerivedKind { DERIVED_NONE = -1, DERIVED_WINO_U = 0, DERIVED_X6_PLANES = 1, DERIVED_WINO_U_X6_PLANES = 2, DERIVED_H3_PLANES = 3, DERIVED_WINO_U_H3_PLANES = 4,
+                   DERIVED_TAPS_REVERSED = 8 };
 void* derived_cached(const void* w, int kind, size_t bytes, int64_t version, hipStream_t st, const std::function<int(void*)>& fill);
 void* derived_acquire(const void* w, int kind, size_t bytes, int64_t version, hipStream_t st, void** token, std::vector<hipStream_t>* waited = nullptr);
 void derived_commit(void* const* tokens, int n, hipStream_t st);
@@ -148,6 +150,7 @@
     size_t bytes;
 };
 ConvRoute conv_route(const abr_conv_desc& d);
+bool conv_dgrad_adjoint(const abr_conv_desc& d);
 
 struct PrepJob {
     const float* src;
@@ -156,6 +159,7 @@
     int a, b, c;
     int gx, gy;
     int first_block;
+    int taps;
 };
 struct PrepTable { const PrepJob* jobs; int njobs; };
 template <int PrepJob::*F = &PrepJob::first_block>
diff --git a/abr_iod_amd/csrc/conv_igemm.hip b/abr_iod_amd/csrc/conv_igemm.hip
--- a/abr_iod_amd/csrc/conv_igemm.hip
+++ b/abr_iod_amd/csrc/conv_igemm.hip
@@ -1257,9 +1257,22 @@
     r.bytes = r.kind == DERIVED_NONE ? 0 : (size_t)(r.kind == DERIVED_WINO_U ? r.rows * r.K * 4 : (h3 ? h3_packed_bytes(r.rows, r.K) : x6_packed_bytes(r.rows, r.K)));
     return r;
 }
-}
-
-static bool wino_split_kind(int kind) { return kind == abr::DERIVED_WINO_U_X6_PLANES || kind == abr::DERIVED_WINO_U_H3_PLANES; }
+
+bool conv_dgrad_adjoint(const abr_conv_desc& d) {
+    abr_conv_desc f = d;
+    f.residual = nullptr; f.out_H = f.out_W = 0; f.out_sh = f.out_sw = 1;
+    const ConvRoute rf = conv_route(f);
+    if (!(rf.fwd_wino && rf.wgrad_wino) || d.math == ABR_MATH_BF16 || d.math == ABR_MATH_F16) return false;
+    abr_conv_desc g = f;
+    g.Cin = d.Cout; g.Cout = d.Cin;
+    return conv_route(g).fwd_wino;
+}
+}
+
+static bool wino_split_kind(int kind) {
+    kind &= ~abr::DERIVED_TAPS_REVERSED;
+    return kind == abr::DERIVED_WINO_U_X6_PLANES || kind == abr::DERIVED_WINO_U_H3_PLANES;
+}
 
 namespace {
 constexpr size_t kPrepRing = 8192;
@@ -1317,7 +1330,7 @@
         abr::PrepJob& j = add(h3 ? PREP_H3 : PREP_X6, m, dst, (int)rows, K, gx, gy, gx * gy);
         if (h3) { j.c = scale_blocks[PREP_H3]; scale_blocks[PREP_H3] += gy * 8; }
     }
-    void derived(const abr::ConvRoute& r, const float* w, void* dst) {
+    void derived(const abr::ConvRoute& r, const float* w, void* dst, int taps = 0) {
         if (r.kind == abr::DERIVED_NONE) return;
         const bool h3 = r.kind == abr::DERIVED_H3_PLANES || r.kind == abr::DERIVED_WINO_U_H3_PLANES;
         if (r.kind == abr::DERIVED_H3_PLANES || r.kind == abr::DERIVED_X6_PLANES) return pack(h3, w, r.rows, r.K, dst);
@@ -1325,12 +1338,13 @@
         if (h3 && C % 64 == 0) {
             abr::PrepJob& j = add(PREP_WINO_H3, w, dst, N, C, C / 64, N / 32, (C / 64) * (N / 32));
             j.c = scale_blocks[PREP_WINO_H3];
+            j.taps = taps;
             scale_blocks[PREP_WINO_H3] += N / 4;
             return;
         }
         const int gx = (int)(((int64_t)N * (C / 4) + 255) / 256);
         const bool via = r.kind != abr::DERIVED_WINO_U;
-        add(PREP_WINO_U, w, via ? nullptr : dst, N, C, gx, 1, gx);
+        add(PREP_WINO_U, w, via ? nullptr : dst, N, C, gx, 1, gx).taps = taps;
         if (!via) return;
         const int pk = h3 ? PREP_H3 : PREP_X6;
         via_u.push_back({jobs[PREP_WINO_U].size() - 1, jobs[pk].size(), pk, u_floats});
@@ -1380,44 +1394,51 @@
 }
 }
 
-static const void* cached_weights(const abr::ConvRoute& r, const float* w, int64_t version, hipStream_t st) {
+static const void* cached_weights(const abr::ConvRoute& r, const float* w, int64_t version, hipStream_t st, int taps = 0) {
     if (!version) return nullptr;
-    return abr::derived_cached(w, r.kind, r.bytes, version, st, [&](void* buf) {
+    return abr::derived_cached(w, r.kind | (taps ? abr::DERIVED_TAPS_REVERSED : 0), r.bytes, version, st, [&](void* buf) {
         PrepPlan p;
-        p.derived(r, w, buf);
+        p.derived(r, w, buf, taps);
         return prep_launch(p, p.u_floats ? abr::wino_ws(st, p.u_floats) : nullptr, st) || hipGetLastError() != hipSuccess;
     });
 }
 
-static const void* conv_weights(const abr::ConvRoute& r, const float* w, int64_t version, hipStream_t st, size_t own = 0, float** ws = nullptr) {
-    const void* cached = cached_weights(r, w, version, st);
+static const void* conv_weights(const abr::ConvRoute& r, const float* w, int64_t version, hipStream_t st, size_t own = 0, float** ws = nullptr,
+                                int taps = 0) {
+    const void* cached = cached_weights(r, w, version, st, taps);
     const size_t mine = cached ? 0 : r.bytes / 4 + (wino_split_kind(r.kind) ? (size_t)r.rows * r.K : 0);
     float* s = own + mine ? abr::wino_ws(st, own + mine) : nullptr;
     if (ws) *ws = s;
     if (cached || !s) return cached;
     float* buf = s + own;
     PrepPlan p;
-    p.derived(r, w, buf);
+    p.derived(r, w, buf, taps);
     return prep_launch(p, buf + r.bytes / 4, st) || hipGetLastError() != hipSuccess ? nullptr : buf;
 }
 
-static bool wino_conv(const ConvP& p, const abr::ConvRoute& r, const float* x, const float* w, float* out, hipStream_t st) {
+static bool wino_conv(const ConvP& p, const abr::ConvRoute& r, const float* x, const float* w, float* out, hipStream_t st, float* mg = nullptr) {
     const int th_n = (p.H + 3) / 4, tw_n = (p.W + 3) / 4;
     const int64_t T = (int64_t)p.B * th_n * tw_n;
-    const size_t nV = p.v_out ? 0 : (size_t)36 * T * p.Cin, nM = (size_t)36 * T * p.Cout;
+    const size_t nV = p.v_out || mg ? 0 : (size_t)36 * T * p.Cin, nM = (size_t)36 * T * p.Cout;
     float* ws = nullptr;
-    const void* U = conv_weights(r, w, p.w_version, st, nV + nM, &ws);
+    const void* U = conv_weights(r, w, p.w_version, st, nV + nM, &ws, mg ? 1 : 0);
     if (!U || !ws) return false;
-    float* V = p.v_out ? p.v_out : ws;
+    float* V = mg ? mg : (p.v_out ? p.v_out : ws);
     float* Mm = ws + nV;
     const bool h3 = p.math == ABR_MATH_F16X3, x6 = p.math == ABR_MATH_BF16X6;
     abr::AmaxRef v_ref{nullptr, 0};
-    if (h3) {
+    if (h3 && mg) {
+        v_ref = abr::h3_amax_recall(mg);
+        if (!v_ref.word) {
+            v_ref = abr::h3_amax_alloc();
+            if (!v_ref.word || abr::h3_amax_reduce(mg, (int64_t)36 * T * p.Cin, v_ref, st)) return false;
+        }
+    } else if (h3) {
         v_ref = abr::h3_amax_alloc();
         if (!v_ref.word) return false;
         if (p.v_out) abr::h3_amax_remember(p.v_out, v_ref);
     }
-    if (abr::wino_input_transform(x, p.B, p.H, p.W, p.Cin, V, st, h3 ? &v_ref : nullptr)) return false;
+    if (!mg && abr::wino_input_transform(x, p.B, p.H, p.W, p.Cin, V, st, h3 ? &v_ref : nullptr)) return false;
     ConvP g = p;
     g.B = (int)T; g.H = g.W = 1; g.R = g.S = 1; g.stride = 1; g.pad = 0; g.Ho = g.Wo = 1;
     g.M = (int)T; g.K = p.Cin;
@@ -1438,10 +1459,33 @@
     if (h3 || x6) dispatch_igemm_x6(g, V, nullptr, Mm, st);
     else dispatch_igemm(g, V, static_cast<const float*>(U), Mm, st);
     const abr::AmaxRef o_ref{p.out_amax, p.out_epoch};
+    if (mg) return abr::wino_ingrad_transform(Mm, p.B, p.H, p.W, p.Cout, p.mask, out, st, p.out_amax ? &o_ref : nullptr) == 0;
     return abr::wino_output_transform(Mm, p.B, p.H, p.W, p.Cout, p.scale, p.bias, p.relu, p.mask, out, st, p.out_amax ? &o_ref : nullptr) == 0;
 }
 
 extern "C" int64_t abr_conv_wino_v_floats(const abr_conv_desc* d) { return d ? abr::conv_route(*d).v_floats : 0; }
+
+extern "C" int64_t abr_conv_wino_mg_floats(const abr_conv_desc* d) {
+    if (!d || !abr::conv_dgrad_adjoint(*d)) return 0;
+    return (int64_t)36 * d->B * ((d->H + 3) / 4) * ((d->W + 3) / 4) * d->Cout;
+}
+
+extern "C" int abr_conv_wino_outgrad(const abr_conv_desc* d, const float* gy, void* stream) {
+    ABR_REQUIRE(d && gy && d->wino_mg, "conv_wino_outgrad: null pointer");
+    ABR_REQUIRE(d->B > 0 && d->H > 0 && d->W > 0 && d->Ho == d->H && d->Wo == d->W && abr::conv_route(*d).wgrad_wino,
+                "conv_wino_outgrad: the conv's weight gradient does not take the Winograd path");
+    hipStream_t st = abr::as_stream(stream);
+    abr::AmaxRef ref{nullptr, 0};
+    const bool h3 = d->math == ABR_MATH_F16X3;
+    if (h3) {
+        ref = abr::h3_amax_alloc();
+        ABR_REQUIRE(ref.word, "conv_wino_outgrad: no amax word");
+        abr::h3_amax_remember(d->wino_mg, ref);
+    }
+    ABR_REQUIRE(abr::wino_outgrad_transform(gy, d->B, d->H, d->W, d->Cout, d->wino_mg, st, h3 ? &ref : nullptr) == 0, "conv_wino_outgrad: launch failed");
+    ABR_CHECK_LAUNCH("conv_wino_outgrad");
+    return ABR_OK;
+}
 
 extern "C" int abr_conv_route_info(const abr_conv_desc* d, int32_t out[4]) {
     ABR_REQUIRE(d && out, "conv_route_info: null pointer");
@@ -1490,9 +1534,13 @@
     p.a_amax = nullptr; p.a_epoch = 0; p.w_scales = nullptr;
     p.out_amax = reinterpret_cast<unsigned long long*>(d->out_amax); p.out_epoch = d->out_amax_epoch;
     const bool h3 = p.math == ABR_MATH_F16X3 || p.math == ABR_MATH_F16;
+    if (d->wino_mg) {
+        ABR_REQUIRE(r.fwd_wino && d->Cout % 4 == 0, "conv_forward: wino_mg given for a call that does not take the Winograd path (abr_conv_wino_mg_floats)");
+        ABR_REQUIRE(!d->wino_v && !d->scale && !d->bias && !d->relu, "conv_forward: an input gradient from wino_mg takes mask / out / out_amax only");
+    }
     if (h3) {
         abr::AmaxRef ar{reinterpret_cast<unsigned long long*>(const_cast<uint64_t*>(d->x_amax)), d->x_amax_epoch};
-        if (!ar.word) {
+        if (!ar.word && !d->wino_mg) {
             ar = abr::h3_amax_alloc();
             ABR_REQUIRE(ar.word && abr::h3_amax_reduce(x, (int64_t)d->B * d->H * d->W * d->Cin, ar, st) == 0, "conv_forward (f16x3): amax reduction failed");
         }
@@ -1502,7 +1550,7 @@
         p.wp_bytes = (unsigned)h3_planes_bytes(d->Cout, p.K);
     }
     if (r.fwd_wino) {
-        ABR_REQUIRE(wino_conv(p, r, x, w, out, st), "conv_forward (winograd): no memory for the scratch or an amax word, or a launch failed");
+        ABR_REQUIRE(wino_conv(p, r, x, w, out, st, d->wino_mg), "conv_forward (winograd): no memory for the scratch or an amax word, or a launch failed");
         ABR_CHECK_LAUNCH("conv_forward (winograd)");
         return ABR_OK;
     }
@@ -1608,25 +1656,27 @@
         std::vector<void*>& t; bool committed = false;
         ~TokenGuard() { if (!committed && !t.empty()) abr::derived_abandon(t.data(), (int)t.size()); }
     } token_guard{tokens};
-    auto derive = [&](const float* w, int Cout, int R, int S, int Cin, int stride, int pad, int math, int64_t ver) {
+    auto derive = [&](const float* w, int Cout, int R, int S, int Cin, int stride, int pad, int math, int64_t ver, int taps) {
         const abr::ConvRoute r = prep_route(Cout, R, S, Cin, stride, pad, math);
         if (r.kind == abr::DERIVED_NONE) return true;
         void* tok = nullptr;
-        void* dst = abr::derived_acquire(w, r.kind, r.bytes, ver, st, &tok, &waited);
+        void* dst = abr::derived_acquire(w, r.kind | (taps ? abr::DERIVED_TAPS_REVERSED : 0), r.bytes, ver, st, &tok, &waited);
         if (!dst) return false;
         if (tok) {
             tokens.push_back(tok);
-            plan.derived(r, w, dst);
+            plan.derived(r, w, dst, taps);
         }
         return true;
     };
     for (int i = 0; i < n; i++) {
         const abr_prep_item& it = items[i];
         ABR_REQUIRE(it.w && it.w_version != 0 && it.Cout > 0 && it.R > 0 && it.S > 0 && it.Cin > 0, "conv_prepare_batch: bad item");
-        ABR_REQUIRE(derive(it.w, it.Cout, it.R, it.S, it.Cin, it.stride, it.pad, it.math, it.w_version), "conv_prepare_batch: no memory for the derived weights");
+        ABR_REQUIRE(derive(it.w, it.Cout, it.R, it.S, it.Cin, it.stride, it.pad, it.math, it.w_version, 0), "conv_prepare_batch: no memory for the derived weights");
         if (it.wt) {
             plan.transpose(it.w, it.scale, it.wt, it.Cout, it.R * it.S, it.Cin);
-            ABR_REQUIRE(derive(it.wt, it.Cin, it.R, it.S, it.Cout, 1, it.R - 1 - it.pad, it.math, it.w_version),
+            abr_conv_desc fd{};
+            fd.Cout = it.Cout; fd.R = it.R; fd.S = it.S; fd.Cin = it.Cin; fd.stride = it.stride; fd.pad = it.pad; fd.math = it.math;
+            ABR_REQUIRE(derive(it.wt, it.Cin, it.R, it.S, it.Cout, 1, it.R - 1 - it.pad, it.math, it.w_version, abr::conv_dgrad_adjoint(fd) ? 1 : 0),
                         "conv_prepare_batch: no memory for the derived weights");
         }
     }
@@ -1650,6 +1700,7 @@
             case ABR_OP_FORWARD: rc = abr_conv_forward(&o.desc, o.a, o.b, o.out, o.stream); break;
             case ABR_OP_WGRAD: rc = abr_conv_wgrad(&o.desc, o.a, o.b, o.out, o.stream); break;
             case ABR_OP_STREAM_WAIT: rc = abr_stream_wait_stream(o.stream, o.other); break;
+            case ABR_OP_WINO_OUTGRAD: rc = abr_conv_wino_outgrad(&o.desc, o.b, o.stream); break;
             default: ABR_REQUIRE(false, "conv_run: unknown op kind");
         }
         if (rc != ABR_OK) return rc;
diff --git a/abr_iod_amd/csrc/conv_wgrad.hip b/abr_iod_amd/csrc/conv_wgrad.hip
--- a/abr_iod_amd/csrc/conv_wgrad.hip
+++ b/abr_iod_amd/csrc/conv_wgrad.hip
@@ -587,20 +587,23 @@
         const int64_t T = (int64_t)d->B * th_n * tw_n;
         const size_t nV = (size_t)36 * T * d->Cin, nM = (size_t)36 * T * d->Cout, nU = (size_t)36 * d->Cout * d->Cin;
         float* vin = route.v_floats ? d->wino_v : nullptr;
-        float* ws = abr::wino_ws(st, (vin ? 0 : nV) + nM + nU);
+        float* mgin = d->wino_mg;
+        float* ws = abr::wino_ws(st, (vin ? 0 : nV) + (mgin ? 0 : nM) + nU);
         if (ws) {
             float* V = vin ? vin : ws;
-            float *Mg = ws + (vin ? 0 : nV), *dU = Mg + nM;
+            float *Mg = mgin ? mgin : ws + (vin ? 0 : nV), *dU = ws + (vin ? 0 : nV) + (mgin ? 0 : nM);
             abr::AmaxRef v_ref{nullptr, 0}, m_ref{nullptr, 0};
             if (h3) {
                 if (vin) v_ref = abr::h3_amax_recall(vin);
                 else v_ref = abr::h3_amax_alloc();
-                m_ref = abr::h3_amax_alloc();
-                ABR_REQUIRE(m_ref.word && (vin || v_ref.word), "conv_wgrad (f16x3): no amax words");
+                if (mgin) m_ref = abr::h3_amax_recall(mgin);
+                else m_ref = abr::h3_amax_alloc();
+                ABR_REQUIRE((mgin || m_ref.word) && (vin || v_ref.word), "conv_wgrad (f16x3): no amax words");
                 if (vin && !v_ref.word) ABR_REQUIRE(need_ref(v_ref, vin, (int64_t)nV), "conv_wgrad (f16x3): amax reduction failed");
+                if (mgin && !m_ref.word) ABR_REQUIRE(need_ref(m_ref, mgin, (int64_t)nM), "conv_wgrad (f16x3): amax reduction failed");
             }
             int bad = vin ? 0 : abr::wino_input_transform(x, d->B, d->H, d->W, d->Cin, V, st, h3 ? &v_ref : nullptr);
-            bad |= abr::wino_outgrad_transform(gy, d->B, d->H, d->W, d->Cout, Mg, st, h3 ? &m_ref : nullptr);
+            if (!mgin) bad |= abr::wino_outgrad_transform(gy, d->B, d->H, d->W, d->Cout, Mg, st, h3 ? &m_ref : nullptr);
             const int cus_ = abr::num_cus();
             const long out_tiles = 36L * ((d->Cout + TN_ - 1) / TN_) * ((d->Cin + TK_ - 1) / TK_);
             const int own = out_tiles >= 2L * cus_;
diff --git a/abr_iod_amd/csrc/conv_winograd.hip b/abr_iod_amd/csrc/conv_winograd.hip
--- a/abr_iod_amd/csrc/conv_winograd.hip
+++ b/abr_iod_amd/csrc/conv_winograd.hip
@@ -166,6 +166,7 @@
         u[5].v[e] = t[2];
     }
 }
+__device__ __forceinline__ int wino_tap(int taps, int r, int q) { return taps ? 8 - (3 * r + q) : 3 * r + q; }
 template <typename F>
 __device__ __forceinline__ void for_rows6(F&& f) {
     f(std::integral_constant<int, 0>{}); f(std::integral_constant<int, 1>{}); f(std::integral_constant<int, 2>{});
@@ -188,7 +189,7 @@
 #pragma unroll
     for (int r = 0; r < 3; r++)
 #pragma unroll
-        for (int q = 0; q < 3; q++) g[r][q] = vld<4>(w + ((n * 3 + r) * 3 + q) * C + c);
+        for (int q = 0; q < 3; q++) g[r][q] = vld<4>(w + (n * 9 + wino_tap(jb.taps, r, q)) * C + c);
     for_rows6([&](auto I) {
         constexpr int i = decltype(I)::value;
         fv u[6];
@@ -217,7 +218,7 @@
 #pragma unroll
         for (int r = 0; r < 3; r++)
 #pragma unroll
-            for (int q = 0; q < 3; q++) g[r][q] = vld<4>(w + ((n * 3 + r) * 3 + q) * C + c);
+            for (int q = 0; q < 3; q++) g[r][q] = vld<4>(w + (n * 9 + wino_tap(jb.taps, r, q)) * C + c);
         for_rows6([&](auto I) {
             constexpr int i = decltype(I)::value;
             fv u[6];
@@ -277,7 +278,8 @@
     for (int r = 0; r < 3; r++)
 #pragma unroll
         for (int q = 0; q < 3; q++) {
-            const float4 a = *reinterpret_cast<const float4*>(src + (r * 3 + q) * 64), b = *reinterpret_cast<const float4*>(src + (r * 3 + q) * 64 + 4);
+            const int tap = wino_tap(jb.taps, r, q);
+            const float4 a = *reinterpret_cast<const float4*>(src + tap * 64), b = *reinterpret_cast<const float4*>(src + tap * 64 + 4);
             gA[r][q] = {{a.x, a.y, a.z, a.w}};
             gB[r][q] = {{b.x, b.y, b.z, b.w}};
         }
@@ -430,6 +432,96 @@
 }
 
 template <typename T>
+__device__ __forceinline__ void b6_inner(const T v0, const T v1, const T v2, const T v3, const T v4, const T v5, T& o1, T& o2, T& o3, T& o4) {
+    o1 = 4.f * (v2 - v1) + 2.f * (v4 - v3) + 4.f * v5;
+    o2 = -(5.f * v0) - 4.f * (v1 + v2) - (v3 + v4);
+    o3 = (v1 - v2) + 2.f * (v3 - v4) - 5.f * v5;
+    o4 = v0 + (v1 + v2) + (v3 + v4);
+}
+
+template <int V>
+__global__ __launch_bounds__(256) void wino_ingrad_kernel(const float* __restrict__ dV, int B, int H, int W, int C, int th_n, int tw_n,
+                                                          const float* __restrict__ mask, float* __restrict__ out, unsigned long long* amax, unsigned epoch) {
+    typedef vf<V> f2;
+    unsigned am = 0;
+    const int64_t T = (int64_t)B * th_n * tw_n;
+    const int C2 = C / V;
+    const int64_t total = T * C2;
+    const int64_t ps = T * C;
+    for (int64_t idx = (int64_t)blockIdx.x * blockDim.x + threadIdx.x; idx < total; idx += (int64_t)gridDim.x * blockDim.x) {
+        const int c = V * (int)(idx % C2);
+        const int64_t t = idx / C2;
+        const int tw = (int)(t % tw_n), th = (int)((t / tw_n) % th_n), b = (int)(t / ((int64_t)tw_n * th_n));
+        const float* m = dV + t * C + c;
+        const bool up = th > 0, dn = th + 1 < th_n, lf = tw > 0, rt = tw + 1 < tw_n;
+        const float* mu = up ? m - (int64_t)tw_n * C : m;
+        const float* md = dn ? m + (int64_t)tw_n * C : m;
+        const float* ml = lf ? m - C : m;
+        const float* mr = rt ? m + C : m;
+        f2 mk[4][4];
+        if (mask) {
+#pragma unroll
+            for (int i = 0; i < 4; i++)
+#pragma unroll
+                for (int j = 0; j < 4; j++) {
+                    const int oy = 4 * th + i, ox = 4 * tw + j;
+                    const bool in = oy < H && ox < W;
+                    mk[i][j] = vld<V>(mask + (((int64_t)b * H + (in ? oy : 4 * th)) * W + (in ? ox : 4 * tw)) * C + c);
+                }
+        }
+        f2 tcol[4][6];
+#pragma unroll
+        for (int j = 0; j < 6; j++)
+            b6_inner(vld<V>(m + (0 + j) * ps), vld<V>(m + (6 + j) * ps), vld<V>(m + (12 + j) * ps), vld<V>(m + (18 + j) * ps), vld<V>(m + (24 + j) * ps),
+                     vld<V>(m + (30 + j) * ps), tcol[0][j], tcol[1][j], tcol[2][j], tcol[3][j]);
+        f2 acc[4][4];
+#pragma unroll
+        for (int i = 0; i < 4; i++)
+            b6_inner(tcol[i][0], tcol[i][1], tcol[i][2], tcol[i][3], tcol[i][4], tcol[i][5], acc[i][0], acc[i][1], acc[i][2], acc[i][3]);
+        f2 e[4];
+        b6_inner(vld<V>(mu + 30 * ps), vld<V>(mu + 31 * ps), vld<V>(mu + 32 * ps), vld<V>(mu + 33 * ps), vld<V>(mu + 34 * ps), vld<V>(mu + 35 * ps), e[0], e[1],
+                 e[2], e[3]);
+#pragma unroll
+        for (int j = 0; j < 4; j++) acc[0][j] = acc[0][j] + (up ? e[j] : vzero<V>());
+        b6_inner(vld<V>(md), vld<V>(md + ps), vld<V>(md + 2 * ps), vld<V>(md + 3 * ps), vld<V>(md + 4 * ps), vld<V>(md + 5 * ps), e[0], e[1], e[2], e[3]);
+#pragma unroll
+        for (int j = 0; j < 4; j++) acc[3][j] = acc[3][j] + (dn ? 4.f * e[j] : vzero<V>());
+        b6_inner(vld<V>(ml + 5 * ps), vld<V>(ml + 11 * ps), vld<V>(ml + 17 * ps), vld<V>(ml + 23 * ps), vld<V>(ml + 29 * ps), vld<V>(ml + 35 * ps), e[0], e[1],
+                 e[2], e[3]);
+#pragma unroll
+        for (int i = 0; i < 4; i++) acc[i][0] = acc[i][0] + (lf ? e[i] : vzero<V>());
+        b6_inner(vld<V>(mr), vld<V>(mr + 6 * ps), vld<V>(mr + 12 * ps), vld<V>(mr + 18 * ps), vld<V>(mr + 24 * ps), vld<V>(mr + 30 * ps), e[0], e[1], e[2],
+                 e[3]);
+#pragma unroll
+        for (int i = 0; i < 4; i++) acc[i][3] = acc[i][3] + (rt ? 4.f * e[i] : vzero<V>());
+        const int64_t du = up ? -(int64_t)tw_n * C : 0, dd = dn ? (int64_t)tw_n * C : 0, dl = lf ? -C : 0, dr = rt ? C : 0;
+        const f2 cul = vld<V>(m + du + dl + 35 * ps), cur = vld<V>(m + du + dr + 30 * ps), cdl = vld<V>(m + dd + dl + 5 * ps), cdr = vld<V>(m + dd + dr);
+        acc[0][0] = acc[0][0] + (up && lf ? cul : vzero<V>());
+        acc[0][3] = acc[0][3] + (up && rt ? 4.f * cur : vzero<V>());
+        acc[3][0] = acc[3][0] + (dn && lf ? 4.f * cdl : vzero<V>());
+        acc[3][3] = acc[3][3] + (dn && rt ? 16.f * cdr : vzero<V>());
+#pragma unroll
+        for (int i = 0; i < 4; i++) {
+            const int oy = 4 * th + i;
+            if (oy >= H) continue;
+#pragma unroll
+            for (int j = 0; j < 4; j++) {
+                const int ox = 4 * tw + j;
+                if (ox >= W) continue;
+                f2 v = acc[i][j];
+                if (mask) {
+#pragma unroll
+                    for (int k = 0; k < V; k++) v.v[k] = mk[i][j].v[k] > 0.f ? v.v[k] : 0.f;
+                }
+                vst(out + (((int64_t)b * H + oy) * W + ox) * C + c, v);
+                if (amax) am = vabs_max(am, v);
+            }
+        }
+    }
+    if (amax) abr::h3_amax_emit(amax, epoch, am);
+}
+
+template <typename T>
 __device__ __forceinline__ void gt3(const T u0, const T u1, const T u2, const T u3, const T u4, const T u5, T& o0, T& o1, T& o2) {
     o0 = 0.25f * u0 - (1.f / 6.f) * (u1 + u2) + (1.f / 24.f) * (u3 + u4);
     o1 = (1.f / 6.f) * (u2 - u1) + (1.f / 12.f) * (u3 - u4);
@@ -513,6 +605,17 @@
         wino_output_kernel<4><<<grid_for((int64_t)B * th_n * tw_n * (N / 4), aw != nullptr), 256, 0, st>>>(Mm, B, H, W, N, th_n, tw_n, scale, bias, relu, mask, out, aw, ae);
     else
         wino_output_kernel<2><<<grid_for((int64_t)B * th_n * tw_n * (N / 2), aw != nullptr), 256, 0, st>>>(Mm, B, H, W, N, th_n, tw_n, scale, bias, relu, mask, out, aw, ae);
+    return hipGetLastError() == hipSuccess ? 0 : 1;
+}
+
+int wino_ingrad_transform(const float* dV, int B, int H, int W, int C, const float* mask, float* out, hipStream_t st, const AmaxRef* amax) {
+    const int th_n = (H + 3) / 4, tw_n = (W + 3) / 4;
+    unsigned long long* aw = amax ? amax->word : nullptr;
+    const unsigned ae = amax ? amax->epoch : 0u;
+    if (wide((int64_t)B * th_n * tw_n, C))
+        wino_ingrad_kernel<4><<<grid_for((int64_t)B * th_n * tw_n * (C / 4), aw != nullptr), 256, 0, st>>>(dV, B, H, W, C, th_n, tw_n, mask, out, aw, ae);
+    else
+        wino_ingrad_kernel<2><<<grid_for((int64_t)B * th_n * tw_n * (C / 2), aw != nullptr), 256, 0, st>>>(dV, B, H, W, C, th_n, tw_n, mask, out, aw, ae);
     return hipGetLastError() == hipSuccess ? 0 : 1;
 }
 
diff --git a/abr_iod_amd/modeling/backbone/resnet.py b/abr_iod_amd/modeling/backbone/resnet.py
--- a/abr_iod_amd/modeling/backbone/resnet.py
+++ b/abr_iod_amd/modeling/backbone/resnet.py
@@ -379,8 +379,8 @@
             return self._bwd_pairs(x, o1, o2, s, v2, g, need_dx, mask_dx, s1, s2, s3)
         ops.conv_wgrad_async(o2, g, _grad_buf(self.conv3.weight), 1, 0, scale=s3, math=self.math)
         g2 = self._dgrad(g, self.conv3, s3, 0, mask=o2)
-        ops.conv_wgrad_async(o1, g2, _grad_buf(self.conv2.weight), 1, 1, scale=s2, math=self.math, wino_v=v2)
-        g1 = self._dgrad(g2, self.conv2, s2, 1, mask=o1)
+        g1 = ops.conv_backward(o1, g2, _grad_buf(self.conv2.weight), self.conv2.dgrad_weight(s2), 1, 1, scale=s2, math=self.math,
+                               w_version=self.conv2.version(), wino_v=v2, mask=o1)
         ops.conv_wgrad_async(x, g1, _grad_buf(self.conv1.weight), s, 0, scale=s1, math=self.math)
         ds = self.downsample
         if ds is not None:
diff --git a/abr_iod_amd/modeling/rpn/rpn.py b/abr_iod_amd/modeling/rpn/rpn.py
--- a/abr_iod_amd/modeling/rpn/rpn.py
+++ b/abr_iod_amd/modeling/rpn/rpn.py
@@ -170,9 +170,10 @@
         ops.conv_wgrad_async(t, g, head.fused_weight_grad, 1, 0, math=head.math)
         ops.bias_grad(g, head.fused_bias_grad)
         gt = ops.conv_forward(g, head.fused_dgrad_weight(), 1, 0, mask=t, math=head.math)
-        ops.conv_wgrad_async(xh, gt, _grad_buf(head.conv.weight), 1, 1, math=head.math, wino_v=v)
         ops.bias_grad(gt, _grad_buf(head.conv.bias))
-        gx = from_nhwc(ops.conv_forward(gt, head.conv.dgrad_weight(), 1, 1, math=head.math, w_version=head.conv.version())) if ctx.need_dx else None
+        gx = ops.conv_backward(xh, gt, _grad_buf(head.conv.weight), head.conv.dgrad_weight() if ctx.need_dx else None, 1, 1, math=head.math,
+                               w_version=head.conv.version(), wino_v=v, dgrad=ctx.need_dx)
+        gx = from_nhwc(gx) if ctx.need_dx else None
         ctx.saved = None
         return (gx, None) + (None,) * (len(ctx.needs_input_grad) - 2)
 
diff --git a/abr_iod_amd/ops.py b/abr_iod_amd/ops.py
--- a/abr_iod_amd/ops.py
+++ b/abr_iod_amd/ops.py
@@ -552,8 +552,8 @@
     return w, e
 
 
-def amax_wgrad_operands(x, gy, wino_v=None):
-    return amax_operand(x, reduce=wino_v is None), amax_operand(gy)
+def amax_wgrad_operands(x, gy, wino_v=None, wino_mg=None):
+    return amax_operand(x, reduce=wino_v is None), amax_operand(gy, reduce=wino_mg is None)
 
 
 def conv_out_emits(out, residual, sh, sw, emit_amax, math):
@@ -709,16 +709,39 @@
     return torch.empty(n, dtype=_f32, device=x.device) if n > 0 else None
 
 
+_mg_floats = {}
+
+
+def wino_mg_floats(x_shape, w_shape, stride, pad, math=MATH_F32):
+    key = (tuple(x_shape), tuple(w_shape), stride, pad, math)
+    n = _mg_floats.get(key)
+    if n is None:
+        if len(_mg_floats) > 8192:
+            _mg_floats.clear()
+        d = conv_desc(key[0], key[1], stride, pad, math=math)
+        n = _mg_floats[key] = int(L.lib().abr_conv_wino_mg_floats(C.byref(d)))
+    return n
+
+
+def wino_outgrad(gy, x_shape, w_shape, stride, pad, math=MATH_F32):
+    mg = torch.empty(wino_mg_floats(x_shape, w_shape, stride, pad, math), dtype=_f32, device=gy.device)
+    d = conv_desc(tuple(x_shape), tuple(w_shape), stride, pad, math=math)
+    d.wino_mg = mg.data_ptr()
+    L.check(L.lib().abr_conv_wino_outgrad(C.byref(d), L.ptr(gy), L.stream()), "conv_wino_outgrad")
+    return mg
+
+
 def conv_forward(x, w, stride=1, pad=0, scale=None, bias=None, residual=None, mask=None, relu=False,
-                 out=None, out_hw=None, out_stride=(1, 1), math=MATH_F32, wino_v=None, w_planes=None, w_version=0, emit_amax=None):
+                 out=None, out_hw=None, out_stride=(1, 1), math=MATH_F32, wino_v=None, w_planes=None, w_version=0, emit_amax=None, wino_mg=None):
     L.require_cuda(x, w)
     xc, w = L.f32c(x), L.f32c(w)
     d = conv_desc(xc.shape, w.shape, stride, pad, scale, bias, residual, mask, relu, out_hw, out_stride, math)
     d.wino_v = L.ptr(wino_v)
+    d.wino_mg = L.ptr(wino_mg)
     d.w_planes = L.ptr(w_planes)
     d.w_version = int(w_version)
     if uses_amax(math):
-        d.x_amax, d.x_amax_epoch = amax_operand(xc)
+        d.x_amax, d.x_amax_epoch = amax_operand(xc, reduce=wino_mg is None)
     fresh = out is None
     ow, oe = amax_new() if conv_out_emits(out, residual, d.out_sh, d.out_sw, emit_amax, math) else (None, 0)
     d.out_amax, d.out_amax_epoch = ow, oe
@@ -824,13 +847,14 @@
     return int(L.lib().abr_scratch_bytes())
 
 
-def conv_wgrad(x, gy, dw, stride=1, pad=0, scale=None, math=MATH_F32, wino_v=None, amax_refs=None, stream=None):
+def conv_wgrad(x, gy, dw, stride=1, pad=0, scale=None, math=MATH_F32, wino_v=None, amax_refs=None, stream=None, wino_mg=None):
     L.require_cuda(x, gy, dw)
     xc, gyc = L.f32c(x), L.f32c(gy)
     d = conv_desc(xc.shape, dw.shape, stride, pad, scale=scale, math=math)
     d.wino_v = L.ptr(wino_v)
+    d.wino_mg = L.ptr(wino_mg)
     if uses_amax(math):
-        (d.x_amax, d.x_amax_epoch), (d.gy_amax, d.gy_amax_epoch) = amax_refs or amax_wgrad_operands(xc, gyc, wino_v)
+        (d.x_amax, d.x_amax_epoch), (d.gy_amax, d.gy_amax_epoch) = amax_refs or amax_wgrad_operands(xc, gyc, wino_v, wino_mg)
     L.check(L.lib().abr_conv_wgrad(C.byref(d), L.ptr(xc), L.ptr(gyc), L.ptr(dw), L.stream() if stream is None else stream), "conv_wgrad")
     return dw
 
@@ -929,18 +953,18 @@
         del lst[:]
 
 
-def conv_wgrad_async(x, gy, dw, stride=1, pad=0, scale=None, math=MATH_F32, wino_v=None):
+def conv_wgrad_async(x, gy, dw, stride=1, pad=0, scale=None, math=MATH_F32, wino_v=None, wino_mg=None):
     if not WGRAD_SIDE_STREAM:
-        return conv_wgrad(x, gy, dw, stride, pad, scale, math, wino_v)
+        return conv_wgrad(x, gy, dw, stride, pad, scale, math, wino_v, wino_mg=wino_mg)
     side = _wgrad_stream(x.device.index, _wgrad_owner(dw))
     _arm_join()
     x, gy = L.f32c(x), L.f32c(gy)
-    refs = amax_wgrad_operands(x, gy, wino_v) if uses_amax(math) else None
+    refs = amax_wgrad_operands(x, gy, wino_v, wino_mg) if uses_amax(math) else None
     raw = side.cuda_stream
     main = L.stream()
     L.check(L.lib().abr_stream_wait_stream(raw, main), "stream_wait_stream")
-    conv_wgrad(x, gy, dw, stride, pad, scale, math, wino_v, amax_refs=refs, stream=raw)
-    _wg_hold(main, (x, gy, wino_v))
+    conv_wgrad(x, gy, dw, stride, pad, scale, math, wino_v, amax_refs=refs, stream=raw, wino_mg=wino_mg)
+    _wg_hold(main, (x, gy, wino_v, wino_mg))
     return dw
 
 
@@ -949,12 +973,17 @@
 
 def conv_backward(x, gy, dw, wt, stride, pad, scale=None, math=MATH_F32, w_version=0, wino_v=None, dgrad=True, mask=None, residual=None,
                   out=None, out_hw=None, out_stride=(1, 1)):
+    mg_floats = wino_mg_floats(x.shape, dw.shape, stride, pad, math) if dgrad and out_hw is None else 0
     if not (WGRAD_SIDE_STREAM and H3_TAGS and x.is_contiguous() and gy.is_contiguous() and x.dtype == _f32 and gy.dtype == _f32):
-        conv_wgrad_async(x, gy, dw, stride, pad, scale=scale, math=math, wino_v=wino_v)
+        mg = None
+        if mg_floats and residual is None:
+            gy = L.f32c(gy)
+            mg = wino_outgrad(gy, x.shape, dw.shape, stride, pad, math)
+        conv_wgrad_async(x, gy, dw, stride, pad, scale=scale, math=math, wino_v=wino_v, wino_mg=mg)
         if not dgrad:
             return None
         return conv_forward(gy, wt, 1, dw.shape[1] - 1 - pad, mask=mask, residual=residual, out=out, out_hw=out_hw, out_stride=out_stride,
-                            math=math, w_version=w_version)
+                            math=math, w_version=w_version, wino_mg=mg)
     key = (dw.data_ptr(), x.shape, gy.shape, stride, pad, math, dgrad, out_hw, out_stride, wino_v is not None)
     plan = _bwd_plans.get(key)
     wtp = wt.data_ptr() if dgrad else 0
@@ -962,37 +991,47 @@
     if plan is None or plan[2] != wtp or plan[3] != scp:
         if len(_bwd_plans) > 4096:
             _bwd_plans.clear()
-        arr = (L.ConvOp * 3)()
-        arr[0].kind = L.OP_STREAM_WAIT
-        arr[1].kind = L.OP_WGRAD
-        arr[1].desc = conv_desc(x.shape, dw.shape, stride, pad, scale=scale, math=math)
-        arr[1].out = dw.data_ptr()
+        arr = (L.ConvOp * 4)()
+        arr[0].kind = L.OP_WINO_OUTGRAD
+        arr[0].desc = conv_desc(x.shape, dw.shape, stride, pad, scale=scale, math=math)
+        arr[1].kind = L.OP_STREAM_WAIT
+        arr[2].kind = L.OP_WGRAD
+        arr[2].desc = conv_desc(x.shape, dw.shape, stride, pad, scale=scale, math=math)
+        arr[2].out = dw.data_ptr()
         if dgrad:
-            arr[2].kind = L.OP_FORWARD
-            arr[2].desc = conv_desc(gy.shape, wt.shape, 1, dw.shape[1] - 1 - pad, out_hw=out_hw, out_stride=out_stride, math=math)
-            arr[2].b = wtp
-        plan = _bwd_plans[key] = (arr, C.cast(arr, C.c_void_p), wtp, scp, _wgrad_owner(dw), (scale, dw), threading.Lock())
+            arr[3].kind = L.OP_FORWARD
+            arr[3].desc = conv_desc(gy.shape, wt.shape, 1, dw.shape[1] - 1 - pad, out_hw=out_hw, out_stride=out_stride, math=math)
+            arr[3].b = wtp
+        ptrs = (C.cast(arr, C.c_void_p), C.c_void_p(C.addressof(arr) + C.sizeof(L.ConvOp)))
+        plan = _bwd_plans[key] = (arr, ptrs, wtp, scp, _wgrad_owner(dw), (scale, dw), threading.Lock())
     arr, ptr, _, _, owner, _, lock = plan
     with lock:
-        return _conv_backward_run(arr, ptr, owner, x, gy, dw, math, wino_v, dgrad, mask, residual, out, out_hw, w_version)
-
-
-def _conv_backward_run(arr, ptr, owner, x, gy, dw, math, wino_v, dgrad, mask, residual, out, out_hw, w_version):
+        return _conv_backward_run(arr, ptr, owner, x, gy, dw, math, wino_v, dgrad, mask, residual, out, out_hw, w_version, mg_floats)
+
+
+def _conv_backward_run(arr, ptr, owner, x, gy, dw, math, wino_v, dgrad, mask, residual, out, out_hw, w_version, mg_floats=0):
     side = _wgrad_stream(x.device.index, owner).cuda_stream
     _arm_join()
     main = L.stream()
     h3 = uses_amax(math)
     xp, gp = x.data_ptr(), gy.data_ptr()
-    a0, a1 = arr[0], arr[1]
+    mg = torch.empty(mg_floats, dtype=_f32, device=x.device) if mg_floats and residual is None else None
+    mgp = mg.data_ptr() if mg is not None else None
+    a0, a1 = arr[1], arr[2]
     a0.stream, a0.other = side, main
     a1.a, a1.b, a1.stream = xp, gp, side
     d1 = a1.desc
     d1.wino_v = wino_v.data_ptr() if wino_v is not None else None
+    d1.wino_mg = mgp
+    if mg is not None:
+        ag = arr[0]
+        ag.b, ag.stream = gp, main
+        ag.desc.wino_mg = mgp
     if h3:
-        (d1.x_amax, d1.x_amax_epoch), (gw, ge) = amax_wgrad_operands(x, gy, wino_v)
+        (d1.x_amax, d1.x_amax_epoch), (gw, ge) = amax_wgrad_operands(x, gy, wino_v, mg)
         d1.gy_amax, d1.gy_amax_epoch = gw, ge
     if dgrad:
-        a2 = arr[2]
+        a2 = arr[3]
         d2 = a2.desc
         fresh = out is None
         ow, oe = amax_new() if conv_out_emits(out, residual, d2.out_sh, d2.out_sw, None, math) else (None, 0)
@@ -1004,10 +1043,14 @@
         d2.residual = residual.data_ptr() if residual is not None else None
         d2.mask = mask.data_ptr() if mask is not None else None
         d2.w_version = int(w_version)
-    L.check(L.lib().abr_conv_run(ptr, 3 if dgrad else 2), "conv_run (conv backward)")
+        d2.wino_mg = mgp
+    if mg is not None:
+        L.check(L.lib().abr_conv_run(ptr[0], 4), "conv_run (conv backward)")
+    else:
+        L.check(L.lib().abr_conv_run(ptr[1], 3 if dgrad else 2), "conv_run (conv backward)")
     if dgrad:
         conv_out_done(out, fresh, ow, oe, d2.out_sh, d2.out_sw)
-    _wg_hold(main, (x, gy, wino_v))
+    _wg_hold(main, (x, gy, wino_v, mg))
     return out if dgrad else None
 
 
diff --git a/include/abr_iod_hip.h b/include/abr_iod_hip.h
--- a/include/abr_iod_hip.h
+++ b/include/abr_iod_hip.h
@@ -176,6 +176,7 @@
     const uint64_t* x_amax;   uint32_t x_amax_epoch;
     const uint64_t* gy_amax;  uint32_t gy_amax_epoch;
     uint64_t* out_amax;       uint32_t out_amax_epoch;
+    float* wino_mg;
 } abr_conv_desc;
 
 #define ABR_H3_AMAX_RING 65536
@@ -202,6 +203,7 @@
 #define ABR_OP_FORWARD 0
 #define ABR_OP_WGRAD 1
 #define ABR_OP_STREAM_WAIT 2
+#define ABR_OP_WINO_OUTGRAD 3
 typedef struct abr_conv_op {
     int32_t kind;
     int32_t reserved;
@@ -218,6 +220,8 @@
 int64_t abr_conv_cache_bytes(void);
 int64_t abr_scratch_bytes(void);
 int64_t abr_conv_wino_v_floats(const abr_conv_desc* d_host);
+int64_t abr_conv_wino_mg_floats(const abr_conv_desc* d_host);
+int abr_conv_wino_outgrad(const abr_conv_desc* d_host, const float* gy, void* stream);
 int abr_conv_route_info(const abr_conv_desc* d_host, int32_t out[4]);
 int64_t abr_conv_packed_bytes(int64_t rows, int64_t K);
 int abr_conv_pack_weights(const float* w, int64_t rows, int K, void* planes, void* stream);
```

New measurement: 231.1, median of 6. About the same (+0.9%).
